# cliangyu/video-diffusion

Measured on AMD Instinct MI355X. Metric: denoise-steps/sec, higher is better.
Workload: dtype f32

## Files before the change

include/vd_amd.h:

```cpp
#ifndef VD_AMD_H
#define VD_AMD_H
#ifdef __cplusplus
extern "C" {
#endif

typedef struct vd_config {
    int image_size;
    int num_channels;
    int num_res_blocks;
    int num_heads;
    int T;
    int n_attention_ds;
    int attention_ds[8];
    int use_scale_shift_norm;
    int use_spatial_encoding;
    int use_frame_encoding;
    int enforce_position_invariance;
    int use_rpe_net;
    int allow_interactions_between_padding;
    float rp_alpha, rp_beta, rp_gamma;
    int time_embed_mult;
    int cond_emb_type;
    int learn_sigma;
} vd_config;
// ... 121 lines not shown
int vd_known_region(vd_engine* e);
int vd_known_merge(vd_engine* e, int B, int T, long long frame_pixels, float* sample, const float* known_src, const float* known_mask,
                   const float* latent_mask, const long long* t, const float* known_noise, unsigned long long seed,
                   unsigned long long offset, void* stream);
int vd_set_jump_rows(vd_engine* e, int num_timesteps, const float* sqrt_alpha, const float* sqrt_beta);
int vd_q_jump(vd_engine* e, int B, int T, long long frame_pixels, const float* x, const float* latent_mask, const long long* t,
              const float* noise, unsigned long long seed, unsigned long long offset, float* out, void* stream);
int vd_window_jump(vd_engine* e, int n, void* stream);

int vd_set_measurement(vd_engine* e, const float* y, int scale, int gray);
int vd_measurement(vd_engine* e, int* scale, int* gray);
int vd_measurement_project(vd_engine* e, int B, int T, int H, int W, float* x0_inout, const float* y, const float* latent_mask, int scale,
                           int gray, void* stream);

int vd_posterior_update(vd_engine* e, int mode, int B, long long per_sample, const float* x, const float* eps,
                        const long long* t, int clip_denoised, float eta, const float* noise,
                        unsigned long long seed, unsigned long long offset, float* sample, float* pred_xstart,
                        void* stream);

int vd_posterior_from_xstart(vd_engine* e, int mode, int B, long long per_sample, const float* x, const float* xstart_in,
                             const long long* t, int clip_denoised, float eta, const float* noise,
                             unsigned long long seed, unsigned long long offset, float* sample, float* pred_xstart,
                             float* mean, void* stream);

int vd_attn_blocks(vd_engine* e);
int vd_attn_block_info(vd_engine* e, int i, int* resolution, int* channels);
int vd_set_attn_capture(vd_engine* e, float* const* temporal, float* const* spatial, int n);

long long vd_bwd_weights_bytes(vd_engine* e);
int vd_set_bwd_weight_storage(vd_engine* e, void* buf, long long bytes, int on_host);
int vd_load_weight_bwd(vd_engine* e, const char* name, const float* host_data, long long numel);
int vd_guided_step(vd_engine* e, int B, int T, const float* x, const float* obs_mask, const float* latent_mask,
                   const float* kinda_marg_mask, const long long* frame_indices, const long long* t, int clip_denoised,
                   const float* x_t_minus_1, const float* noise, const float* noise2, float* mean, float* pred_xstart,
                   float* grad, float* sample, void* stream);

int vd_q_sample(vd_engine* e, int B, long long per_sample, const float* x_start, const long long* t,
                const float* noise, float* out, void* stream);

int vd_randn(float* out, long long n, unsigned long long seed, unsigned long long offset, void* stream);

int vd_profile_begin(void);
int vd_profile_end(double* out, int cap);
int vd_profile_classes(void);
const char* vd_profile_class_name(int i);

int vd_math_mode(void);
long long vd_split_image_u16(long long n_out, long long k_total);

int vd_op_conv(const float* src0, const float* src1, int C0, int Cin, int nfr, int Hs, int Ws, int ups, int stride,
               int pad, int ksz, const float* w_packed, const float* w_frag, const float* w_wino, const float* bias,
               const float* affA, const float* affB, int act, const float* res, const float* fbias, int fbias_ld,
               float* out, int Cout, void* stream);
int vd_conv_stats_split(int Hout);
int vd_conv_wino_block_couts(int nfr, int H, int Cin, int Cout);
int vd_op_conv_stats(const float* src0, int Cin, int nfr, int Hs, int Ws, int ups, const float* w_wino, const float* bias,
                     const float* res, const float* fbias, int fbias_ld, float* out, int Cout, double* gn_part,
                     void* stream);
int vd_op_gn_affine(const double* part0, int split0, int C0, const double* part1, int split1, int C, int nfr, int HW,
                    const float* gamma, const float* beta, const float* film, int film_ld, float* affA, float* affB,
                    void* stream);
int vd_pack_conv3_wino(const float* host_oihw, float* host_out, int O, int I);
int vd_pack_linear_frag(const float* host_w, float* host_out, int N, int K);
int vd_pack_linear_split(const float* host_w, unsigned short* host_out, int N, int K);
int vd_pack_conv3_split(const float* host_oihw, unsigned short* host_out, int O, int I);
int vd_op_conv_split(const float* src0, int Cin, int nfr, int Hs, int Ws, int stride, const void* w_split, const float* bias,
                     const float* res, float* out, int Cout, void* stream);
int vd_pack_conv3_wino_split(const float* host_oihw, unsigned short* host_out, int O, int I);
int vd_op_conv_wino_split(const float* src0, int Cin, int nfr, int Hs, int Ws, int ups, const void* w_split, const float* bias,
                          const float* res, const float* fbias, int fbias_ld, float* out, int Cout, double* gn_part,
                          void* stream);
int vd_op_conv_wino_act(const float* src0, const float* src1, int C0, int Cin, int nfr, int Hs, int Ws, const void* w_split, const float* bias,
                        const float* affA, const float* affB, const float* res, float* out, int Cout, double* gn_part, void* stream);
int vd_conv_wino_act_ok(int nfr, int H, int Cin, int Cout);
int vd_pack_conv3_wino_ups(const float* host_oihw, unsigned short* host_out, int O, int I);
int vd_conv_ups_stats_split(int Hs);
int vd_op_conv_wino_ups(const float* src0, int Cin, int nfr, int Hs, const void* w_ups, const float* bias, float* out, int Cout,
                        double* gn_part, void* stream);
int vd_op_linear_split(const float* a, int M, int K, const void* w_split, const float* bias, const float* res, int act,
                       float* out, int N, void* stream);
int vd_op_linear_split_stats(const float* a, int M, int K, const void* w_split, const float* bias, const float* res, int act,
                             float* out, int N, int HW, double* gn_part, void* stream);
int vd_linear_stats_split(int M, int N, int HW);
int vd_op_gn_fold(const float* src0, const float* src1, int C0, int C, int nfr, int HW, const float* gamma,
                  const float* beta, const float* film, int film_ld, float* affA, float* affB, void* stream);
int vd_op_affine_apply(const float* x, const float* affA, const float* affB, int nfr, int HW, int C, float* y,
                       void* stream);
int vd_op_affine_act(const float* src0, const float* src1, int C0, int C, const float* affA, const float* affB, int nfr,
                     int HW, int act, float* y, void* stream);
int vd_op_gn_temporal(const float* x, const float* gamma, const float* beta, int B, int T, int HW, int C, float* y,
                      void* stream);
int vd_op_attn_spatial(const float* qkv, int nfr, int L, int C, int heads, float* out, void* stream);
int vd_op_attn_temporal(const float* qkv, const float* Rk, const float* Rq, const float* Rv, const float* mask, int B,
                        int T, int HW, int C, int heads, int allow_pad, float* out, void* stream);
int vd_attn_temporal_variant(int T, int HW, int C, int heads, int rpe, char* name, int cap);
int vd_attn_spatial_variant(int L, int C, int heads, char* name, int cap);
int vd_op_out_conv(const float* x, const float* affA, const float* affB, const float* w_packed, const float* bias,
                   int nfr, int H, int W, int C, int Cout, float* out_nchw, void* stream);
int vd_op_gn_bwd(const float* x0, const float* x1, int C0, int C, const float* affA, const float* affB, const float* mr,
                 const float* dy, int act, int nfr, int HW, const float* extra, float* dx0, int acc0, float* dx1, int acc1,
                 void* stream);
int vd_op_gn_temporal_bwd(const float* x, const float* gamma, const float* dy, int B, int T, int HW, int C, int accumulate,
                          float* dx, void* stream);
int vd_op_attn_temporal_bwd(const float* qkv, const float* Rk, const float* Rq, const float* Rv, const float* mask, int B,
                            int T, int HW, int C, int heads, int allow_pad, const float* dout, float* dqkv, void* stream);
int vd_op_attn_spatial_bwd(const float* qkv, int nfr, int L, int C, int heads, const float* dout, float* dqkv, void* stream);
int vd_op_out_conv_bwd(const float* deps, const float* w, int nfr, int H, int W, int C, int Cout, float* da, void* stream);
int vd_op_stem_col2im(const float* dcols, const float* obs, const float* lat, const float* km, int nfr, int H, int W,
                      int cond_mode, float* dx, void* stream);
int vd_op_sinus_embed(const float* t, int n, int dim, const float* freqs, float* out, void* stream);
int vd_op_frame_t(const long long* frame_indices, int B, int T, int center, float* tv, void* stream);
int vd_op_rpe_hidden(const float* te, int te_ld, const float* wbase, const long long* tab, const long long* frame_indices, int B, int T,
                     int C, float* E, int nz, long long zs_e, void* stream);
int vd_op_rpe_table(const float* table, const long long* frame_indices, int B, int T, int C, float alpha, float beta, float gamma,
                    float* R, void* stream);
int vd_op_posenc_add(const float* x, const float* P, const float* femb, int nfr, int HW, int C, float* y, void* stream);
int vd_op_assemble(const float* x, const float* obs_src, const float* obs_mask, const float* latent_mask, const float* kinda_marg_mask,
                   const float* t_model, int obs_t_mode, int B, int T, int H, int W, int Kpad, int cond_mode, const int* frame_list,
                   int n_list, int scalars_only, float* x_cols, float* t_frames, float* amask, void* stream);
int vd_op_move_rows(int scatter, const float* src, const int* list, int n, long long row_floats, float* dst, void* stream);
int vd_op_scatter_stats(const double* src, int split, int C, const int* list, int n, double* dst, void* stream);

typedef struct vd_lpips vd_lpips;
int vd_lpips_create(vd_lpips** out);
void vd_lpips_destroy(vd_lpips* h);
int vd_lpips_load_weight(vd_lpips* h, const char* name, const float* host, long long bytes);
long long vd_lpips_dim(int H, int W);
int vd_lpips_embed(vd_lpips* h, int N, int H, int W, const float* frames, float* out, void* stream);
int vd_fps_select(int B, int n_cand, long long D, const float* embs, int n, const int* always_host, int n_always, float* work,
                  int* out, void* stream);

int vd_frame_metrics(int N, int C, int H, int W, const float* gt, const void* pred, int pred_is_u8, double ssim_data_range,
                     double* ssim_out, double* psnr_out, void* stream);
int vd_pair_sqdist(int N, long long D, const float* a, const float* b, double* out, void* stream);

int vd_hallway_counts(int N, int H, int W, int row0, int row1, const void* frames, int is_u8, int* counts, void* stream);
int vd_hallway_max_strip(void);
int vd_op_green_mask(long long n, const unsigned char* rgb, unsigned char* hsv, unsigned char* mask, void* stream);

typedef struct vd_i3d vd_i3d;
int vd_i3d_create(vd_i3d** out);
void vd_i3d_destroy(vd_i3d* h);
int vd_i3d_load_weight(vd_i3d* h, const char* name, const float* host, long long bytes);
int vd_i3d_max_frames(void);
int vd_i3d_embed(vd_i3d* h, int N, int T, int H, int W, const unsigned char* videos, float* out, void* stream);
int vd_op_conv3d_same(const float* x, const float* w, const float* bias, int T, int H, int W, int Cin, int Cout, int kt, int kh,
                      int kw, int st, int sh, int sw, int relu, float* out, long long out_stride, void* stream);
int vd_op_maxpool3d_same(const float* x, int T, int H, int W, int C, int kt, int kh, int kw, int st, int sh, int sw, float* out,
                         void* stream);
int vd_op_resize_bilinear_tf1(const unsigned char* frames, int T, int H, int W, float* out, void* stream);

#ifdef __cplusplus
}
#endif
#endif
```

video-diffusion_amd/_lib.py:

```python
import ctypes
import os
import subprocess

_HERE = os.path.dirname(os.path.abspath(__file__))
_CSRC = os.path.join(_HERE, "csrc")
SO_PATH = os.path.join(_HERE, "libvdamd.so")
SOURCES = ["igemm.hip", "conv_wino.hip", "conv_wino_r64.hip", "conv_wino_z128.hip", "gemm_frag.hip", "gemm_split.hip", "split_pack.hip", "norm.hip", "backward.hip", "attn_spatial.hip", "attn_temporal.hip", "attn_temporal_long.hip", "misc.hip", "guidance.hip", "known.hip", "measure.hip", "engine.hip", "lpips.hip", "metrics.hip", "i3d.hip", "conv_cl.hip", "hallway.hip"]
HEADER = os.path.join(os.path.dirname(_HERE), "include", "vd_amd.h")
HEADERS = [os.path.join(_CSRC, "vd_common.h"), os.path.join(_CSRC, "wino_common.h"), os.path.join(_CSRC, "igemm_tile.h"), HEADER]
SOURCE_FLAGS = {"conv_wino_z128.hip": ["-mllvm", "-pragma-unroll-threshold=1000000"]}


def _toolchain():
    hipcc = os.environ.get("HIPCC", "/opt/rocm/bin/hipcc")
    flags = ["--offload-arch=gfx950", "-O3", "-std=c++17", "-fPIC", "-Wno-unused-value"] + \
        os.environ.get("VD_HIPCC_FLAGS", "").split()
    return hipcc, flags


def _sha(*parts):
    import hashlib
    h = hashlib.sha1()
    for p in parts:
        h.update(p if isinstance(p, bytes) else str(p).encode())
# ... 114 lines not shown
    "vd_device_errors": (_I, [_P, ctypes.POINTER(_I)]),
    "vd_pos_channels": (_I, [_P]),
    "vd_pos_resolution": (_I, [_P]),
    "vd_set_freqs": (_I, [_P, _P, _I, _P, _I]),
    "vd_set_schedule": (_I, [_P, _I, _P, _P, _F]),
    "vd_workspace_bytes": (_I, [_P, _I, _I, ctypes.POINTER(_L)]),
    "vd_unet_forward": (_I, [_P, _I, _I, _P, _P, _P, _P, _P, _P, _P, _I, _P, _P]),
    "vd_p_sample": (_I, [_P, _I, _I, _P, _P, _P, _P, _P, _P, _P, _I, _I, _P, _U, _U, _P, _P, _P, _P]),
    "vd_ddim_sample": (_I, [_P, _I, _I, _P, _P, _P, _P, _P, _P, _P, _I, _I, _F, _P, _U, _U, _P, _P, _P, _P]),
    "vd_ddim_reverse_sample": (_I, [_P, _I, _I, _P, _P, _P, _P, _P, _P, _P, _I, _I, _P, _P, _P, _P]),
    "vd_ddim_reverse_from_xstart": (_I, [_P, _I, _L, _P, _P, _P, _I, _P, _P, _P]),
    "vd_set_multistep_weights": (_I, [_P, _I, _P]),
    "vd_dpmpp_2m_sample": (_I, [_P, _I, _I, _P, _P, _P, _P, _P, _P, _P, _P, _I, _I, _P, _P, _P, _P]),
    "vd_dpmpp_2m_from_xstart": (_I, [_P, _I, _L, _P, _P, _P, _P, _I, _P, _P, _P]),
    "vd_p_mean_variance": (_I, [_P, _I, _I, _P, _P, _P, _P, _P, _P, _P, _I, _I, _P, _P, _P, _P]),
    "vd_vb_terms": (_I, [_P, _I, _I, _P, _P, _P, _P, _P, _I, _P, _P, _P, _P, _P, _P]),
    "vd_prior_bpd": (_I, [_P, _I, _I, _P, _P, _P, _P]),
    "vd_score_windows": (_I, [_P, _I, _I, _P, _P, _P, _P, _P, _P, _I, _U, _P, _P, _I, _P, _P]),
    "vd_op_eps_mse": (_I, [_P, _I, _I, _P, _P, _P, _I, _P, _U, _P, _P, _P, _P]),
    "vd_window_generation": (_U, [_P]),
    "vd_set_window_prefix_cache": (_I, [_P, _I]),
    "vd_window_prefix_frames": (_I, [_P]),
    "vd_set_window_suffix_skip": (_I, [_P, _I]),
    "vd_window_suffix_frames": (_I, [_P]),
    "vd_set_cfg_scale": (_I, [_P, _F]),
    "vd_cfg_scale": (_F, [_P]),
    "vd_op_cfg_combine": (_I, [_P, _P, _F, _L, _P, _P]),
    "vd_set_guidance_rescale": (_I, [_P, _F]),
    "vd_guidance_rescale": (_F, [_P]),
    "vd_set_dynamic_threshold": (_I, [_P, _F]),
    "vd_dynamic_threshold": (_F, [_P]),
    "vd_op_cfg_rescale": (_I, [_P, _P, _F, _P, _I, _I, _L, _F, _P, _P, _P]),
    "vd_op_dynamic_threshold": (_I, [_P, _P, _I, _I, _L, _F, _P, _P, _P]),
    "vd_set_known_region": (_I, [_P, _P, _P, _P, _U, _U]),
    "vd_known_region": (_I, [_P]),
    "vd_known_merge": (_I, [_P, _I, _I, _L, _P, _P, _P, _P, _P, _P, _U, _U, _P]),
    "vd_set_jump_rows": (_I, [_P, _I, _P, _P]),
    "vd_q_jump": (_I, [_P, _I, _I, _L, _P, _P, _P, _P, _U, _U, _P, _P]),
    "vd_window_jump": (_I, [_P, _I, _P]),
    "vd_set_measurement": (_I, [_P, _P, _I, _I]),
    "vd_measurement": (_I, [_P, _P, _P]),
    "vd_measurement_project": (_I, [_P, _I, _I, _I, _I, _P, _P, _P, _I, _I, _P]),
    "vd_window_begin": (_I, [_P, _I, _I, _P, _P, _P, _P, _P, _P, _I, _I, _I, _F, _U, _U, _L, _P]),
    "vd_window_run": (_I, [_P, _I, _P]),
    "vd_window_graphs": (_I, [_P]),
    "vd_posterior_update": (_I, [_P, _I, _I, _L, _P, _P, _P, _I, _F, _P, _U, _U, _P, _P, _P]),
    "vd_posterior_from_xstart": (_I, [_P, _I, _I, _L, _P, _P, _P, _I, _F, _P, _U, _U, _P, _P, _P, _P]),
    "vd_attn_blocks": (_I, [_P]),
    "vd_attn_block_info": (_I, [_P, _I, ctypes.POINTER(_I), ctypes.POINTER(_I)]),
    "vd_set_attn_capture": (_I, [_P, _P, _P, _I]),
    "vd_bwd_weights_bytes": (_L, [_P]),
    "vd_set_bwd_weight_storage": (_I, [_P, _P, _L, _I]),
    "vd_load_weight_bwd": (_I, [_P, ctypes.c_char_p, _P, _L]),
    "vd_guided_step": (_I, [_P, _I, _I, _P, _P, _P, _P, _P, _P, _I, _P, _P, _P, _P, _P, _P, _P, _P]),
    "vd_q_sample": (_I, [_P, _I, _L, _P, _P, _P, _P, _P]),
    "vd_randn": (_I, [_P, _L, _U, _U, _P]),
    "vd_profile_begin": (_I, []),
    "vd_profile_end": (_I, [_P, _I]),
    "vd_profile_classes": (_I, []),
    "vd_profile_class_name": (ctypes.c_char_p, [_I]),
    "vd_op_conv": (_I, [_P, _P, _I, _I, _I, _I, _I, _I, _I, _I, _I, _P, _P, _P, _P, _P, _P, _I, _P, _P, _I, _P, _I, _P]),
    "vd_conv_stats_split": (_I, [_I]),
    "vd_conv_wino_block_couts": (_I, [_I, _I, _I, _I]),
    "vd_op_conv_stats": (_I, [_P, _I, _I, _I, _I, _I, _P, _P, _P, _P, _I, _P, _I, _P, _P]),
    "vd_op_gn_affine": (_I, [_P, _I, _I, _P, _I, _I, _I, _I, _P, _P, _P, _I, _P, _P, _P]),
    "vd_pack_conv3_wino": (_I, [_P, _P, _I, _I]),
    "vd_pack_linear_frag": (_I, [_P, _P, _I, _I]),
    "vd_pack_linear_split": (_I, [_P, _P, _I, _I]),
    "vd_pack_conv3_wino_split": (_I, [_P, _P, _I, _I]),
    "vd_set_model_mean_type": (_I, [_P, _I]),
    "vd_math_mode": (_I, []),
    "vd_split_image_u16": (_L, [_L, _L]),
    "vd_pack_conv3_wino_ups": (_I, [_P, _P, _I, _I]),
    "vd_conv_ups_stats_split": (_I, [_I]),
    "vd_op_conv_wino_ups": (_I, [_P, _I, _I, _I, _P, _P, _P, _I, _P, _P]),
    "vd_op_conv_wino_split": (_I, [_P, _I, _I, _I, _I, _I, _P, _P, _P, _P, _I, _P, _I, _P, _P]),
    "vd_op_conv_wino_act": (_I, [_P, _P, _I, _I, _I, _I, _I, _P, _P, _P, _P, _P, _P, _I, _P, _P]),
    "vd_conv_wino_act_ok": (_I, [_I, _I, _I, _I]),
    "vd_pack_conv3_split": (_I, [_P, _P, _I, _I]),
    "vd_op_conv_split": (_I, [_P, _I, _I, _I, _I, _I, _P, _P, _P, _P, _I, _P]),
    "vd_op_linear_split": (_I, [_P, _I, _I, _P, _P, _P, _I, _P, _I, _P]),
    "vd_op_linear_split_stats": (_I, [_P, _I, _I, _P, _P, _P, _I, _P, _I, _I, _P, _P]),
    "vd_linear_stats_split": (_I, [_I, _I, _I]),
    "vd_op_gn_fold": (_I, [_P, _P, _I, _I, _I, _I, _P, _P, _P, _I, _P, _P, _P]),
    "vd_op_affine_apply": (_I, [_P, _P, _P, _I, _I, _I, _P, _P]),
    "vd_op_affine_act": (_I, [_P, _P, _I, _I, _P, _P, _I, _I, _I, _P, _P]),
    "vd_op_gn_temporal": (_I, [_P, _P, _P, _I, _I, _I, _I, _P, _P]),
    "vd_op_attn_spatial": (_I, [_P, _I, _I, _I, _I, _P, _P]),
    "vd_op_attn_temporal": (_I, [_P, _P, _P, _P, _P, _I, _I, _I, _I, _I, _I, _P, _P]),
    "vd_attn_temporal_variant": (_I, [_I, _I, _I, _I, _I, ctypes.c_char_p, _I]),
    "vd_attn_spatial_variant": (_I, [_I, _I, _I, ctypes.c_char_p, _I]),
    "vd_op_out_conv": (_I, [_P, _P, _P, _P, _P, _I, _I, _I, _I, _I, _P, _P]),
    "vd_op_gn_bwd": (_I, [_P, _P, _I, _I, _P, _P, _P, _P, _I, _I, _I, _P, _P, _I, _P, _I, _P]),
    "vd_op_gn_temporal_bwd": (_I, [_P, _P, _P, _I, _I, _I, _I, _I, _P, _P]),
    "vd_op_attn_temporal_bwd": (_I, [_P, _P, _P, _P, _P, _I, _I, _I, _I, _I, _I, _P, _P, _P]),
    "vd_op_attn_spatial_bwd": (_I, [_P, _I, _I, _I, _I, _P, _P, _P]),
    "vd_op_out_conv_bwd": (_I, [_P, _P, _I, _I, _I, _I, _I, _P, _P]),
    "vd_op_stem_col2im": (_I, [_P, _P, _P, _P, _I, _I, _I, _I, _P, _P]),
    "vd_op_sinus_embed": (_I, [_P, _I, _I, _P, _P, _P]),
    "vd_op_frame_t": (_I, [_P, _I, _I, _I, _P, _P]),
    "vd_op_rpe_hidden": (_I, [_P, _I, _P, _P, _P, _I, _I, _I, _P, _I, _L, _P]),
    "vd_op_rpe_table": (_I, [_P, _P, _I, _I, _I, _F, _F, _F, _P, _P]),
    "vd_op_posenc_add": (_I, [_P, _P, _P, _I, _I, _I, _P, _P]),
    "vd_op_assemble": (_I, [_P, _P, _P, _P, _P, _P, _I, _I, _I, _I, _I, _I, _I, _P, _I, _I, _P, _P, _P, _P]),
    "vd_op_move_rows": (_I, [_I, _P, _P, _I, _L, _P, _P]),
    "vd_op_scatter_stats": (_I, [_P, _I, _I, _P, _I, _P, _P]),
    "vd_lpips_create": (_I, [ctypes.POINTER(_P)]),
    "vd_lpips_destroy": (None, [_P]),
    "vd_lpips_load_weight": (_I, [_P, ctypes.c_char_p, _P, _L]),
    "vd_lpips_dim": (_L, [_I, _I]),
    "vd_lpips_embed": (_I, [_P, _I, _I, _I, _P, _P, _P]),
    "vd_fps_select": (_I, [_I, _I, _L, _P, _I, _P, _I, _P, _P, _P]),
    "vd_frame_metrics": (_I, [_I, _I, _I, _I, _P, _P, _I, _D, _P, _P, _P]),
    "vd_pair_sqdist": (_I, [_I, _L, _P, _P, _P, _P]),
    "vd_i3d_create": (_I, [ctypes.POINTER(_P)]),
    "vd_i3d_destroy": (None, [_P]),
    "vd_i3d_load_weight": (_I, [_P, ctypes.c_char_p, _P, _L]),
    "vd_i3d_max_frames": (_I, []),
    "vd_i3d_embed": (_I, [_P, _I, _I, _I, _I, _P, _P, _P]),
    "vd_op_conv3d_same": (_I, [_P, _P, _P, _I, _I, _I, _I, _I, _I, _I, _I, _I, _I, _I, _I, _P, _L, _P]),
    "vd_op_maxpool3d_same": (_I, [_P, _I, _I, _I, _I, _I, _I, _I, _I, _I, _I, _P, _P]),
    "vd_op_resize_bilinear_tf1": (_I, [_P, _I, _I, _I, _P, _P]),
    "vd_hallway_counts": (_I, [_I, _I, _I, _I, _I, _P, _I, _P, _P]),
    "vd_hallway_max_strip": (_I, []),
    "vd_op_green_mask": (_I, [_L, _P, _P, _P, _P]),
}

_lib = None


def lib():
    global _lib
    if _lib is None:
        path = os.environ.get("VD_LIB")
        if not path:
            build()
            path = SO_PATH
        L = ctypes.CDLL(path)
        for name, (res, args) in SIGNATURES.items():
            fn = getattr(L, name)
            fn.restype = res
            fn.argtypes = args
        if not os.environ.get("VD_LIB") and L.vd_source_sha().decode() != source_sha():
            raise RuntimeError(f"libvdamd.so was built from other sources ({L.vd_source_sha().decode()}) than the ones beside it "
                               f"({source_sha()}): rebuild (video_diffusion_amd._lib.build(force=True))")
        _lib = L
    return _lib


class VdError(RuntimeError):
    pass


def check(rc):
    if rc != 0:
        msg = lib().vd_last_error().decode(errors="replace")
        raise VdError(f"libvdamd error {rc}: {msg}")


def ptr(t):
    if t is None:
        return None
    if hasattr(t, "data_ptr"):
        return ctypes.c_void_p(t.data_ptr())
    return ctypes.c_void_p(t.ctypes.data)

# ... 5 lines not shown
```

video-diffusion_amd/csrc/attn_temporal.hip:

```cpp
#include "vd_common.h"
#include <cstdlib>
#include <string>

namespace vd {

__device__ __forceinline__ float dot4(f32x4 a, f32x4 b) { return a.x * b.x + a.y * b.y + a.z * b.z + a.w * b.w; }

template <int PB, int TMAX, bool RPE>
__global__ __launch_bounds__(256) void attn_temporal_kernel(AttnTemporalArgs a) {
    extern __shared__ __attribute__((aligned(16))) float smem[];
    const int T = a.T, C = a.C, HW = a.HW, C3 = 3 * a.C;
    const int F = C / a.heads, F4 = F >> 2, FP = F + 4, TS = T + 1;
    float* qs = smem;
    float* ks = qs + PB * T * FP;
    float* sc = ks + PB * T * FP;
    const int b = blockIdx.z, h = blockIdx.y, p0 = blockIdx.x * PB;
    const int np = min(PB, HW - p0);
    const int tid = threadIdx.x;
    const float* qkv_b = a.qkv + (size_t)b * T * HW * C3 + h * F;

    for (int idx = tid; idx < PB * T * F4; idx += 256) {
        const int f4 = idx % F4, r = idx / F4;
        const int t = r % T, p = r / T;
        const float* src = qkv_b + ((size_t)t * HW + p0 + min(p, np - 1)) * C3 + f4 * 4;
        f32x4 q = *reinterpret_cast<const f32x4*>(src) * a.scale;
        f32x4 k = *reinterpret_cast<const f32x4*>(src + C);
        if (p >= np) { q = f32x4{0.f, 0.f, 0.f, 0.f}; k = q; }
        *reinterpret_cast<f32x4*>(qs + (p * T + t) * FP + f4 * 4) = q;
        *reinterpret_cast<f32x4*>(ks + (p * T + t) * FP + f4 * 4) = k;
    }
    __syncthreads();

    for (int pr = tid; pr < T * T; pr += 256) {
        const int t = pr / T, s = pr - t * T;
        float acc[PB];
#pragma unroll
        for (int p = 0; p < PB; ++p) acc[p] = 0.f;
        const float* rk = RPE ? a.Rk + (((size_t)b * T + t) * T + s) * C + h * F : nullptr;
        const float* rq = RPE ? a.Rq + (((size_t)b * T + s) * T + t) * C + h * F : nullptr;
        const float* qrow = qs + t * FP;
        const float* krow = ks + s * FP;
#pragma unroll 3
        for (int f0 = 0; f0 < F; f0 += 8) {
            f32x4 rk0, rk1, rq0, rq1;
            if constexpr (RPE) {
                rk0 = *reinterpret_cast<const f32x4*>(rk + f0); rk1 = *reinterpret_cast<const f32x4*>(rk + f0 + 4);
                rq0 = *reinterpret_cast<const f32x4*>(rq + f0) * a.scale; rq1 = *reinterpret_cast<const f32x4*>(rq + f0 + 4) * a.scale;
            }
#pragma unroll
            for (int p = 0; p < PB; ++p) {
                const f32x4 q0 = *reinterpret_cast<const f32x4*>(qrow + p * T * FP + f0);
                const f32x4 q1 = *reinterpret_cast<const f32x4*>(qrow + p * T * FP + f0 + 4);
                const f32x4 k0 = *reinterpret_cast<const f32x4*>(krow + p * T * FP + f0);
                const f32x4 k1 = *reinterpret_cast<const f32x4*>(krow + p * T * FP + f0 + 4);
                if constexpr (RPE)
                    acc[p] += dot4(q0, k0 + rk0) + dot4(q1, k1 + rk1) + dot4(k0, rq0) + dot4(k1, rq1);
                else
                    acc[p] += dot4(q0, k0) + dot4(q1, k1);
            }
        }
        bool masked = false;
        if (a.mask) {
            const float mt = a.mask[b * T + t], ms = a.mask[b * T + s];
            float allowed = mt * ms;
            if (a.allow_pad) allowed += (1.f - mt) * (1.f - ms);
            else if (t == s) allowed = 1.f;
            masked = allowed == 0.f;
        }
#pragma unroll
        for (int p = 0; p < PB; ++p) sc[(p * T + t) * TS + s] = masked ? -INFINITY : acc[p];
    }
    __syncthreads();

    for (int row = tid; row < np * T; row += 256) {
        float* r = sc + row * TS;
        float mx = -INFINITY;
        for (int s = 0; s < T; ++s) mx = fmaxf(mx, r[s]);
        float sum = 0.f;
        for (int s = 0; s < T; ++s) { const float e = __expf(r[s] - mx); r[s] = e; sum += e; }
        const float inv = 1.0f / sum;
        for (int s = 0; s < T; ++s) r[s] *= inv;
    }
    __syncthreads();

    for (int item = tid; item < T * F4; item += 256) {
        const int t = item / F4, f4 = item - t * F4;
        f32x4 rv[TMAX];
#pragma unroll
        for (int s = 0; s < TMAX; ++s) {
            rv[s] = f32x4{0.f, 0.f, 0.f, 0.f};
            if constexpr (RPE)
                rv[s] = *reinterpret_cast<const f32x4*>(a.Rv + (((size_t)b * T + t) * T + min(s, T - 1)) * C + h * F + f4 * 4);
        }
        for (int p = 0; p < np; ++p) {
            const float* ar = sc + (p * T + t) * TS;
            const float* vbase = qkv_b + 2 * C + (size_t)(p0 + p) * C3 + f4 * 4;
            f32x4 o = {0.f, 0.f, 0.f, 0.f};
#pragma unroll
            for (int s = 0; s < TMAX; ++s) {
                const f32x4 v = *reinterpret_cast<const f32x4*>(vbase + (size_t)min(s, T - 1) * HW * C3);
                const float w = s < T ? ar[min(s, T - 1)] : 0.f;
                o += (v + rv[s]) * w;
            }
            *reinterpret_cast<f32x4*>(a.out + (((size_t)b * T + t) * HW + p0 + p) * C + h * F + f4 * 4) = o;
        }
    }
}

#ifdef VD_ATT_TIMING
__device__ unsigned long long g_att_stamp[16];
#define ATT_STAMP(i)                                                                                   \
    do {                                                                                               \
        if (threadIdx.x == 0 && blockIdx.x == 3 && blockIdx.y == 1 && blockIdx.z == 2) {               \
            __builtin_amdgcn_sched_barrier(0);                                                         \
            g_att_stamp[i] = __builtin_amdgcn_s_memrealtime();                                         \
            __builtin_amdgcn_sched_barrier(0);                                                         \
        }                                                                                              \
    } while (0)
extern "C" int vd_debug_att_stamps(unsigned long long* host_out) {
    return (int)hipMemcpyFromSymbol(host_out, HIP_SYMBOL(g_att_stamp), sizeof(g_att_stamp));
}
#else
#define ATT_STAMP(i)
#endif

__device__ __forceinline__ f32x4 mfma4(float x, float y, f32x4 c) { return __builtin_amdgcn_mfma_f32_16x16x4f32(x, y, c, 0, 0, 0); }

__device__ __forceinline__ void rows_regs_transpose(float& x0, float& x1, float& x2, float& x3) {
    auto u = [](float f) { return __builtin_bit_cast(unsigned, f); };
    auto f = [](unsigned v) { return __builtin_bit_cast(float, v); };
    auto p01 = __builtin_amdgcn_permlane16_swap(u(x0), u(x1), false, false);
    auto p23 = __builtin_amdgcn_permlane16_swap(u(x2), u(x3), false, false);
    auto q02 = __builtin_amdgcn_permlane32_swap(p01[0], p23[0], false, false);
    auto q13 = __builtin_amdgcn_permlane32_swap(p01[1], p23[1], false, false);
    x0 = f(q02[0]); x2 = f(q02[1]); x1 = f(q13[0]); x3 = f(q13[1]);
}

template <int NT, int JM, bool RPE, bool EXACT>
__global__ __launch_bounds__(512, 2) void attn_temporal_mfma_kernel(AttnTemporalArgs a) {
    constexpr int TP = 16 * NT, RS = TP + 1, PS = TP * RS + (NT == 1 ? 1 : 17);
    extern __shared__ __attribute__((aligned(16))) float smem[];
    float* w = smem;
    const int T = EXACT ? 16 * NT : a.T, C = a.C, HW = a.HW, C3 = 3 * a.C;
    const int F = C / a.heads, NJ = EXACT ? JM : F >> 4;
    const int b = blockIdx.z, h = blockIdx.y, p0 = blockIdx.x * 16;
    const int tid = threadIdx.x, wv = tid >> 6, l = tid & 63, i16 = l & 15, g = l >> 4;
    const float* qb = a.qkv + ((size_t)b * T * HW + p0) * C3 + h * F;
    auto row = [&](int t, int px) { return qb + ((size_t)t * HW + px) * C3; };
    auto ld4 = [](const float* p) { return *reinterpret_cast<const f32x4*>(p); };
    const int tcl[2] = {min(i16, T - 1), min(16 + i16, T - 1)};
    const f32x4 zero4 = {0.f, 0.f, 0.f, 0.f};

    ATT_STAMP(0);
    constexpr int JG = NT == 1 ? 2 : 1, NG = JM / JG, NU = 2 * NT;
    constexpr bool AHEAD = NT == 1;
    struct Ops { f32x4 qa1[2][NT][JG], kb1[2][NT][JG], xa2[NU][JG], rb2[NU][NT][JG], xa3[NU][JG], rb3[NU][NT][JG]; };
    f32x4 acc1[2][NT][NT], acc2[NU][NT], acc3[NU][NT];
#pragma unroll
    for (int u = 0; u < 2; ++u)
#pragma unroll
        for (int m = 0; m < NT; ++m)
#pragma unroll
            for (int n = 0; n < NT; ++n) acc1[u][m][n] = zero4;
#pragma unroll
    for (int u = 0; u < NU; ++u)
#pragma unroll
        for (int n = 0; n < NT; ++n) { acc2[u][n] = zero4; acc3[u][n] = zero4; }
    const float* q1[2][NT];
#pragma unroll
    for (int u = 0; u < 2; ++u)
#pragma unroll
        for (int m = 0; m < NT; ++m) q1[u][m] = row(tcl[m], 2 * wv + u) + 4 * g;
    const float* rkq[NT];
#pragma unroll
    for (int n = 0; n < NT; ++n) rkq[n] = (size_t)b * T * T * C + (size_t)tcl[n] * C + h * F + 4 * g + (const float*)nullptr;
    auto request = [&](Ops& o, int grp, bool own, bool rel) {
#pragma unroll
        for (int jj = 0; jj < JG; ++jj) {
            const int j = grp * JG + jj;
            if (EXACT || j < NJ) {
                if (own) {
#pragma unroll
                    for (int u = 0; u < 2; ++u)
#pragma unroll
                        for (int m = 0; m < NT; ++m) { o.qa1[u][m][jj] = ld4(q1[u][m] + 16 * j); o.kb1[u][m][jj] = ld4(q1[u][m] + C + 16 * j); }
                }
                if constexpr (RPE) {
#pragma unroll
                    for (int u = 0; u < (rel ? NU : 0); ++u) {
                        const int t = wv + 8 * u;
                        if (EXACT || t < T) {
                            const float* xr = row(t, i16) + 4 * g + 16 * j;
                            o.xa2[u][jj] = ld4(xr);
                            o.xa3[u][jj] = ld4(xr + C);
#pragma unroll
                            for (int n = 0; n < NT; ++n) {
                                const size_t ro = (size_t)(rkq[n] - (const float*)nullptr) + (size_t)t * T * C + 16 * j;
                                o.rb2[u][n][jj] = ld4(a.Rk + ro);
                                o.rb3[u][n][jj] = ld4(a.Rq + ro);
                            }
                        }
                    }
                }
            }
        }
    };
    auto products = [&](const Ops& o, int grp, bool own, bool rel) {
#pragma unroll
        for (int jj = 0; jj < JG; ++jj) {
            if (EXACT || grp * JG + jj < NJ) {
#pragma unroll
                for (int e = 0; e < 4; ++e) {
#pragma unroll
                    for (int u = 0; u < (own ? 2 : 0); ++u)
#pragma unroll
                        for (int m = 0; m < NT; ++m)
#pragma unroll
                            for (int n = 0; n < NT; ++n) acc1[u][m][n] = mfma4(o.qa1[u][m][jj][e] * a.scale, o.kb1[u][n][jj][e], acc1[u][m][n]);
                    if constexpr (RPE) {
#pragma unroll
                        for (int u = 0; u < (rel ? NU : 0); ++u)
                            if (EXACT || wv + 8 * u < T) {
#pragma unroll
                                for (int n = 0; n < NT; ++n) {
                                    acc2[u][n] = mfma4(o.xa2[u][jj][e] * a.scale, o.rb2[u][n][jj][e], acc2[u][n]);
                                    acc3[u][n] = mfma4(o.xa3[u][jj][e], o.rb3[u][n][jj][e] * a.scale, acc3[u][n]);
                                }
                            }
                    }
                }
            }
        }
    };
    if constexpr (AHEAD) {
        Ops o[2];
        request(o[0], 0, true, true);
#pragma unroll
        for (int grp = 0; grp < NG; ++grp) {
            if (grp + 1 < NG) request(o[(grp + 1) & 1], grp + 1, true, true);
            __builtin_amdgcn_sched_barrier(0);
            products(o[grp & 1], grp, true, true);
            __builtin_amdgcn_sched_barrier(0);
        }
    } else {
#pragma unroll 1
        for (int grp = 0; grp < NG; ++grp) {
            Ops o;
            request(o, grp, true, false);
            products(o, grp, true, false);
            if constexpr (RPE) {
                request(o, grp, false, true);
                products(o, grp, false, true);
            }
        }
    }
    ATT_STAMP(1);
#pragma unroll
    for (int u = 0; u < 2; ++u)
#pragma unroll
        for (int m = 0; m < NT; ++m)
#pragma unroll
            for (int n = 0; n < NT; ++n)
#pragma unroll
                for (int r = 0; r < 4; ++r) w[(2 * wv + u) * PS + (16 * m + 4 * g + r) * RS + 16 * n + i16] = acc1[u][m][n][r];
    __syncthreads();
    if constexpr (RPE) {
#pragma unroll
        for (int u = 0; u < NU; ++u) {
            const int t = wv + 8 * u;
            if (t < T) {
#pragma unroll
                for (int n = 0; n < NT; ++n)
#pragma unroll
                    for (int r = 0; r < 4; ++r) w[(4 * g + r) * PS + t * RS + 16 * n + i16] += acc2[u][n][r];
            }
        }
        __syncthreads();
#pragma unroll
        for (int u = 0; u < NU; ++u) {
            const int sk = wv + 8 * u;
            if (sk < T) {
#pragma unroll
                for (int n = 0; n < NT; ++n)
#pragma unroll
                    for (int r = 0; r < 4; ++r) w[(4 * g + r) * PS + (16 * n + i16) * RS + sk] += acc3[u][n][r];
            }
        }
        __syncthreads();
    }

    ATT_STAMP(2);
    for (int rix = tid; rix < 16 * TP; rix += 512) {
        const int px = rix / TP, t = rix - px * TP;
        float* r = w + px * PS + t * RS;
        if (t >= T) {
            for (int s = 0; s < TP; ++s) r[s] = 0.f;
            continue;
        }
        float mx = -INFINITY;
        const float mt = a.mask ? a.mask[b * T + t] : 1.f;
        for (int s = 0; s < T; ++s) {
            float v = r[s];
            if (a.mask) {
                const float ms = a.mask[b * T + s];
                float allowed = mt * ms;
                if (a.allow_pad) allowed += (1.f - mt) * (1.f - ms);
                else if (t == s) allowed = 1.f;
                if (allowed == 0.f) v = -INFINITY;
            }
            r[s] = v;
            mx = fmaxf(mx, v);
        }
        float sum = 0.f;
        for (int s = 0; s < T; ++s) { const float e = __expf(r[s] - mx); r[s] = e; sum += e; }
        const float inv = 1.0f / sum;
        for (int s = 0; s < T; ++s) r[s] *= inv;
        for (int s = T; s < TP; ++s) r[s] = 0.f;
    }
    __syncthreads();

    ATT_STAMP(3);
    const int KS = (T + 3) >> 2;
    if (EXACT ? wv < JM : wv < NJ) {
        const int f0 = 16 * wv + i16;
        const float* vb = qb + 2 * C + f0;
        const float* rvb = RPE ? a.Rv + ((size_t)b * T) * T * C + h * F + f0 : nullptr;
#pragma unroll 1
        for (int m = 0; m < NT; ++m) {
            if (16 * m >= T) break;
            float rr[NT == 1 ? 4 : 1][16];
            f32x4 acc[16];
#pragma unroll
            for (int px = 0; px < 16; ++px) acc[px] = zero4;
#pragma unroll 1
            for (int kc = 0; kc < NT; ++kc) {
                if (16 * kc >= T) break;
                float vr[4][16];
#pragma unroll
                for (int k4 = 0; k4 < 4; ++k4)
                    if (EXACT || 4 * kc + k4 < KS) {
                        const float* vs = vb + (size_t)min(16 * kc + 4 * k4 + g, T - 1) * HW * C3;
#pragma unroll
                        for (int px = 0; px < 16; ++px) vr[k4][px] = vs[(size_t)px * C3];
                    }
                if constexpr (RPE && NT == 1) {
#pragma unroll
                    for (int k4 = 0; k4 < 4; ++k4)
                        if (EXACT || k4 < KS) {
                            const float* rv = rvb + (size_t)min(4 * k4 + g, T - 1) * C;
#pragma unroll
                            for (int tl = 0; tl < 16; ++tl) rr[k4][tl] = rv[(size_t)min(tl, T - 1) * T * C];
                        }
                }
                __builtin_amdgcn_sched_barrier(0);
#pragma unroll
                for (int k4 = 0; k4 < 4; ++k4)
                    if (EXACT || 4 * kc + k4 < KS) {
                        const float* ar = w + (16 * m + i16) * RS + 16 * kc + 4 * k4 + g;
#pragma unroll
                        for (int px = 0; px < 16; ++px) acc[px] = mfma4(ar[px * PS], vr[k4][px], acc[px]);
                    }
            }
            ATT_STAMP(4);
            f32x4 res[16];
#pragma unroll
            for (int bq = 0; bq < 4; ++bq)
#pragma unroll
                for (int d = 0; d < 4; ++d) {
                    float x0 = acc[bq][d], x1 = acc[4 + bq][d], x2 = acc[8 + bq][d], x3 = acc[12 + bq][d];
                    rows_regs_transpose(x0, x1, x2, x3);
                    res[d][bq] = x0; res[4 + d][bq] = x1; res[8 + d][bq] = x2; res[12 + d][bq] = x3;
                }
            if constexpr (RPE) {
                if constexpr (NT == 1) {
#pragma unroll
                    for (int k4 = 0; k4 < 4; ++k4)
                        if (EXACT || k4 < KS) {
                            const float* ar = w + i16 * PS + 4 * k4 + g;
#pragma unroll
                            for (int tl = 0; tl < 16; ++tl) res[tl] = mfma4(ar[tl * RS], rr[k4][tl], res[tl]);
                        }
                } else {
#pragma unroll 1
                    for (int kc = 0; kc < NT; ++kc) {
                        if (16 * kc >= T) break;
                        float r4[4][16];
#pragma unroll
                        for (int k4 = 0; k4 < 4; ++k4)
                            if (4 * kc + k4 < KS) {
                                const float* rv = rvb + (size_t)min(16 * kc + 4 * k4 + g, T - 1) * C;
#pragma unroll
                                for (int tl = 0; tl < 16; ++tl) r4[k4][tl] = rv[(size_t)min(16 * m + tl, T - 1) * T * C];
                            }
#pragma unroll
                        for (int k4 = 0; k4 < 4; ++k4)
                            if (4 * kc + k4 < KS) {
                                const float* ar = w + i16 * PS + (16 * m) * RS + 16 * kc + 4 * k4 + g;
#pragma unroll
                                for (int tl = 0; tl < 16; ++tl) res[tl] = mfma4(ar[tl * RS], r4[k4][tl], res[tl]);
                            }
                    }
                }
            }
            ATT_STAMP(5);
#pragma unroll
            for (int tl = 0; tl < 16; ++tl) {
                const int t = 16 * m + tl;
                if (t < T) {
                    float* o = a.out + (((size_t)b * T + t) * HW + p0 + 4 * g) * C + h * F + f0;
// ... 85 lines not shown
```

video-diffusion_amd/csrc/attn_temporal_long.hip:

```cpp
#include "vd_common.h"

namespace vd {

namespace {

__device__ __forceinline__ f32x4 mfma_l(float x, float y, f32x4 c) { return __builtin_amdgcn_mfma_f32_16x16x4f32(x, y, c, 0, 0, 0); }

__device__ __forceinline__ void rows_regs_transpose_l(float& x0, float& x1, float& x2, float& x3) {
    auto u = [](float f) { return __builtin_bit_cast(unsigned, f); };
    auto f = [](unsigned v) { return __builtin_bit_cast(float, v); };
    auto p01 = __builtin_amdgcn_permlane16_swap(u(x0), u(x1), false, false);
    auto p23 = __builtin_amdgcn_permlane16_swap(u(x2), u(x3), false, false);
    auto q02 = __builtin_amdgcn_permlane32_swap(p01[0], p23[0], false, false);
    auto q13 = __builtin_amdgcn_permlane32_swap(p01[1], p23[1], false, false);
    x0 = f(q02[0]); x2 = f(q02[1]); x1 = f(q13[0]); x3 = f(q13[1]);
}

__device__ __forceinline__ bool frame_pair_allowed(const AttnTemporalArgs& a, int b, int t, int s) {
    if (!a.mask) return true;
    const float mt = a.mask[b * a.T + t], ms = a.mask[b * a.T + s];
    float allowed = mt * ms;
    if (a.allow_pad) allowed += (1.f - mt) * (1.f - ms);
    else if (t == s) allowed = 1.f;
    return allowed != 0.f;
}

}

template <int NJ, bool RPE>
__global__ __launch_bounds__(512, 2) void attn_temporal_long_mfma_kernel(AttnTemporalArgs a) {
    constexpr int RS = 17, PS = 16 * RS;
    extern __shared__ __attribute__((aligned(16))) float smem[];
    float* pb = smem;
    float* al = pb + 16 * PS;
    float* s1 = al + 256;
    float* s2 = s1 + 16 * PS;
    float* s3 = s2 + 16 * PS;
    const int T = a.T, C = a.C, HW = a.HW, C3 = 3 * a.C, F = 16 * NJ;
    const int NQ = (T + 15) >> 4;
    const int b = blockIdx.z / NQ, t0 = 16 * (blockIdx.z - b * NQ), h = blockIdx.y, p0 = blockIdx.x * 16;
    const int tid = threadIdx.x, wv = tid >> 6, l = tid & 63, i16 = l & 15, g = l >> 4;
    const float* qb = a.qkv + ((size_t)b * T * HW + p0) * C3 + h * F;
    auto row = [&](int t, int px) { return qb + ((size_t)t * HW + px) * C3; };
    auto ld4 = [](const float* p) { return *reinterpret_cast<const f32x4*>(p); };
    const f32x4 zero4 = {0.f, 0.f, 0.f, 0.f};
    const size_t rbase = (size_t)b * T * T * C + h * F;
    const int tq = min(t0 + i16, T - 1);

    f32x4 acc[16];
#pragma unroll
    for (int i = 0; i < 16; ++i) acc[i] = zero4;
    float m_run = -INFINITY, l_run = 0.f;

    const int NK = (T + 15) >> 4;
#pragma unroll 1
    for (int kt = 0; kt < NK; ++kt) {
        const int s0 = 16 * kt;
        const int sk = min(s0 + i16, T - 1);
        f32x4 a1[2], a2[2], a3[2];
#pragma unroll
        for (int u = 0; u < 2; ++u) { a1[u] = zero4; a2[u] = zero4; a3[u] = zero4; }
        const int tf[2] = {min(t0 + wv, T - 1), min(t0 + wv + 8, T - 1)};
        const int sf[2] = {min(s0 + wv, T - 1), min(s0 + wv + 8, T - 1)};
#pragma unroll
        for (int j = 0; j < NJ; ++j) {
            const int fo = 16 * j + 4 * g;
            f32x4 qa[2], kb[2], x2[2], r2[2], x3[2], r3[2];
#pragma unroll
            for (int u = 0; u < 2; ++u) {
                qa[u] = ld4(row(tq, 2 * wv + u) + fo);
                kb[u] = ld4(row(sk, 2 * wv + u) + C + fo);
                if constexpr (RPE) {
                    x2[u] = ld4(row(tf[u], i16) + fo);
                    r2[u] = ld4(a.Rk + rbase + ((size_t)tf[u] * T + sk) * C + fo);
                    x3[u] = ld4(row(sf[u], i16) + C + fo);
                    r3[u] = ld4(a.Rq + rbase + ((size_t)sf[u] * T + tq) * C + fo);
                }
            }
#pragma unroll
            for (int e = 0; e < 4; ++e)
#pragma unroll
                for (int u = 0; u < 2; ++u) {
                    a1[u] = mfma_l(qa[u][e] * a.scale, kb[u][e], a1[u]);
                    if constexpr (RPE) {
                        a2[u] = mfma_l(x2[u][e] * a.scale, r2[u][e], a2[u]);
                        a3[u] = mfma_l(x3[u][e], r3[u][e] * a.scale, a3[u]);
                    }
                }
        }
#pragma unroll
        for (int u = 0; u < 2; ++u)
#pragma unroll
            for (int r = 0; r < 4; ++r) {
                s1[(2 * wv + u) * PS + (4 * g + r) * RS + i16] = a1[u][r];
                if constexpr (RPE) {
                    s2[(4 * g + r) * PS + (wv + 8 * u) * RS + i16] = a2[u][r];
                    s3[(4 * g + r) * PS + i16 * RS + wv + 8 * u] = a3[u][r];
                }
            }
        __syncthreads();

        if (tid < 256) {
            const int px = tid >> 4, tl = tid & 15, t = min(t0 + tl, T - 1);
            const int o = px * PS + tl * RS;
            float w[16];
            float mx = m_run;
#pragma unroll
            for (int s = 0; s < 16; ++s) {
                float v = s1[o + s];
                if constexpr (RPE) v = v + s2[o + s] + s3[o + s];
                if (s0 + s >= T || !frame_pair_allowed(a, b, t, s0 + s)) v = -INFINITY;
                w[s] = v;
                mx = fmaxf(mx, v);
            }
            const bool none = mx == -INFINITY;
            const float alpha = none ? 1.f : __expf(m_run - mx);
            float sum = 0.f;
#pragma unroll
            for (int s = 0; s < 16; ++s) {
                const float p = none ? 0.f : __expf(w[s] - mx);
                pb[o + s] = p;
                sum += p;
            }
            l_run = l_run * alpha + sum;
            m_run = mx;
            al[tid] = alpha;
        }
        __syncthreads();

        if (wv < NJ) {
            const int f0 = h * F + 16 * wv + i16;
#pragma unroll
            for (int tl = 0; tl < 16; ++tl)
#pragma unroll
                for (int r = 0; r < 4; ++r) acc[tl][r] *= al[(4 * g + r) * 16 + tl];
            if constexpr (RPE) {
                const float* rvb = a.Rv + (size_t)b * T * T * C + f0;
#pragma unroll 1
                for (int k4 = 0; k4 < 4; ++k4) {
                    const int s = min(s0 + 4 * k4 + g, T - 1);
                    float rr[16];
#pragma unroll
                    for (int tl = 0; tl < 16; ++tl) rr[tl] = rvb[((size_t)min(t0 + tl, T - 1) * T + s) * C];
#pragma unroll
                    for (int tl = 0; tl < 16; ++tl) acc[tl] = mfma_l(pb[i16 * PS + tl * RS + 4 * k4 + g], rr[tl], acc[tl]);
                }
            }
            f32x4 pv[16];
#pragma unroll
            for (int px = 0; px < 16; ++px) pv[px] = zero4;
            const float* vb = a.qkv + ((size_t)b * T * HW + p0) * C3 + 2 * C + f0;
#pragma unroll 1
            for (int k4 = 0; k4 < 4; ++k4) {
                const int s = min(s0 + 4 * k4 + g, T - 1);
                float vr[16];
#pragma unroll
                for (int px = 0; px < 16; ++px) vr[px] = vb[((size_t)s * HW + px) * C3];
#pragma unroll
                for (int px = 0; px < 16; ++px) pv[px] = mfma_l(pb[px * PS + i16 * RS + 4 * k4 + g], vr[px], pv[px]);
            }
#pragma unroll
            for (int bq = 0; bq < 4; ++bq)
#pragma unroll
                for (int d = 0; d < 4; ++d) {
                    float x0 = pv[bq][d], x1 = pv[4 + bq][d], x2 = pv[8 + bq][d], x3 = pv[12 + bq][d];
                    rows_regs_transpose_l(x0, x1, x2, x3);
                    acc[d][bq] += x0; acc[4 + d][bq] += x1; acc[8 + d][bq] += x2; acc[12 + d][bq] += x3;
                }
        }
    }
    __syncthreads();
    if (tid < 256) al[tid] = 1.0f / l_run;
    __syncthreads();

    if (wv < NJ) {
        const int f0 = h * F + 16 * wv + i16;
#pragma unroll
        for (int tl = 0; tl < 16; ++tl) {
            const int t = t0 + tl;
            if (t < T) {
                float* o = a.out + (((size_t)b * T + t) * HW + p0 + 4 * g) * C + f0;
#pragma unroll
                for (int r = 0; r < 4; ++r) o[(size_t)r * C] = acc[tl][r] * al[(4 * g + r) * 16 + tl];
            }
        }
    }
}

template <bool RPE>
__global__ __launch_bounds__(256) void attn_temporal_long_kernel(AttnTemporalArgs a) {
    extern __shared__ __attribute__((aligned(16))) float sc[];
    const int T = a.T, C = a.C, HW = a.HW, C3 = 3 * a.C, F = C / a.heads, F4 = F >> 2, TS = T + 1;
    const int NQ = (T + 15) >> 4;
    const int b = blockIdx.z / NQ, t0 = 16 * (blockIdx.z - b * NQ), h = blockIdx.y, p = blockIdx.x;
    const int nq = min(16, T - t0);
    const int tid = threadIdx.x;
    const float* qb = a.qkv + ((size_t)b * T * HW + p) * C3 + h * F;
    const size_t fr = (size_t)HW * C3;
    auto ld4 = [](const float* x) { return *reinterpret_cast<const f32x4*>(x); };

    for (int pr = tid; pr < nq * T; pr += 256) {
        const int tl = pr / T, s = pr - tl * T, t = t0 + tl;
        const float* q = qb + t * fr;
        const float* k = qb + s * fr + C;
        const float* rk = RPE ? a.Rk + (((size_t)b * T + t) * T + s) * C + h * F : nullptr;
        const float* rq = RPE ? a.Rq + (((size_t)b * T + s) * T + t) * C + h * F : nullptr;
        float acc = 0.f;
        for (int f = 0; f < F; f += 4) {
            const f32x4 qv = ld4(q + f) * a.scale, kv = ld4(k + f);
            if constexpr (RPE) {
                const f32x4 kr = kv + ld4(rk + f), rqv = ld4(rq + f) * a.scale;
                acc += qv.x * kr.x + qv.y * kr.y + qv.z * kr.z + qv.w * kr.w + kv.x * rqv.x + kv.y * rqv.y + kv.z * rqv.z + kv.w * rqv.w;
            } else {
                acc += qv.x * kv.x + qv.y * kv.y + qv.z * kv.z + qv.w * kv.w;
            }
        }
        sc[tl * TS + s] = frame_pair_allowed(a, b, t, s) ? acc : -INFINITY;
    }
    __syncthreads();
    if (tid < nq) {
        float* r = sc + tid * TS;
        float mx = -INFINITY;
        for (int s = 0; s < T; ++s) mx = fmaxf(mx, r[s]);
        float sum = 0.f;
        for (int s = 0; s < T; ++s) { const float e = mx == -INFINITY ? 0.f : __expf(r[s] - mx); r[s] = e; sum += e; }
        const float inv = 1.0f / sum;
        for (int s = 0; s < T; ++s) r[s] *= inv;
    }
    __syncthreads();
    for (int item = tid; item < nq * F4; item += 256) {
        const int tl = item / F4, f4 = item - tl * F4, t = t0 + tl;
        const float* ar = sc + tl * TS;
        const float* vb = qb + 2 * C + 4 * f4;
        const float* rv = RPE ? a.Rv + (((size_t)b * T + t) * T) * C + h * F + 4 * f4 : nullptr;
        f32x4 o = {0.f, 0.f, 0.f, 0.f};
        for (int s = 0; s < T; ++s) {
            f32x4 v = ld4(vb + s * fr);
            if constexpr (RPE) v += ld4(rv + (size_t)s * C);
            o += v * ar[s];
        }
        *reinterpret_cast<f32x4*>(a.out + (((size_t)b * T + t) * HW + p) * C + h * F + 4 * f4) = o;
    }
}

template <int NJ, bool RPE>
static int launch_long_mfma(const AttnTemporalArgs& a, hipStream_t s) {
    constexpr int PS = 16 * 17;
    constexpr size_t lds = ((size_t)(RPE ? 4 : 2) * 16 * PS + 256) * sizeof(float);
    if (lds > 48 * 1024) VD_RAISE_LDS((&attn_temporal_long_mfma_kernel<NJ, RPE>), lds);
    dim3 grid(a.HW / 16, a.heads, a.B * ((a.T + 15) / 16));
    hipLaunchKernelGGL((attn_temporal_long_mfma_kernel<NJ, RPE>), grid, dim3(512), lds, s, a);
    VD_HIP(hipGetLastError());
    return 0;
}

template <bool RPE>
static int launch_long_generic(const AttnTemporalArgs& a, hipStream_t s) {
    const size_t lds = (size_t)16 * (a.T + 1) * sizeof(float);
    dim3 grid(a.HW, a.heads, a.B * ((a.T + 15) / 16));
    hipLaunchKernelGGL((attn_temporal_long_kernel<RPE>), grid, dim3(256), lds, s, a);
    VD_HIP(hipGetLastError());
    return 0;
}

template <bool RPE>
static int launch_long_nj(const AttnTemporalArgs& a, int nj, hipStream_t s) {
    switch (nj) {
        case 1: return launch_long_mfma<1, RPE>(a, s);
        case 2: return launch_long_mfma<2, RPE>(a, s);
        case 3: return launch_long_mfma<3, RPE>(a, s);
        case 4: return launch_long_mfma<4, RPE>(a, s);
        case 5: return launch_long_mfma<5, RPE>(a, s);
        case 6: return launch_long_mfma<6, RPE>(a, s);
        case 7: return launch_long_mfma<7, RPE>(a, s);
        default: return launch_long_mfma<8, RPE>(a, s);
    }
}

int launch_attn_temporal_long(const AttnTemporalArgs& a, hipStream_t s) {
    const bool rpe = a.Rk != nullptr;
    const AttnTemporalVariant v = attn_temporal_variant(a.T, a.HW, a.C, a.heads, rpe);
    VD_REQUIRE(v.family == AttnTemporalVariant::kLongMfma || v.family == AttnTemporalVariant::kLongGeneric, "long temporal window: 33..128 frames");
    if (v.family == AttnTemporalVariant::kLongMfma) return rpe ? launch_long_nj<true>(a, v.p0, s) : launch_long_nj<false>(a, v.p0, s);
    return rpe ? launch_long_generic<true>(a, s) : launch_long_generic<false>(a, s);
}

}
```

video-diffusion_amd/csrc/backward.hip:

```cpp
#include <algorithm>
#include <cmath>

#include "vd_common.h"

namespace vd {

__device__ __forceinline__ float sigmoid_f(float v) { return __builtin_amdgcn_rcpf(1.0f + __expf(-v)); }
__device__ __forceinline__ float silu_grad_f(float y) { const float s = sigmoid_f(y); return s * (1.0f + y * (1.0f - s)); }

__global__ __launch_bounds__(256) void gn_bwd_partial_kernel(GnBwdArgs a, int split, int per) {
    const int n = blockIdx.y, sp = blockIdx.x;
    const int C = a.C, tpp = C >> 2, ppi = 256 / tpp, cg = C / 32;
    const int tid = threadIdx.x, pl = tid / tpp, q = tid - pl * tpp, c = q * 4;
    const int p_begin = sp * per, p_end = min(a.HW, p_begin + per);
    double t1[4] = {0, 0, 0, 0}, t2[4] = {0, 0, 0, 0};
    if (pl < ppi) {
        const float* src; int ld;
        if (c < a.C0) { src = a.x0 + (size_t)n * a.HW * a.C0 + c; ld = a.C0; } else { src = a.x1 + (size_t)n * a.HW * (C - a.C0) + (c - a.C0); ld = C - a.C0; }
        const f32x4 A = *reinterpret_cast<const f32x4*>(a.A + (size_t)n * C + c), B = *reinterpret_cast<const f32x4*>(a.B + (size_t)n * C + c);
        float mu[4];
#pragma unroll
        for (int e = 0; e < 4; ++e) mu[e] = a.mr[((size_t)n * 32 + (c + e) / cg) * 2];
        for (int p = p_begin + pl; p < p_end; p += ppi) {
            const f32x4 x = *reinterpret_cast<const f32x4*>(src + (size_t)p * ld);
// ... 514 lines not shown
        const float nz = tl != 0 ? 1.0f : 0.0f;
        const float smp = mean + nz * expf(0.5f * tb[TAB_LOGVAR * NT]) * a.noise[i];
        const float om = a.obs[(size_t)b * a.T + (i - (size_t)b * a.per) / perf];
        const float dmean = 2.0f * (smp - a.xtm1[i]) * om * om;
        const float pass = (!a.clip || (x0r >= -1.0f && x0r <= 1.0f)) ? 1.0f : 0.0f;
        const float dx0r = tb[TAB_COEF1 * NT] * dmean * pass;
        a.deps[i] = -tb[TAB_SQRT_RECIPM1 * NT] * dx0r;
        a.dxd[i] = tb[TAB_COEF2 * NT] * dmean + tb[TAB_SQRT_RECIP * NT] * dx0r;
        if (a.mean) a.mean[i] = mean;
        if (a.xstart) a.xstart[i] = x0;
    }
}
int launch_guided_grad(const GuidedArgs& a, hipStream_t s) {
    const size_t total = (size_t)a.B * a.per;
    hipLaunchKernelGGL(guided_grad_kernel, dim3((unsigned)std::min<size_t>((total + 255) / 256, 4096)), dim3(256), 0, s, a);
    VD_HIP(hipGetLastError());
    return 0;
}

__global__ __launch_bounds__(256) void grad_absmax_kernel(const float* __restrict__ g, size_t n, unsigned* __restrict__ mx) {
    float m = 0.f;
    for (size_t i = (size_t)blockIdx.x * 256 + threadIdx.x; i < n; i += (size_t)gridDim.x * 256) m = fmaxf(m, fabsf(g[i]));
    for (int o = 32; o > 0; o >>= 1) m = fmaxf(m, __shfl_xor(m, o));
    if ((threadIdx.x & 63) == 0) atomicMax(mx, __builtin_bit_cast(unsigned, m));
}
__global__ __launch_bounds__(256) void grad_scale_kernel(float* __restrict__ g, size_t n, float* __restrict__ gs) {
    const float m = __builtin_bit_cast(float, reinterpret_cast<const unsigned*>(gs)[2]);
    float s = 1.f;
    if (m > 0.f && m < 3.0e38f) {
        int ex;
        (void)frexpf(m, &ex);
        s = ldexpf(1.f, max(-100, min(100, 1 - ex)));
    }
    if (blockIdx.x == 0 && threadIdx.x == 0) { gs[0] = s; gs[1] = 1.f / s; }
    for (size_t i = (size_t)blockIdx.x * 256 + threadIdx.x; i < n; i += (size_t)gridDim.x * 256) g[i] *= s;
}
int launch_grad_rescale(float* deps, size_t n, float* gs, hipStream_t st) {
    VD_HIP(hipMemsetAsync(gs, 0, 4 * sizeof(float), st));
    const unsigned grid = (unsigned)std::min<size_t>((n + 255) / 256, 1024);
    hipLaunchKernelGGL(grad_absmax_kernel, dim3(grid), dim3(256), 0, st, deps, n, reinterpret_cast<unsigned*>(gs) + 2);
    hipLaunchKernelGGL(grad_scale_kernel, dim3(grid), dim3(256), 0, st, deps, n, gs);
    VD_HIP(hipGetLastError());
    return 0;
}

__global__ __launch_bounds__(256) void guided_final_kernel(GuidedArgs a, const float* __restrict__ dx_net, const float* __restrict__ noise2,
                                                           float* __restrict__ grad, float* __restrict__ mean_out, float* __restrict__ sample) {
    const float inv_s = a.gscale[1];
    const size_t total = (size_t)a.B * a.per;
    for (size_t i = (size_t)blockIdx.x * 256 + threadIdx.x; i < total; i += (size_t)gridDim.x * 256) {
        const int b = (int)(i / a.per);
        const long long tl = a.t[b];
        const int NT = a.num_timesteps;
        if (tl < 0 || tl >= NT) { if (mean_out) mean_out[i] = __builtin_nanf(""); if (sample) sample[i] = __builtin_nanf(""); continue; }
        const float* tb = a.tab + (int)tl;
        const float g = a.dxd[i] + dx_net[i] * inv_s;
        const float m = a.mean[i] - 10.0f * tb[TAB_ALPHA * NT] * g / 2.0f;
        if (grad) grad[i] = g;
        if (mean_out) mean_out[i] = m;
        if (sample) sample[i] = m + (tl != 0 ? 1.0f : 0.0f) * expf(0.5f * tb[TAB_LOGVAR * NT]) * noise2[i];
    }
}
int launch_guided_final(const GuidedArgs& a, const float* dx_net, const float* noise2, float* grad, float* mean_out, float* sample, hipStream_t s) {
    const size_t total = (size_t)a.B * a.per;
    hipLaunchKernelGGL(guided_final_kernel, dim3((unsigned)std::min<size_t>((total + 255) / 256, 4096)), dim3(256), 0, s, a, dx_net, noise2, grad, mean_out,
                       sample);
    VD_HIP(hipGetLastError());
    return 0;
}

}

namespace vd {

template <bool RPE>
__global__ __launch_bounds__(256) void attn_temporal_weights_kernel(AttnTemporalArgs a, float* __restrict__ out) {
    extern __shared__ __attribute__((aligned(16))) float smem[];
    const int T = a.T, C = a.C, HW = a.HW, C3 = 3 * C, F = C / a.heads, FP = F + 4, TS = T + 1;
    float* qs = smem;
    float* ks = qs + T * FP;
    float* P = ks + T * FP;
    float* M = P + T * TS;
    const int p = blockIdx.x, b = blockIdx.y, tid = threadIdx.x;
    const size_t tok0 = (size_t)b * T * HW + p;
    for (int i = tid; i < T * TS; i += 256) M[i] = 0.f;
    for (int h = 0; h < a.heads; ++h) {
        __syncthreads();
        for (int i = tid; i < T * F; i += 256) {
            const int t = i / F, f = i - t * F;
            const float* r = a.qkv + (tok0 + (size_t)t * HW) * C3 + h * F + f;
            qs[t * FP + f] = r[0] * a.scale; ks[t * FP + f] = r[C];
        }
        __syncthreads();
        for (int pr = tid; pr < T * T; pr += 256) {
            const int t = pr / T, s_ = pr - t * T;
            const float* rk = RPE ? a.Rk + (((size_t)b * T + t) * T + s_) * C + h * F : nullptr;
            const float* rq = RPE ? a.Rq + (((size_t)b * T + s_) * T + t) * C + h * F : nullptr;
            float w = 0.f;
            for (int f = 0; f < F; ++f) {
                const float k = ks[s_ * FP + f];
                w += qs[t * FP + f] * (k + (RPE ? rk[f] : 0.f)) + (RPE ? a.scale * k * rq[f] : 0.f);
            }
            bool masked = false;
            if (a.mask) {
                const float mt = a.mask[b * T + t], ms = a.mask[b * T + s_];
                float allowed = mt * ms;
                if (a.allow_pad) allowed += (1.f - mt) * (1.f - ms);
                else if (t == s_) allowed = 1.f;
                masked = allowed == 0.f;
            }
            P[t * TS + s_] = masked ? -INFINITY : w;
        }
        __syncthreads();
        if (tid < T) {
            float* r = P + tid * TS;
            float mx = -INFINITY;
            for (int s_ = 0; s_ < T; ++s_) mx = fmaxf(mx, r[s_]);
            float sum = 0.f;
            for (int s_ = 0; s_ < T; ++s_) { const float e = __expf(r[s_] - mx); r[s_] = e; sum += e; }
            const float inv = 1.0f / sum;
            for (int s_ = 0; s_ < T; ++s_) M[tid * TS + s_] += r[s_] * inv;
        }
    }
    __syncthreads();
    const float ih = 1.0f / (float)a.heads;
    for (int i = tid; i < T * T; i += 256) out[((size_t)b * HW + p) * T * T + i] = fabsf(M[(i / T) * TS + (i % T)] * ih);
}

template <bool RPE>
__global__ __launch_bounds__(256) void attn_temporal_weights_long_kernel(AttnTemporalArgs a, float* __restrict__ out) {
    constexpr int QC = 32;
    extern __shared__ __attribute__((aligned(16))) float smem[];
    const int T = a.T, C = a.C, HW = a.HW, C3 = 3 * C, F = C / a.heads, FP = F + 4, TS = T + 1;
    const int p = blockIdx.x, b = blockIdx.y, r0 = QC * blockIdx.z, nr = min(QC, T - r0), tid = threadIdx.x;
    float* qs = smem;
    float* ks = qs + QC * FP;
    float* P = ks + T * FP;
    float* M = P + QC * TS;
    const size_t tok0 = (size_t)b * T * HW + p;
    for (int i = tid; i < QC * TS; i += 256) M[i] = 0.f;
    for (int h = 0; h < a.heads; ++h) {
        __syncthreads();
        for (int i = tid; i < T * F; i += 256) {
            const int t = i / F, f = i - t * F;
            const float* r = a.qkv + (tok0 + (size_t)t * HW) * C3 + h * F + f;
            if (t >= r0 && t < r0 + nr) qs[(t - r0) * FP + f] = r[0] * a.scale;
            ks[t * FP + f] = r[C];
        }
        __syncthreads();
        for (int pr = tid; pr < nr * T; pr += 256) {
            const int tl = pr / T, s_ = pr - tl * T, t = r0 + tl;
            const float* rk = RPE ? a.Rk + (((size_t)b * T + t) * T + s_) * C + h * F : nullptr;
            const float* rq = RPE ? a.Rq + (((size_t)b * T + s_) * T + t) * C + h * F : nullptr;
            float w = 0.f;
            for (int f = 0; f < F; ++f) {
                const float k = ks[s_ * FP + f];
                w += qs[tl * FP + f] * (k + (RPE ? rk[f] : 0.f)) + (RPE ? a.scale * k * rq[f] : 0.f);
            }
            bool masked = false;
            if (a.mask) {
                const float mt = a.mask[b * T + t], ms = a.mask[b * T + s_];
                float allowed = mt * ms;
                if (a.allow_pad) allowed += (1.f - mt) * (1.f - ms);
                else if (t == s_) allowed = 1.f;
                masked = allowed == 0.f;
            }
            P[tl * TS + s_] = masked ? -INFINITY : w;
        }
        __syncthreads();
        if (tid < nr) {
            float* r = P + tid * TS;
            float mx = -INFINITY;
            for (int s_ = 0; s_ < T; ++s_) mx = fmaxf(mx, r[s_]);
            float sum = 0.f;
            for (int s_ = 0; s_ < T; ++s_) { const float e = __expf(r[s_] - mx); r[s_] = e; sum += e; }
            const float inv = 1.0f / sum;
            for (int s_ = 0; s_ < T; ++s_) M[tid * TS + s_] += r[s_] * inv;
        }
    }
    __syncthreads();
    const float ih = 1.0f / (float)a.heads;
    float* o = out + (((size_t)b * HW + p) * T + r0) * T;
    for (int i = tid; i < nr * T; i += 256) o[i] = fabsf(M[(i / T) * TS + (i % T)] * ih);
}

static int launch_attn_temporal_weights_long(const AttnTemporalArgs& a, float* out, hipStream_t s) {
    constexpr int QC = 32;
    const int F = a.C / a.heads;
    const size_t lds = ((size_t)(QC + a.T) * (F + 4) + (size_t)2 * QC * (a.T + 1)) * sizeof(float);
    VD_REQUIRE(lds <= 150 * 1024, "temporal attention weights: head dim too large");
    const dim3 grid(a.HW, a.B, (a.T + QC - 1) / QC);
    if (a.Rk) {
        VD_RAISE_LDS((&attn_temporal_weights_long_kernel<true>), lds);
        hipLaunchKernelGGL(attn_temporal_weights_long_kernel<true>, grid, dim3(256), lds, s, a, out);
    } else {
        VD_RAISE_LDS((&attn_temporal_weights_long_kernel<false>), lds);
        hipLaunchKernelGGL(attn_temporal_weights_long_kernel<false>, grid, dim3(256), lds, s, a, out);
    }
    VD_HIP(hipGetLastError());
    return 0;
}

int launch_attn_temporal_weights(const AttnTemporalArgs& a, float* out, hipStream_t s) {
    VD_REQUIRE(a.T >= 1 && a.T <= kMaxWindowFrames && a.C % a.heads == 0, "temporal attention weights: shape");
    if (a.T > 32) return launch_attn_temporal_weights_long(a, out, s);
    const int F = a.C / a.heads;
    const size_t lds = ((size_t)2 * a.T * (F + 4) + (size_t)2 * a.T * (a.T + 1)) * sizeof(float);
    VD_REQUIRE(lds <= 150 * 1024, "temporal attention weights: head dim too large");
    const dim3 grid(a.HW, a.B);
    if (a.Rk) {
        VD_RAISE_LDS((&attn_temporal_weights_kernel<true>), lds);
        hipLaunchKernelGGL(attn_temporal_weights_kernel<true>, grid, dim3(256), lds, s, a, out);
    } else {
        VD_RAISE_LDS((&attn_temporal_weights_kernel<false>), lds);
        hipLaunchKernelGGL(attn_temporal_weights_kernel<false>, grid, dim3(256), lds, s, a, out);
    }
    VD_HIP(hipGetLastError());
    return 0;
}

__global__ __launch_bounds__(256) void attn_spatial_weights_kernel(AttnSpatialArgs a, float* __restrict__ out) {
    extern __shared__ __attribute__((aligned(16))) float smem[];
    const int L = a.L, C = a.C, C3 = 3 * C, F = C / a.heads, FP = F + 4, LS = L + 1;
    float* qs = smem;
    float* S = qs + SQT * FP;
    float* M = S + SQT * LS;
    const int n = blockIdx.y, t0 = blockIdx.x * SQT, tid = threadIdx.x;
    const size_t tok0 = (size_t)n * L;
    for (int i = tid; i < SQT * LS; i += 256) M[i] = 0.f;
    for (int h = 0; h < a.heads; ++h) {
        __syncthreads();
        for (int i = tid; i < SQT * F; i += 256) {
            const int t = i / F, f = i - t * F, tt = min(t0 + t, L - 1);
            qs[t * FP + f] = a.qkv[(tok0 + tt) * C3 + h * F + f] * a.scale;
        }
        __syncthreads();
// ... 50 lines not shown
```

video-diffusion_amd/csrc/engine.hip:

```cpp
#include <cmath>
#include <cstring>
#include <unordered_map>
#include <vector>

#include "../../include/vd_amd.h"
#include "vd_common.h"

namespace vd {

thread_local std::string g_last_error;
void set_error(const std::string& msg) { g_last_error = msg; }

int launch_frame_t(const int64_t* fidx, int B, int T, int center, float* tv, hipStream_t s);

enum ParamKind { PK_RAW = 0, PK_CONV3, PK_STEM, PK_POSENC, PK_OUTCONV, PK_LINF, PK_CONV3W, PK_CONV3S,
                 PK_CONV3WU };

struct Param {
    std::string name;
    int nd = 0;
    long long shape[4] = {1, 1, 1, 1};
    size_t numel = 0;
    size_t packed = 0;
    size_t off = 0;
    int kind = PK_RAW;
    bool loaded = false;
    int frag_rows = 0, frag_row0 = 0;
    int kind_bwd = -1;
    size_t off_bwd = 0, packed_bwd = 0;
};

struct ResP {
    int cin, cout;
    int gn1w, gn1b, c1w, c1b, embw, embb, gn2w, gn2b, c2w, c2b, skw = -1, skb = -1;
    int film_off = 0;
};
struct RpeP { int dw = -1, db = -1, tw = -1, tb = -1, ow = -1, ob = -1, table = -1; int te_off = 0; };
struct AttP { int normw, normb, qkvw, qkvb, projw, projb; };
struct AttnP { int C; AttP sp, tp; RpeP rq, rk, rv; };
struct ConvP { int w, b, c; };
struct Layer { int type; int idx; };
struct Tens { float* p; int C, H; double* part = nullptr; int split = 0; };

struct TapeRes { int idx; Tens x0, x1; bool has_x1; int N; float *A1, *B1, *mr1, *h, *A2, *B2, *mr2, *o; };
struct TapeAttn { int idx; Tens x; int B, T; float *xn, *qkv, *Rk, *Rq, *Rv, *o, *xt, *A, *Bf, *mr, *xn2, *qkv2, *o2, *xs; const float* amask; };
struct TapeConv { int type, idx; Tens in, out; };
struct TapePos { Tens in, out; };
struct TapeOp { int kind, i; };
struct Tape {
    std::vector<TapeOp> ops;
    std::vector<TapeRes> res; std::vector<TapeAttn> attn; std::vector<TapeConv> conv; std::vector<TapePos> pos;
    Tens head; float *headA = nullptr, *headB = nullptr, *head_mr = nullptr;
    void clear() { ops.clear(); res.clear(); attn.clear(); conv.clear(); pos.clear(); }
};

static const int CH_MULT_256[] = {1, 1, 2, 2, 4, 4};
static const int CH_MULT_128[] = {1, 1, 2, 3, 4};
static const int CH_MULT_64[] = {1, 2, 3, 4};
static const int CH_MULT_32[] = {1, 2, 2, 2};
static bool split_math() { return math_mode() != MATH_FP32; }

constexpr int STEM_KPAD = 64;

struct Arena {
    char* base = nullptr;
    size_t cap = 0, used = 0, peak = 0;
    bool dry = false, overflow = false;
    template <class Tp> Tp* get(size_t n) {
        size_t bytes = (n * sizeof(Tp) + 255) & ~(size_t)255;
        if (!dry && cap && used + bytes > cap) {
            overflow = true;
            return reinterpret_cast<Tp*>(base);
        }
        char* p = (dry ? reinterpret_cast<char*>(0x1000) : base) + used;
        used += bytes;
        peak = std::max(peak, used);
        return reinterpret_cast<Tp*>(p);
    }
    size_t mark() const { return used; }
    void release(size_t m) { used = m; }
};

enum ProfClass { PC_IGEMM_128x128 = 0, PC_IGEMM_128x64, PC_IGEMM_64x128, PC_IGEMM_64x64, PC_GN_STATS, PC_GN_TEMPORAL,
                 PC_ATTN_SPATIAL, PC_ATTN_TEMPORAL, PC_OUT_CONV, PC_ELEMENTWISE, PC_POSTERIOR,
                 PC_CONV_128x128, PC_CONV_128x64, PC_CONV_64x128, PC_CONV_64x64, PC_CONV_WINO, PC_CONV_WINO_R64, PC_IGEMM_128x192,
                 PC_CONV_WINO_R64_UPS, PC_CONV_WINO_Z128, PC_COUNT };
static const char* kProfNames[PC_COUNT][2] = {
    {"gemm_split_kernel<128,128>", "gemm_frag_kernel<128,128>"}, {"gemm_split_kernel<128,64>", "gemm_frag_kernel<128,64>"},
    {"gemm_split_kernel<64,128>", "gemm_frag_kernel<64,128>"}, {"gemm_split_kernel<64,64>", "gemm_frag_kernel<64,64>"},
    {"gn_stats_partial", "gn_stats_partial"}, {"gn_temporal_kernel", "gn_temporal_kernel"},
    {"attn_spatial_kernel", "attn_spatial_kernel"}, {"attn_temporal_kernel", "attn_temporal_kernel"},
    {"out_conv_kernel", "out_conv_kernel"}, {"affine_act_kernel", "affine_act_kernel"}, {"posterior_kernel", "posterior_kernel"},
    {"igemm_kernel<128,128> 3x3", "igemm_kernel<128,128> 3x3"}, {"igemm_kernel<128,64> 3x3", "igemm_kernel<128,64> 3x3"},
    {"igemm_kernel<64,128> 3x3", "igemm_kernel<64,128> 3x3"}, {"igemm_kernel<64,64> 3x3", "igemm_kernel<64,64> 3x3"},
    {"conv3x3_wino_kernel", "conv3x3_wino_kernel"}, {"conv3x3_wino_r64_kernel", "conv3x3_wino_r64_kernel"},
    {"gemm_split_kernel<128,192>", "gemm_split_kernel<128,192>"},
    {"conv3x3_wino_r64_ups_kernel", "conv3x3_wino_r64_ups_kernel"}, {"conv3x3_wino_z128_kernel", "conv3x3_wino_z128_kernel"}};
struct ProfRec { int cls; double flops, bytes; hipEvent_t a, b; char tag[56]; };
struct Profiler {
    bool on = false;
    std::vector<ProfRec> recs;
};
static Profiler g_prof;
static const char* prof_name(int i) {
    if (i < 0 || i >= PC_COUNT) return "";
    return kProfNames[i][!split_math()];
}

struct ProfScope {
    hipStream_t st; bool live;
    ProfScope(int cls, double flops, double bytes, hipStream_t s, const char* tag = "") : st(s), live(g_prof.on) {
        if (!live) return;
        ProfRec r{cls, flops, bytes, nullptr, nullptr, {0}};
        snprintf(r.tag, sizeof(r.tag), "%s", tag);
        (void)hipEventCreate(&r.a); (void)hipEventCreate(&r.b);
        (void)hipEventRecord(r.a, st);
        g_prof.recs.push_back(r);
    }
    ~ProfScope() { if (live) (void)hipEventRecord(g_prof.recs.back().b, st); }
};
struct ProfPause {
    bool was = g_prof.on;
    ProfPause() { g_prof.on = false; }
    ~ProfPause() { g_prof.on = was; }
};

static bool act_conv_will_dispatch(const IgemmArgs& g) {
    return g.affA && igemm_kernel(igemm_first_launch(g)) == IK_Z128;
}

static int igemm_p(const IgemmArgs& g, hipStream_t st, int cin_alg = 0) {
    const double taps = (double)g.ksz * g.ksz, cin = cin_alg ? cin_alg : g.Cin;
    const double in_pix = (double)g.nfr * g.Hs * g.Ws;
    const double nz = g.zcount > 1 ? g.zcount : 1;
    const double bytes = nz * 4.0 * (in_pix * cin + (double)g.M * g.Cout * (g.res ? 2 : 1) + taps * cin * g.Cout + (g.side ? in_pix * cin : 0.0));
    const IgemmArgs one = igemm_first_launch(g);
    const IgemmKernel k = igemm_kernel(one);
    const bool wino = k == IK_R64_UPS || k == IK_Z128 || k == IK_R64 || k == IK_WINO;
    const int tile = igemm_tile_class(igemm_sel_M(one), g.Cout);
    int cls;
    switch (k) {
        case IK_R64_UPS: cls = PC_CONV_WINO_R64_UPS; break;
        case IK_Z128: cls = PC_CONV_WINO_Z128; break;
        case IK_R64: cls = PC_CONV_WINO_R64; break;
        case IK_WINO: cls = PC_CONV_WINO; break;
        case IK_SPLIT: cls = gemm_split_tile_class(igemm_sel_M(one), g.Cout) == 4 ? (int)PC_IGEMM_128x192 : tile; break;
        default: cls = tile + (g.ksz == 3 ? (int)PC_CONV_128x128 : 0);
    }
    char tag[56];
    snprintf(tag, sizeof(tag), "M=%d N=%d K=%d k%d s%d%s%s%s", g.M, g.Cout, g.Cin, g.ksz, g.stride, g.ups ? " ups" : "",
             g.affA ? " pro" : (g.act ? " act" : ""), g.res ? " res" : "");
    VD_REQUIRE(g.stats == nullptr || wino || (k == IK_SPLIT && g.stats_hw > 0),
               "GroupNorm partial sums requested from a kernel that has no such epilogue");
    ProfScope ps(cls, nz * 2.0 * g.M * g.Cout * cin * taps, bytes, st, tag);
    return launch_igemm(g, st);
}

static int affine_act(const float* src0, const float* src1, int C0, int C, const float* A, const float* B, int N, int HW,
                      float* y, hipStream_t st) {
    ProfScope ps(PC_ELEMENTWISE, 0.0, 8.0 * N * HW * C, st);
    return launch_affine_act(src0, src1, C0, C, A, B, N, HW, 1, y, st);
}

struct FwdIn {
    int B, T;
    const float *x, *obs_src, *obs, *lat, *km, *t_model;
    const int64_t* fidx;
    int obs_mode;
    float* eps;
};

struct PrefixStore { std::vector<float*> tens; std::vector<double*> parts; std::vector<size_t> floats; };
struct PrefixPlan {
    int n = 0;
    const int* list = nullptr;
    bool build_only = false;
    PrefixStore* store = nullptr;
};

struct SuffixPlan { int n = 0; const int* list = nullptr; };

static inline int out_t_cols(int Cout) { return (9 * Cout + 31) / 32 * 32; }

static thread_local int g_sel_nfr = 0;

}

using namespace vd;

struct vd_engine {
    vd_config cfg;
    int E = 0;
    std::vector<Param> params;
    std::unordered_map<std::string, int> pidx;
    std::vector<ResP> res;
    std::vector<AttnP> attn;
    std::vector<ConvP> convs;
    std::vector<std::vector<Layer>> input_blocks, output_blocks;
    std::vector<Layer> middle;
    int n_before_attn = 0, pos_res = 0, pos_ch = 0, final_ch = 0;
    int suf_blk = -2, suf_layer = -1;
    int p_posenc = -1, p_te0w, p_te0b, p_te2w, p_te2b, p_outgw, p_outgb, p_outw, p_outb;
    size_t film_w_off = 0, film_b_off = 0, te_w_off = 0, te_b_off = 0;
    int film_total = 0, te_total = 0;
    size_t packed_total = 0;
    float* wbuf = nullptr;
    bool wbuf_on_host = false;
    int put(void* dst, const void* src, size_t bytes) {
        if (wbuf_on_host) { std::memcpy(dst, src, bytes); return 0; }
        VD_HIP(hipMemcpy(dst, src, bytes, hipMemcpyHostToDevice));
        return 0;
    }
    struct RpeGroup { int C; std::vector<int> blocks; long long* d_hid = nullptr; long long* d_out = nullptr; };
    std::vector<RpeGroup> rpe_groups;
    std::vector<float*> rpe_R;
    int rpe_all(const float* te, const int64_t* fidx, int B, int T, hipStream_t st, Arena& ar);
    int rpe_tables();
    void rpe_group_blocks();
    float* d_freq_time = nullptr; int n_freq_time = 0;
    float* d_freq_frame = nullptr; int n_freq_frame = 0;
    float* d_tab = nullptr; int num_timesteps = 0;
    float* d_tmap = nullptr; float rescale = 1.f;
    float* d_w2m = nullptr;
    float* d_jump = nullptr;
    char* ws = nullptr; size_t ws_cap = 0;
    bool ws_suf = false;
    int ws_B = 0, ws_T = 0; size_t ws_tail = 0;
    std::unordered_map<long long, size_t> ws_peaks;
    static size_t tm_bytes(int B) { return ((size_t)B * sizeof(float) + 255) & ~(size_t)255; }
    size_t out_floats(int B, int T) const { return (size_t)B * T * (cfg.learn_sigma ? 6 : 3) * cfg.image_size * cfg.image_size; }
    size_t guid_off(int B, int T) const { return (tm_bytes(B) + 2 * out_floats(B, T) * sizeof(float) + 255) & ~(size_t)255; }
    size_t step_tail_bytes(int B, int T) const { return guid_off(B, T) + guidance_scratch_bytes(B); }
    float* step_tm() const { return reinterpret_cast<float*>(ws + ws_tail); }
    float* step_eps(int B) const { return reinterpret_cast<float*>(ws + ws_tail + tm_bytes(B)); }
    float* step_eps_u(int B, int T) const { return step_eps(B) + out_floats(B, T); }
    void* step_guid(int B, int T) const { return ws + ws_tail + guid_off(B, T); }
    Arena step_arena() const { Arena a; a.base = ws; a.cap = ws_tail; return a; }
    float* wbuf_bwd = nullptr; bool wbuf_bwd_on_host = false; size_t packed_bwd_total = 0;
    Tape* tape = nullptr;
    std::vector<float*> attn_cap_t, attn_cap_s;
    int attn_seq = 0;
    float cfg_w = 1.f;
    float* d_cfg_zero = nullptr; size_t cfg_zero_cap = 0;
    float guid_phi = 0.f, dyn_p = 0.f;
    const float *known_src = nullptr, *known_mask = nullptr, *known_noise = nullptr;
    unsigned long long known_seed = 0, known_offset = 0;
    const float* meas_y = nullptr;
    int meas_scale = 1, meas_gray = 0;
    int mean_type = 0;
    int* d_err = nullptr;
    int device = -1;
    double* d_part = nullptr; size_t part_cap = 0;
    float* d_score_xt = nullptr; size_t score_xt_cap = 0;
    int* d_score_list = nullptr; size_t score_list_cap = 0;
    std::vector<float> score_mask_h; std::vector<int> score_list_h;
    struct WinKey {
        int B, T, obs_mode, sampler, clip, flags; float eta;
        float cfg_w;
        float guid_phi, dyn_p;
        float* x; const float *obs_src, *obs, *lat, *km; const long long* fidx;
        const float *known_src, *known_mask;
        const float* meas_y; int meas_scale, meas_gray;
        bool operator==(const WinKey& o) const { return std::memcmp(this, &o, sizeof(WinKey)) == 0; }
    };
    struct WinGraph {
        WinKey key; hipGraph_t graph = nullptr; hipGraphExec_t exec = nullptr;
        std::vector<unsigned char> inv; int n_inv = 0, n_suf = 0;
        int* d_lists = nullptr;
        PrefixStore* store = nullptr;
        void release() {
            if (exec) (void)hipGraphExecDestroy(exec);
            if (graph) (void)hipGraphDestroy(graph);
            if (d_lists) (void)hipFree(d_lists);
            if (store) { for (float* p : store->tens) if (p) (void)hipFree(p); for (double* p : store->parts) if (p) (void)hipFree(p); delete store; }
            exec = nullptr; graph = nullptr; d_lists = nullptr; store = nullptr;
        }
    };
    bool prefix_cache_on = false;
    bool suffix_skip_on = false;
    std::vector<WinGraph> win_graphs;
    int win_cur = -1;
    bool win_lost = false;
    unsigned long long win_gen = 0;
    long long win_left = 0;
    long long* d_win_t = nullptr; size_t win_t_cap = 0;
    float* d_win_xtm1 = nullptr; size_t win_xtm1_cap = 0;
    unsigned long long* d_win_rng = nullptr;
    float* d_win_hist = nullptr; size_t win_hist_cap = 0;

    ~vd_engine() {
        if (d_freq_time) (void)hipFree(d_freq_time);
        if (d_freq_frame) (void)hipFree(d_freq_frame);
        for (auto& g : rpe_groups) { if (g.d_hid) (void)hipFree(g.d_hid); if (g.d_out) (void)hipFree(g.d_out); }
        if (d_tab) (void)hipFree(d_tab);
        if (d_tmap) (void)hipFree(d_tmap);
        if (ws) (void)hipFree(ws);
        if (d_err) (void)hipFree(d_err);
        if (d_part) (void)hipFree(d_part);
        if (d_score_xt) (void)hipFree(d_score_xt);
// ... 445 lines not shown
            g.out = h; g.ldo = r.cout; g.Cout = r.cout; g.stats = ht.part; g.stats_split = ht.split;
            g.ksplit_ws = ksw; g.ksplit_ws_floats = ksf;
            if (!cfg.use_scale_shift_norm) { g.fbias = film; g.fbias_ld = film_total; }
            VD_REQUIRE(!za1 || act_conv_will_dispatch(g), "res_block: in_layers conv was planned on conv_wino_z128's activating form (no activation image "
                                                          "written) but the call as built is not one it takes");
            if ((rc = igemm_p(g, st))) return rc;
        }
        ar.release(mk);
    }
    if ((!fold || za2 || ar.dry) && (rc = gn_fold(ht, nullptr, N, r.gn2w, r.gn2b, cfg.use_scale_shift_norm ? film : nullptr, film_total, st, ar, &A2, &B2, &mr2)))
        return rc;
    const float* skip = x0.p;
    if (fuse_skip) skip = sk_early;
    else if (r.skw >= 0) {
        float* sk = ar.get<float>((size_t)N * HW * r.cout);
        if (!ar.dry) {
            IgemmArgs g = conv_args(x0, x1, N, 1, 1, 0);
            set_w(g, r.skw); g.bias = W(r.skb); g.out = sk; g.ldo = r.cout; g.Cout = r.cout;
            if ((rc = igemm_p(g, st))) return rc;
        }
        skip = sk;
    } else {
        VD_REQUIRE(x1 == nullptr, "identity skip over a concatenated input");
    }
    float* o = ar.get<float>((size_t)N * HW * r.cout);
    {
        const size_t mk = ar.mark();
        float* a2 = ar.get<float>((size_t)N * HW * r.cout);
        const size_t ksf = ksplit_scratch(ar, N, H, r.cout, r.cout);
        float* ksw = ksf ? ar.get<float>(ksf) : nullptr;
        if (fold && !za2 && (rc = gn_act(ht, nullptr, N, r.gn2w, r.gn2b, cfg.use_scale_shift_norm ? film : nullptr, film_total, 1, a2, st, ar))) return rc;
        if (!ar.dry) {
            if (!fold && !za2 && (rc = affine_act(h, nullptr, r.cout, r.cout, A2, B2, N, HW, a2, st))) return rc;
            Tens at{a2, r.cout, H};
            IgemmArgs g = conv_args(za2 ? ht : at, nullptr, N, 3, 1, 0);
            if (za2) { g.affA = A2; g.affB = B2; g.act = 1; }
            set_w(g, r.c2w); g.bias = W(r.c2b);
            g.res = skip; g.res_ld = r.cout; g.out = o; g.ldo = r.cout; g.Cout = r.cout;
            g.stats = ot.part; g.stats_split = ot.split;
            g.ksplit_ws = ksw; g.ksplit_ws_floats = ksf;
            VD_REQUIRE(!za2 || act_conv_will_dispatch(g), "res_block: out_layers conv was planned on conv_wino_z128's activating form (no activation image "
                                                          "written) but the call as built is not one it takes");
            if ((rc = igemm_p(g, st))) return rc;
        }
        ar.release(mk);
    }
    ot.p = o;
    *out = ot;
    if (tape) {
        tape->ops.push_back(TapeOp{1, (int)tape->res.size()});
        tape->res.push_back(TapeRes{(int)(&r - res.data()), x0, x1 ? *x1 : Tens{}, x1 != nullptr, N, A1, B1, mr1, h, A2, B2, mr2, o});
    }
    return 0;
}

int vd_engine::attn_block(const AttnP& a, Tens x, int B, int T, const int64_t* fidx,
                          const float* amask, hipStream_t st, Arena& ar, Tens* out) {
    const int C = a.C, H = x.H, HW = H * H, N = B * T;
    const size_t tok = (size_t)N * HW;
    const float scale = 1.0f / sqrtf((float)(C / cfg.num_heads));
    int rc;
    float* xn = ar.get<float>(tok * C);
    float* qkv = ar.get<float>(tok * 3 * C);
    const RpeP* rp[3] = {&a.rq, &a.rk, &a.rv};
    const size_t rrows = (size_t)B * T * T;
    const int blk = (int)(&a - attn.data());
    VD_REQUIRE(!cfg.use_rpe_net || !rpe_R.empty(), "attn_block: rpe_all has not run");
    float* Rall = cfg.use_rpe_net ? rpe_R[3 * blk] : ar.get<float>(3 * rrows * C);
    float* R[3] = {Rall + rrows * C, Rall, Rall + 2 * rrows * C};
    float* o = ar.get<float>(tok * C);
    float* xt = ar.get<float>(tok * C);
    Tens xt_t{xt, C, H};
    gemm_stats_table(ar, (int)tok, C, C, &xt_t);
    if (!ar.dry) {
        { ProfScope ps(PC_GN_TEMPORAL, 0.0, 8.0 * tok * C, st);
          rc = launch_gn_temporal(x.p, W(a.tp.normw), W(a.tp.normb), B, T, HW, C, xn, st); }
        if (rc) return rc;
        if ((rc = linear(xn, (int)tok, C, 3 * C, W(a.tp.qkvw), W(a.tp.qkvb), 0, nullptr, qkv, st))) return rc;
        if (!cfg.use_rpe_net)
            for (int i = 0; i < 3; ++i)
                if ((rc = launch_rpe_table(W(rp[i]->table), fidx, B, T, C, cfg.rp_alpha, cfg.rp_beta, cfg.rp_gamma,
                                           Rall + i * rrows * C, st))) return rc;
        AttnTemporalArgs ta{qkv, R[0], R[1], R[2], amask, o, B, T, HW, C, cfg.num_heads,
                            cfg.allow_interactions_between_padding, scale};
        { const double Fd = C / cfg.num_heads;
          ProfScope ps(PC_ATTN_TEMPORAL, 10.0 * B * HW * cfg.num_heads * T * T * Fd, 16.0 * tok * C + 12.0 * rrows * C, st);
          rc = launch_attn_temporal(ta, st); }
        if (rc) return rc;
        if (!attn_cap_t.empty() && attn_seq < (int)attn_cap_t.size() && attn_cap_t[attn_seq] &&
            (rc = launch_attn_temporal_weights(ta, attn_cap_t[attn_seq], st))) return rc;
        if ((rc = linear(o, (int)tok, C, C, W(a.tp.projw), W(a.tp.projb), 0, xn, xt, st, &xt_t))) return rc;
    }
    float *A = nullptr, *Bf = nullptr, *mrs = nullptr;
    const bool fold = !tape;
    if (!fold && (rc = gn_fold(xt_t, nullptr, N, a.sp.normw, a.sp.normb, nullptr, 0, st, ar, &A, &Bf, &mrs))) return rc;
    float* xn2 = ar.get<float>(tok * C);
    float* qkv2 = ar.get<float>(tok * 3 * C);
    float* o2 = ar.get<float>(tok * C);
    float* xs = ar.get<float>(tok * C);
    Tens xs_t{xs, C, H};
    gemm_stats_table(ar, (int)tok, C, C, &xs_t);
    if (fold && (rc = gn_act(xt_t, nullptr, N, a.sp.normw, a.sp.normb, nullptr, 0, 0, xn2, st, ar))) return rc;
    if (!ar.dry) {
        if (!fold) { ProfScope ps(PC_ELEMENTWISE, 0.0, 8.0 * tok * C, st); rc = launch_affine_apply(xt, A, Bf, N, HW, C, xn2, st); }
        if (rc) return rc;
        if ((rc = linear(xn2, (int)tok, C, 3 * C, W(a.sp.qkvw), W(a.sp.qkvb), 0, nullptr, qkv2, st))) return rc;
        AttnSpatialArgs sa{qkv2, o2, N, HW, C, cfg.num_heads, scale};
        { ProfScope ps(PC_ATTN_SPATIAL, 4.0 * N * (double)HW * HW * C, 16.0 * tok * C, st); rc = launch_attn_spatial(sa, st); }
        if (rc) return rc;
        if (!attn_cap_s.empty() && attn_seq < (int)attn_cap_s.size() && attn_cap_s[attn_seq] &&
            (rc = launch_attn_spatial_weights(sa, attn_cap_s[attn_seq], st))) return rc;
        if ((rc = linear(o2, (int)tok, C, C, W(a.sp.projw), W(a.sp.projb), 0, xn2, xs, st, &xs_t))) return rc;
    }
    *out = xs_t;
    if (!ar.dry) ++attn_seq;
    if (tape) {
        tape->ops.push_back(TapeOp{2, (int)tape->attn.size()});
        tape->attn.push_back(TapeAttn{(int)(&a - attn.data()), x, B, T, xn, qkv, R[0], R[1], R[2], o, xt, A, Bf, mrs, xn2, qkv2, o2, xs, amask});
    }
    return 0;
}

void vd_engine::rpe_group_blocks() {
    if (!rpe_groups.empty()) return;
    for (size_t b = 0; b < attn.size(); ++b) {
        size_t gi = 0;
        while (gi < rpe_groups.size() && rpe_groups[gi].C != attn[b].C) ++gi;
        if (gi == rpe_groups.size()) rpe_groups.push_back(RpeGroup{attn[b].C, {}});
        rpe_groups[gi].blocks.push_back((int)b);
    }
}

int vd_engine::rpe_tables() {
    if (!cfg.use_rpe_net || attn.empty() || !te_total) return 0;
    rpe_group_blocks();
    for (auto& g : rpe_groups) {
        if (g.d_hid) continue;
        const int nn = 3 * (int)g.blocks.size();
        std::vector<long long> th(3 * nn), to(2 * nn);
        for (size_t i = 0; i < g.blocks.size(); ++i) {
            const AttnP& a = attn[g.blocks[i]];
            const RpeP* rp[3] = {&a.rq, &a.rk, &a.rv};
            for (int k = 0; k < 3; ++k) {
                const int z = 3 * (int)i + k;
                th[3 * z] = rp[k]->te_off; th[3 * z + 1] = (long long)params[rp[k]->dw].off; th[3 * z + 2] = (long long)params[rp[k]->db].off;
                to[2 * z] = (long long)params[rp[k]->ow].off; to[2 * z + 1] = (long long)params[rp[k]->ob].off;
            }
        }
        VD_HIP(hipMalloc(reinterpret_cast<void**>(&g.d_hid), th.size() * sizeof(long long)));
        VD_HIP(hipMalloc(reinterpret_cast<void**>(&g.d_out), to.size() * sizeof(long long)));
        VD_HIP(hipMemcpy(g.d_hid, th.data(), th.size() * sizeof(long long), hipMemcpyHostToDevice));
        VD_HIP(hipMemcpy(g.d_out, to.data(), to.size() * sizeof(long long), hipMemcpyHostToDevice));
    }
    return 0;
}

int vd_engine::rpe_all(const float* te, const int64_t* fidx, int B, int T, hipStream_t st, Arena& ar) {
    rpe_R.clear();
    if (!cfg.use_rpe_net || attn.empty() || !te_total) return 0;
    rpe_group_blocks();
    const size_t rrows = (size_t)B * T * T;
    rpe_R.assign(3 * attn.size(), nullptr);
    int rc = 0;
    for (auto& g : rpe_groups) {
        const int nn = 3 * (int)g.blocks.size(), C = g.C;
        float* Rg = ar.get<float>((size_t)nn * rrows * C);
        for (size_t i = 0; i < g.blocks.size(); ++i)
            for (int k = 0; k < 3; ++k) rpe_R[3 * g.blocks[i] + k] = Rg + (3 * i + k) * rrows * C;
        const size_t mk = ar.mark();
        float* Eh = ar.get<float>((size_t)nn * rrows * C);
        ar.release(mk);
        if (ar.dry) continue;
        VD_REQUIRE(g.d_hid && g.d_out, "rpe_all: offset tables missing (ensure_ws builds them)");
        if ((rc = launch_rpe_hidden_tab(te, te_total, wbuf, g.d_hid, fidx, B, T, C, Eh, nn, rrows * C, st))) return rc;
        IgemmArgs q = linear_args((int)rrows, C, C);
        q.src0 = Eh; q.out = Rg;
        q.wfrag = wbuf + params[attn[g.blocks[0]].rq.ow].off; q.bias = wbuf + params[attn[g.blocks[0]].rq.ob].off;
        q.zcount = nn; q.zs_a = q.zs_out = (int)(rrows * C); q.ztab = g.d_out; q.zbase = wbuf;
        if ((rc = igemm_p(q, st))) return rc;
    }
    return 0;
}

int vd_engine::forward(const FwdIn& in, hipStream_t st, Arena& ar, const PrefixPlan* pp, const SuffixPlan* sp) {
    const int B = in.B, T = in.T, N = B * T, S = cfg.image_size, mc = cfg.num_channels;
    int rc;
    VD_REQUIRE(!pp || (!tape && !ar.dry && pp->store && n_before_attn > 0), "prefix plan: executor steps only");
    VD_REQUIRE(!sp || (!tape && sp->n > 0 && sp->n <= N && (ar.dry || sp->list)), "suffix plan: executor steps only, at least one frame");
    struct SelGuard { ~SelGuard() { g_sel_nfr = 0; } } sel_guard;
    const int Npre = pp ? pp->n : N;
    float* x8 = ar.get<float>((size_t)Npre * S * S * STEM_KPAD);
    float* tfr = ar.get<float>(N);
    float* amask = ar.get<float>(N);
    float* tsin = ar.get<float>((size_t)N * mc);
    float* e1 = ar.get<float>((size_t)N * E);
    float* emb = ar.get<float>((size_t)N * E);
    float* film = ar.get<float>((size_t)N * film_total);
    float* te = te_total ? ar.get<float>((size_t)N * te_total) : nullptr;
    float* ftv = cfg.use_frame_encoding ? ar.get<float>(N) : nullptr;
    float* femb = cfg.use_frame_encoding ? ar.get<float>((size_t)N * pos_ch) : nullptr;
    if (!ar.dry) {
        VD_REQUIRE(d_freq_time && n_freq_time == mc / 2, "vd_set_freqs not called (time frequencies)");
        AssembleArgs aa{in.x, in.obs_src, in.obs, in.lat, in.km, in.t_model, in.obs_mode, B, T, S, S, STEM_KPAD, cfg.cond_emb_type, x8, tfr, amask};
        if (pp) {
            AssembleArgs sc = aa; sc.scalars_only = 1;
            if ((rc = launch_assemble(sc, st))) return rc;
            aa.frame_list = pp->list; aa.n_list = pp->n;
        }
        if ((rc = launch_assemble(aa, st))) return rc;
        if ((rc = launch_sinus_embed(tfr, N, mc, d_freq_time, tsin, st))) return rc;
        if ((rc = linear(tsin, N, mc, E, W(p_te0w), W(p_te0b), 0, nullptr, e1, st))) return rc;
        if ((rc = linear(e1, N, E, E, W(p_te2w), W(p_te2b), 1, nullptr, emb, st))) return rc;
        if ((rc = linear(emb, N, E, film_total, wbuf + film_w_off, wbuf + film_b_off, 1, nullptr, film, st))) return rc;
        if (te_total && (rc = linear(emb, N, E, te_total, wbuf + te_w_off, wbuf + te_b_off, 0, nullptr, te, st))) return rc;
        if (cfg.use_frame_encoding) {
            VD_REQUIRE(d_freq_frame && n_freq_frame == pos_ch / 2, "vd_set_freqs not called (frame frequencies)");
            if ((rc = launch_frame_t(in.fidx, B, T, cfg.enforce_position_invariance, ftv, st))) return rc;
            if ((rc = launch_sinus_embed(ftv, N, pos_ch, d_freq_frame, femb, st))) return rc;
        }
    }
    rpe_R.clear();
    if (!(pp && pp->build_only) && (rc = rpe_all(te, in.fidx, B, T, st, ar))) return rc;
    attn_seq = 0;
    std::vector<Tens> hs;
    Tens h{x8, STEM_KPAD, S};
    int Nrun = Npre;
    const float* film_full = film;
    if (pp || ar.dry) {
        float* fc = ar.get<float>((size_t)std::max(pp ? Npre : N, 1) * film_total);
        if (pp) {
            if ((rc = launch_gather_rows(film_full, pp->list, Npre, film_total, fc, st))) return rc;
            film = fc;
        }
    }
    auto run = [&](const std::vector<Layer>& blk, Tens in0, const Tens* in1, Tens* outp, size_t l0 = 0, size_t l1 = ~(size_t)0) -> int {
        const int N = Nrun;
        Tens cur = in0;
        const Tens* second = in1;
        for (size_t li = l0; li < std::min(l1, blk.size()); ++li) {
            const Layer& L = blk[li];
            Tens nxt{};
            if (L.type == 1) {
                if ((rc = res_block(res[L.idx], cur, second, N, film, st, ar, &nxt))) return rc;
            } else if (L.type == 2) {
                if ((rc = attn_block(attn[L.idx], cur, B, T, in.fidx, amask, st, ar, &nxt))) return rc;
            } else if (L.type == 0) {
                const ConvP& c = convs[L.idx];
                float* o = ar.get<float>((size_t)N * S * S * c.c);
                nxt = Tens{o, c.c, S};
                gemm_stats_table(ar, N * S * S, STEM_KPAD, c.c, &nxt);
                if (!ar.dry && (rc = linear(cur.p, N * S * S, STEM_KPAD, c.c, W(c.w), W(c.b), 0, nullptr, o, st, &nxt))) return rc;
                if (tape) { tape->ops.push_back(TapeOp{0, (int)tape->conv.size()}); tape->conv.push_back(TapeConv{0, L.idx, cur, nxt}); }
            } else {
                const ConvP& c = convs[L.idx];
                const int stride = L.type == 3 ? 2 : 1, ups = L.type == 4 ? 1 : 0;
                IgemmArgs g = conv_args(cur, nullptr, N, 3, stride, ups);
                float* o = ar.get<float>((size_t)g.M * c.c);
                nxt = Tens{o, c.c, g.Ho};
                const bool phase = params[c.w].kind == PK_CONV3WU;
                if (params[c.w].kind == PK_CONV3W) nxt.part = stats_table(ar, N, g.Ho, c.c, &nxt.split);
                else if (phase) { nxt.split = conv_wino_ups_stats_split(cur.H); nxt.part = ar.get<double>((size_t)N * nxt.split * c.c * 2); }
                else if (stride == 2) conv_split_stats_table(ar, g, c.c, &nxt);
                const size_t mk = ar.mark();
                const size_t ksf = stride == 1 && !phase ? ksplit_scratch(ar, N, g.Ho, cur.C, c.c) : 0;
                float* ksw = ksf ? ar.get<float>(ksf) : nullptr;
                ar.release(mk);
                if (!ar.dry) {
                    g.ksplit_ws = ksw; g.ksplit_ws_floats = ksf;
                    set_w(g, c.w); g.bias = W(c.b); g.out = o; g.ldo = c.c; g.Cout = c.c;
                    g.stats = nxt.part; g.stats_split = nxt.split;
                    if (nxt.part && params[c.w].kind != PK_CONV3W && !phase) g.stats_hw = g.Ho * g.Wo;
                    if ((rc = igemm_p(g, st))) return rc;
                }
                if (tape) { tape->ops.push_back(TapeOp{0, (int)tape->conv.size()}); tape->conv.push_back(TapeConv{L.type, L.idx, cur, nxt}); }
            }
            cur = nxt;
            second = nullptr;
            VD_REQUIRE(!ar.overflow, "workspace overflow: the forward asked for more than the dry run measured (this step's output is invalid)");
        }
        *outp = cur;
        return 0;
    };
    for (size_t i = 0; i < input_blocks.size(); ++i) {
        if (pp && (int)i < n_before_attn) {
            Tens hc{};
            if (Npre > 0 && (rc = run(input_blocks[i], h, nullptr, &hc))) return rc;
            PrefixStore& ps = *pp->store;
            if (ps.tens.size() <= i) { ps.tens.resize(i + 1, nullptr); ps.parts.resize(i + 1, nullptr); ps.floats.resize(i + 1, 0); }
            if (Npre == 0) { VD_REQUIRE(ps.tens[i], "prefix cache: no tensor to reuse"); }
            else {
                const size_t per = (size_t)hc.H * hc.H * hc.C;
                if (!ps.tens[i]) {
                    VD_REQUIRE(pp->build_only, "prefix cache: the window's first pass allocates");
                    VD_HIP(hipMalloc(reinterpret_cast<void**>(&ps.tens[i]), (size_t)N * per * sizeof(float)));
                    ps.floats[i] = per | ((size_t)hc.C << 40) | ((size_t)hc.H << 52);
                    if (hc.part) VD_HIP(hipMalloc(reinterpret_cast<void**>(&ps.parts[i]), (size_t)N * hc.C * 2 * sizeof(double)));
                }
                VD_REQUIRE((ps.parts[i] != nullptr) == (hc.part != nullptr), "prefix cache: statistics table");
                if ((rc = launch_scatter_rows(hc.p, pp->list, Npre, per, ps.tens[i], st))) return rc;
                if (hc.part && (rc = launch_scatter_stats(hc.part, hc.split, hc.C, pp->list, Npre, ps.parts[i], st))) return rc;
            }
            const int Cc = (int)((ps.floats[i] >> 40) & 0xfff), Hc = (int)(ps.floats[i] >> 52);
            Tens full{ps.tens[i], Cc, Hc, ps.parts[i], ps.parts[i] ? 1 : 0};
            if ((int)i + 1 == n_before_attn) {
                if (pp->build_only) return 0;
// ... 962 lines not shown
    if (sampler_has_history(k.sampler)) {
        r.hist = r.xstart = e->d_win_hist;
        r.hist_on = e->d_win_rng + 2;
    }
    if (pre_on) r.pp = &plan;
    if (suf_on) r.sp = &splan;
    r.cfg_w = k.cfg_w; r.guid_phi = k.guid_phi; r.dyn_p = k.dyn_p;
    r.known_src = k.known_src; r.known_mask = k.known_mask;
    r.meas_y = k.meas_y; r.meas_scale = k.meas_scale; r.meas_gray = k.meas_gray;
    if (!rc) rc = step_launches(e, r, st);
    if (!rc) {
        hipLaunchKernelGGL(win_advance_kernel, dim3((B + 63) / 64), dim3(64), 0, st, e->d_win_t, e->d_win_rng, B,
                           sampler_walks_up(k.sampler) ? 1LL : -1LL, sampler_draws_noise(k.sampler) || k.known_src ? (unsigned long long)B * per : 0ULL);
        if (hipGetLastError() != hipSuccess) { set_error("win_advance_kernel launch"); rc = -2; }
    }
    const hipError_t ce = hipStreamEndCapture(st, &wg.graph);
    if (rc) return rc;
    if (ce != hipSuccess) { set_error(std::string("hipStreamEndCapture: ") + hipGetErrorString(ce)); return -2; }
    hipGraphExec_t exec = nullptr;
    if (hipGraphInstantiate(&exec, wg.graph, nullptr, nullptr, 0) != hipSuccess) { set_error("hipGraphInstantiate"); return -2; }
    wg.exec = exec;
    if (wg.store) {
        int cnt = 0, oldest = -1;
        for (size_t i = 0; i < e->win_graphs.size(); ++i) if (e->win_graphs[i].store) { ++cnt; if (oldest < 0) oldest = (int)i; }
        if (cnt >= 4) {
            (void)hipDeviceSynchronize();
            e->win_graphs[oldest].release();
            e->win_graphs.erase(e->win_graphs.begin() + oldest);
        }
    }
    e->win_graphs.push_back(wg);
    owner.g = nullptr;
    e->win_cur = (int)e->win_graphs.size() - 1;
    return 0;
}

int vd_window_begin(vd_engine* e, int B, int T, float* x, const float* obs_src, const float* obs, const float* lat,
                    const float* km, const long long* fidx, int obs_mode, int sampler, int clip, float eta,
                    unsigned long long seed, unsigned long long offset, long long t_start, void* stream) {
    int rc = check_sampler(e, B, T, obs_mode, 3, "observed_frames must be x_0 / x_t / x_t_minus_1 (2: re-noised per step, 3: the caller's tensor as it is)");
    if (rc) return rc;
    VD_REQUIRE(x && obs_src && obs && lat && km && fidx, "null tensor");
    VD_REQUIRE(sampler_valid(sampler), "sampler: 0 p_sample, 1 ddim_sample, 2 ddim_reverse_sample, 3 dpmpp_2m_sample");
    VD_REQUIRE(sampler_draws_noise(sampler) || obs_mode != 2, "sampler " + std::to_string(sampler) + " (" + sampler_name(sampler) + ") draws no noise: observed_frames = 2 "
               "re-noises the observed frames to t - 1 inside the graph and is not served; hand x_t_minus_1 as it is (observed_frames = 3)");
    VD_REQUIRE(!sampler_has_history(sampler) || e->d_w2m, "sampler 3 (dpmpp_2m_sample): no multistep weight row for the bound schedule (vd_set_multistep_weights, after vd_set_schedule)");
    VD_REQUIRE(t_start >= 0 && t_start < e->num_timesteps, "t_start outside the schedule");
    if ((rc = refuse_cut_step(e->cfg_w, e->dyn_p != 0.f && clip, e->prefix_cache_on, e->suffix_skip_on))) return rc;
    if (e->known_src) {
        VD_REQUIRE(!sampler_walks_up(sampler), "sampler 2 (ddim_reverse_sample) together with a known region (vd_set_known_region) is not served: the merge noises to t - 1");
        VD_REQUIRE(!e->known_noise, "a window draws the known region's noise from its own Philox stream: known_noise must be NULL (vd_set_known_region)");
        VD_REQUIRE(!e->prefix_cache_on, "a known region (vd_set_known_region) together with the window prefix cache (vd_set_window_prefix_cache) is not served");
        VD_REQUIRE(!e->suffix_skip_on, "a known region (vd_set_known_region) together with the window suffix skip (vd_set_window_suffix_skip) is not served");
    }
    if (e->meas_y) {
        if ((rc = refuse_with_measurement(e, sampler))) return rc;
        VD_REQUIRE(!e->prefix_cache_on, "a measurement (vd_set_measurement) together with the window prefix cache (vd_set_window_prefix_cache) is not served");
        VD_REQUIRE(!e->suffix_skip_on, "a measurement (vd_set_measurement) together with the window suffix skip (vd_set_window_suffix_skip) is not served");
    }
    hipStream_t st = static_cast<hipStream_t>(stream);
    VD_REQUIRE(st != nullptr, "the window executor captures a hipGraph: it needs a non-default stream");
    if ((rc = step_workspace(e, B, T, st))) return rc;
    if ((rc = window_buffers(e, B, obs_mode, sampler, (size_t)T * 3 * e->cfg.image_size * e->cfg.image_size))) return rc;
    hipLaunchKernelGGL(win_set_kernel, dim3((B + 63) / 64), dim3(64), 0, st, e->d_win_t, e->d_win_rng, B, t_start, seed, offset);
    VD_HIP(hipGetLastError());
    vd_engine::WinKey key;
    std::memset(&key, 0, sizeof(key));
    key.B = B; key.T = T; key.obs_mode = obs_mode; key.sampler = sampler; key.clip = clip; key.eta = eta; key.cfg_w = e->cfg_w;
    key.guid_phi = e->guid_phi; key.dyn_p = e->dyn_p;
    key.x = x; key.obs_src = obs_src; key.obs = obs; key.lat = lat; key.km = km; key.fidx = fidx;
    key.known_src = e->known_src; key.known_mask = e->known_mask;
    if (e->meas_y) { key.meas_y = e->meas_y; key.meas_scale = e->meas_scale; key.meas_gray = e->meas_gray; }
    e->win_cur = -1;
    e->win_lost = false;
    ++e->win_gen;
    e->win_left = sampler_walks_up(sampler) ? e->num_timesteps - t_start : t_start + 1;
    const int N = B * T;
    const bool use_pre = e->prefix_cache_on && obs_mode == 0 && e->cfg.cond_emb_type == 0 && e->n_before_attn > 0;
    const bool want_suf = e->suffix_skip_on && obs_mode != 1 && e->cfg.cond_emb_type == 0 && e->suf_blk >= -1 && !e->attn.empty();
    std::vector<unsigned char> inv;
    int n_inv = 0;
    if ((use_pre || want_suf) && (rc = invariant_frames(obs, lat, N, st, &inv, &n_inv))) return rc;
    const bool pre_on = use_pre && n_inv > 0, suf_on = want_suf && n_inv > 0 && n_inv < N;
    key.flags = (pre_on ? 1 : 0) | (suf_on ? 2 : 0);
    const int hit = find_window_graph(e, key, inv);
    if (hit >= 0) {
        e->win_cur = hit;
        return pre_on ? prefix_build_pass(e, key, e->win_graphs[hit], st) : 0;
    }
    const float* net_obs_src = obs_mode == 2 ? e->d_win_xtm1 : obs_src;
    const int net_mode = obs_mode == 3 ? 2 : obs_mode;
    if ((rc = warmup_forward(e, key, net_obs_src, net_mode, st))) return rc;
    return capture_window(e, key, inv, n_inv, net_obs_src, net_mode, st);
}

int vd_set_window_prefix_cache(vd_engine* e, int on) {
    VD_REQUIRE(e, "null engine");
    e->prefix_cache_on = on != 0;
    return 0;
}

int vd_set_cfg_scale(vd_engine* e, float w) {
    VD_REQUIRE(e, "null engine");
    VD_REQUIRE(w == w && std::fabs(w) <= 3.4028234e38f, "cfg_scale must be finite");
    e->cfg_w = w;
    return 0;
}

float vd_cfg_scale(vd_engine* e) { return e ? e->cfg_w : 1.f; }

int vd_op_cfg_combine(const float* out_c, const float* out_u, float w, long long n, float* out, void* stream) {
    return launch_cfg_combine(out_c, out_u, w, n, out, static_cast<hipStream_t>(stream));
}

int vd_set_guidance_rescale(vd_engine* e, float phi) {
    VD_REQUIRE(e, "null engine");
    VD_REQUIRE(phi >= 0.f && phi <= 1.f, "guidance_rescale must lie in [0, 1]");
    e->guid_phi = phi;
    return 0;
}

float vd_guidance_rescale(vd_engine* e) { return e ? e->guid_phi : 0.f; }

int vd_set_dynamic_threshold(vd_engine* e, float p) {
    VD_REQUIRE(e, "null engine");
    VD_REQUIRE(p >= 0.f && p <= 1.f, "dynamic_threshold must lie in (0, 1], or be 0 (off)");
    e->dyn_p = p;
    return 0;
}

float vd_dynamic_threshold(vd_engine* e) { return e ? e->dyn_p : 0.f; }

int vd_op_cfg_rescale(const float* out_c, const float* out_u, float w, const float* lat, int B, int T, long long frame_elems, float phi,
                      float* out, float* factor_out, void* stream) {
    VD_REQUIRE(B > 0 && frame_elems > 0, "vd_op_cfg_rescale: shape");
    OpScratch ws(stream);
    char* buf = nullptr;
    int rc = ws.get(&buf, guidance_scratch_bytes(B));
    return rc ? rc : launch_cfg_rescale(out_c, out_u, w, lat, B, T, (long)frame_elems, phi, out, factor_out, buf, ws.st);
}

int vd_op_dynamic_threshold(const float* x0, const float* lat, int B, int T, long long frame_elems, float p, float* out, float* s_out,
                            void* stream) {
    VD_REQUIRE(B > 0 && frame_elems > 0, "vd_op_dynamic_threshold: shape");
    OpScratch ws(stream);
    char* buf = nullptr;
    int rc = ws.get(&buf, guidance_scratch_bytes(B));
    if (rc) return rc;
    DynThreshArgs da{x0, nullptr, nullptr, nullptr, 0, lat, B, T, (long)frame_elems, p, out, s_out, nullptr, buf};
    return launch_dynamic_threshold(da, ws.st);
}

int vd_window_prefix_frames(vd_engine* e) {
    VD_REQUIRE(e, "null engine");
    return e->win_cur >= 0 && e->win_graphs[e->win_cur].store ? e->win_graphs[e->win_cur].n_inv : 0;
}

int vd_set_window_suffix_skip(vd_engine* e, int on) {
    VD_REQUIRE(e, "null engine");
    e->suffix_skip_on = on != 0;
    return 0;
}

int vd_window_suffix_frames(vd_engine* e) {
    VD_REQUIRE(e, "null engine");
    return e->win_cur >= 0 ? e->win_graphs[e->win_cur].n_suf : 0;
}
// ... 318 lines not shown

int vd_op_conv_wino_split(const float* src0, int Cin, int nfr, int Hs, int Ws, int ups, const void* w_split, const float* bias,
                          const float* res, const float* fbias, int fbias_ld, float* out, int Cout, double* gn_part,
                          void* stream) {
    IgemmArgs g = conv_args(src0, nullptr, Cin, Cin, nfr, Hs, Ws, ups, 1, 1, 3);
    g.wwino = static_cast<const float*>(w_split); g.wsplit = 2; g.bias = bias; g.res = res; g.res_ld = Cout;
    g.fbias = fbias; g.fbias_ld = fbias_ld; g.out = out; g.ldo = Cout; g.Cout = Cout;
    g.stats = gn_part; g.stats_split = conv_wino_stats_split(g.Ho);
    VD_REQUIRE(conv_wino_r64_supported(g), "vd_op_conv_wino_split: shape not covered by conv_wino_r64.hip");
    return launch_igemm(g, static_cast<hipStream_t>(stream));
}

int vd_op_conv_wino_act(const float* src0, const float* src1, int C0, int Cin, int nfr, int Hs, int Ws, const void* w_split, const float* bias,
                        const float* affA, const float* affB, const float* res, float* out, int Cout, double* gn_part, void* stream) {
    VD_REQUIRE(src0 && (src1 ? C0 > 0 && C0 < Cin : C0 == Cin), "vd_op_conv_wino_act: one source of Cin channels, or two of C0 and Cin - C0");
    IgemmArgs g = conv_args(src0, src1, C0, Cin, nfr, Hs, Ws, 0, 1, 1, 3);
    g.wwino = static_cast<const float*>(w_split); g.wsplit = 2; g.bias = bias; g.res = res; g.res_ld = Cout;
    g.affA = affA; g.affB = affB; g.act = 1;
    g.out = out; g.ldo = Cout; g.Cout = Cout;
    g.stats = gn_part; g.stats_split = conv_wino_stats_split(g.Ho);
    VD_REQUIRE(conv_wino_z128_act_supported(g), "vd_op_conv_wino_act: shape not covered by conv_wino_z128.hip's activating form (vd_conv_wino_act_ok)");
    return launch_igemm(g, static_cast<hipStream_t>(stream));
}

int vd_conv_wino_act_ok(int nfr, int H, int Cin, int Cout) { return f16_math() && conv_wino_z128_act_shape(nfr, H, Cin, Cout) ? 1 : 0; }

int vd_pack_conv3_wino_ups(const float* host_oihw, unsigned short* host_out, int O, int I) {
    VD_REQUIRE(host_oihw && host_out && O % 64 == 0 && I % 32 == 0, "vd_pack_conv3_wino_ups: O multiple of 64, I of 32");
    pack_conv3_wino_ups(host_oihw, host_out, O, I);
    return 0;
}

int vd_conv_ups_stats_split(int Hs) { return conv_wino_ups_stats_split(Hs); }

int vd_op_conv_wino_ups(const float* src0, int Cin, int nfr, int Hs, const void* w_ups, const float* bias, float* out, int Cout,
                        double* gn_part, void* stream) {
    IgemmArgs g = conv_args(src0, nullptr, Cin, Cin, nfr, Hs, Hs, 1, 1, 1, 3);
    g.ups_phase = 1;
    g.wwino = static_cast<const float*>(w_ups); g.wsplit = 2; g.bias = bias; g.out = out; g.ldo = Cout; g.Cout = Cout;
    g.stats = gn_part; g.stats_split = conv_wino_ups_stats_split(Hs);
    VD_REQUIRE(conv_wino_r64_supported(g), "vd_op_conv_wino_ups: shape not covered (square power-of-two source map >= 8, Cout % 64, Cin % 32)");
    return launch_igemm(g, static_cast<hipStream_t>(stream));
}

int vd_pack_conv3_split(const float* host_oihw, unsigned short* host_out, int O, int I) {
    VD_REQUIRE(host_oihw && host_out && O % 32 == 0 && I % 32 == 0, "vd_pack_conv3_split: O, I multiples of 32");
    pack_conv3_split(host_oihw, host_out, O, I);
    return 0;
}

int vd_op_conv_split(const float* src0, int Cin, int nfr, int Hs, int Ws, int stride, const void* w_split, const float* bias,
                     const float* res, float* out, int Cout, void* stream) {
    IgemmArgs g = conv_args(src0, nullptr, Cin, Cin, nfr, Hs, Ws, 0, stride, 1, 3);
    g.wfrag = static_cast<const float*>(w_split); g.wsplit = 1; g.bias = bias; g.res = res; g.res_ld = Cout;
    g.out = out; g.ldo = Cout; g.Cout = Cout;
    VD_REQUIRE(conv_split_supported(g), "vd_op_conv_split: shape not covered by the kernel");
    return launch_igemm(g, static_cast<hipStream_t>(stream));
}

int vd_pack_linear_split(const float* host_w, unsigned short* host_out, int N, int K) {
    VD_REQUIRE(host_w && host_out && N % 32 == 0 && K % 32 == 0, "vd_pack_linear_split: N, K multiples of 32");
    pack_linear_split(host_w, host_out, N, K, N, 0);
    return 0;
}

int vd_op_linear_split(const float* a, int M, int K, const void* w_split, const float* bias, const float* res, int act,
                       float* out, int N, void* stream) {
    IgemmArgs g = linear_args(M, K, N);
    g.src0 = a; g.wfrag = static_cast<const float*>(w_split); g.wsplit = 1; g.bias = bias; g.act = act; g.res = res; g.out = out;
    return launch_igemm(g, static_cast<hipStream_t>(stream));
}

int vd_op_linear_split_stats(const float* a, int M, int K, const void* w_split, const float* bias, const float* res, int act,
                             float* out, int N, int HW, double* gn_part, void* stream) {
    IgemmArgs g = linear_args(M, K, N);
    g.src0 = a; g.wfrag = static_cast<const float*>(w_split); g.wsplit = 1; g.bias = bias; g.act = act; g.res = res; g.out = out;
    VD_REQUIRE(gn_part && HW > 0 && gemm_split_supported(g), "vd_op_linear_split_stats: shape not covered by gemm_split.hip");
    g.stats = gn_part; g.stats_hw = HW; g.stats_split = HW / gemm_split_stats_rows(M, N);
    return launch_igemm(g, static_cast<hipStream_t>(stream));
}

int vd_linear_stats_split(int M, int N, int HW) { return HW / gemm_split_stats_rows(M, N); }

int vd_pack_conv3_wino(const float* host_oihw, float* host_out, int O, int I) {
    VD_REQUIRE(host_oihw && host_out && O % 64 == 0 && I % 16 == 0, "O multiple of 64, I multiple of 16");
    pack_conv3_wino(host_oihw, host_out, O, I);
    return 0;
}

int vd_pack_linear_frag(const float* host_w, float* host_out, int N, int K) {
    VD_REQUIRE(host_w && host_out && N % 32 == 0 && K % 32 == 0, "N and K multiples of 32");
    pack_linear_frag(host_w, host_out, N, K, N, 0);
    return 0;
}

int vd_profile_begin(void) {
    for (auto& r : g_prof.recs) { (void)hipEventDestroy(r.a); (void)hipEventDestroy(r.b); }
    g_prof.recs.clear();
    g_prof.on = true;
    return 0;
}

int vd_profile_end(double* out, int cap) {
    g_prof.on = false;
    VD_REQUIRE(out && cap >= 4 * PC_COUNT, "output needs 4*vd_profile_classes() doubles");
    for (int i = 0; i < 4 * PC_COUNT; ++i) out[i] = 0.0;
    for (auto& r : g_prof.recs) {
        VD_HIP(hipEventSynchronize(r.b));
        float ms = 0.f;
        VD_HIP(hipEventElapsedTime(&ms, r.a, r.b));
        out[r.cls * 4 + 0] += 1.0; out[r.cls * 4 + 1] += ms; out[r.cls * 4 + 2] += r.flops; out[r.cls * 4 + 3] += r.bytes;
        if (getenv("VD_PROF_DUMP"))
            fprintf(stderr, "[vd_prof] %-28s %-40s %8.1f us %7.1f TFLOP/s\n", prof_name(r.cls), r.tag, ms * 1e3,
                    ms > 0 ? r.flops / ms / 1e9 : 0.0);
        (void)hipEventDestroy(r.a); (void)hipEventDestroy(r.b);
    }
    g_prof.recs.clear();
    return 0;
}

int vd_profile_classes(void) { return PC_COUNT; }
const char* vd_profile_class_name(int i) { return prof_name(i); }

int vd_op_conv(const float* src0, const float* src1, int C0, int Cin, int nfr, int Hs, int Ws, int ups, int stride,
               int pad, int ksz, const float* w, const float* w_frag, const float* w_wino, const float* bias, const float* affA,
               const float* affB, int act,
               const float* res, const float* fbias, int fbias_ld, float* out, int Cout, void* stream) {
    IgemmArgs g = conv_args(src0, src1, C0, Cin, nfr, Hs, Ws, ups, stride, pad, ksz);
    g.w = w; g.wfrag = w_frag; g.wwino = w_wino; g.bias = bias; g.affA = affA; g.affB = affB; g.act = act; g.res = res; g.res_ld = Cout;
    g.fbias = fbias; g.fbias_ld = fbias_ld; g.out = out; g.ldo = Cout; g.Cout = Cout;
    return launch_igemm(g, static_cast<hipStream_t>(stream));
}

int vd_conv_stats_split(int Hout) { return conv_wino_stats_split(Hout); }
int vd_conv_wino_block_couts(int nfr, int H, int Cin, int Cout) { return conv_wino_z128_shape(nfr, H, Cin, Cout) ? 128 : 64; }

int vd_op_conv_stats(const float* src0, int Cin, int nfr, int Hs, int Ws, int ups, const float* w_wino, const float* bias,
                     const float* res, const float* fbias, int fbias_ld, float* out, int Cout, double* gn_part,
                     void* stream) {
    IgemmArgs g = conv_args(src0, nullptr, Cin, Cin, nfr, Hs, Ws, ups, 1, 1, 3);
    g.wwino = w_wino; g.bias = bias; g.res = res; g.res_ld = Cout; g.fbias = fbias; g.fbias_ld = fbias_ld;
    g.out = out; g.ldo = Cout; g.Cout = Cout;
    g.stats = gn_part; g.stats_split = conv_wino_stats_split(g.Ho);
    VD_REQUIRE(conv_wino_supported(g), "vd_op_conv_stats: shape not covered by the Winograd kernel");
    return launch_igemm(g, static_cast<hipStream_t>(stream));
}

int vd_op_gn_affine(const double* part0, int split0, int C0, const double* part1, int split1, int C, int nfr, int HW,
                    const float* gamma, const float* beta, const float* film, int film_ld, float* affA, float* affB,
                    void* stream) {
    return launch_gn_affine(part0, split0, C0, part1, split1, (double)HW * (C / 32), gamma, beta, film, film_ld, nfr, C, affA,
                            affB, static_cast<hipStream_t>(stream));
}

int vd_op_gn_fold(const float* src0, const float* src1, int C0, int C, int nfr, int HW, const float* gamma,
                  const float* beta, const float* film, int film_ld, float* affA, float* affB, void* stream) {
    OpScratch ws(stream);
    const int split = gn_stats_split(nfr, HW, C);
    double* part;
    int rc = ws.get(&part, (size_t)nfr * split * C * 2);
    if (!rc) rc = launch_gn_stats(src0, src1, C0, C, nfr, HW, part, split, ws.st);
    if (!rc) rc = launch_gn_affine(part, split, C, nullptr, 0, (double)HW * (C / 32), gamma, beta, film, film_ld, nfr, C, affA, affB, ws.st);
    return rc;
}

int vd_op_affine_act(const float* src0, const float* src1, int C0, int C, const float* affA, const float* affB, int nfr,
// ... 145 lines not shown
```

video-diffusion_amd/csrc/gemm_frag.hip:

```cpp
#include "vd_common.h"

namespace vd {

constexpr int GLD = 36;

#ifdef VD_GEMM_TIMING
__device__ unsigned long long g_gemm_stamp[6];
#define GEMM_STAMP(i) do { if (threadIdx.x == 0 && blockIdx.x == gridDim.x / 2 && blockIdx.y == 0) {                  \
        g_gemm_stamp[i] = __builtin_readcyclecounter();                                                             \
        if (i == 0) g_gemm_stamp[4] = __builtin_amdgcn_s_memrealtime();                                             \
        if (i == 3) g_gemm_stamp[5] = __builtin_amdgcn_s_memrealtime(); } } while (0)
extern "C" int vd_debug_gemm_stamps(unsigned long long* host_out) {
    return (int)hipMemcpyFromSymbol(host_out, HIP_SYMBOL(g_gemm_stamp), sizeof(g_gemm_stamp));
}
#else
#define GEMM_STAMP(i)
#endif

template <int BM, int BN, bool ACT>
__global__ __launch_bounds__(256, 3) void gemm_frag_kernel(IgemmArgs a) {
    constexpr int MI = BM / 64, NI = BN / 64, AR = BM / 32;
    extern __shared__ __attribute__((aligned(16))) float smem[];
    const int tid = threadIdx.x, lane = tid & 63, wave = __builtin_amdgcn_readfirstlane(tid >> 6);
    const int wm = wave >> 1, wn = wave & 1;
    const int lr = lane & 31, lh = lane >> 5;
    const int m0 = blockIdx.x * BM, n0 = blockIdx.y * BN;
    const int lrow = tid >> 3, lq = tid & 7;
    const int nchunk = a.Cin >> 5, ncoblk = a.Cout >> 5;
    const int C1 = a.Cin - a.C0;
    GEMM_STAMP(0);
    if (a.zcount > 1) {
        const int z = blockIdx.z;
        a.src0 += (size_t)z * a.zs_a; a.out += (size_t)z * a.zs_out;
        a.wfrag = a.zbase + a.ztab[2 * z];
        a.bias = a.zbase + a.ztab[2 * z + 1];
    }

    const auto asrc0 = __builtin_amdgcn_make_buffer_rsrc(const_cast<float*>(a.src0), 0, a.M * a.C0 * 4, 0x00020000);
    const auto asrc1 = __builtin_amdgcn_make_buffer_rsrc(const_cast<float*>(a.src1 ? a.src1 : a.src0), 0,
                                                         a.src1 ? a.M * C1 * 4 : 0, 0x00020000);
    unsigned ao0[AR], ao1[AR];
#pragma unroll
    for (int j = 0; j < AR; ++j) {
        const unsigned row = (unsigned)min(m0 + lrow + 32 * j, a.M - 1);
        ao0[j] = row * (unsigned)(a.C0 * 4) + lq * 16u;
        ao1[j] = row * (unsigned)(C1 * 4) + lq * 16u;
    }
    const auto bsrc = __builtin_amdgcn_make_buffer_rsrc(const_cast<float*>(a.wfrag), 0, a.Cin * a.Cout * 4, 0x00020000);
    unsigned bo[NI];
#pragma unroll
    for (int j = 0; j < NI; ++j) bo[j] = (unsigned)min((int)blockIdx.y * (BN / 32) + wn * NI + j, ncoblk - 1) * 4096u + lane * 16u;

    f32x4 ra[AR], bfr[4][NI], afr[2][MI];
    auto a_prefetch = [&](int chunk) {
        const int c = chunk * 32;
        if (c < a.C0) {
#pragma unroll
            for (int j = 0; j < AR; ++j)
                ra[j] = __builtin_bit_cast(f32x4, __builtin_amdgcn_raw_buffer_load_b128(asrc0, ao0[j], c * 4, 0));
        } else {
#pragma unroll
            for (int j = 0; j < AR; ++j)
                ra[j] = __builtin_bit_cast(f32x4, __builtin_amdgcn_raw_buffer_load_b128(asrc1, ao1[j], (c - a.C0) * 4, 0));
        }
    };
    auto a_store = [&](float* Ad) {
#pragma unroll
        for (int j = 0; j < AR; ++j) {
            f32x4 v = ra[j];
            if constexpr (ACT) { v.x = silu_f(v.x); v.y = silu_f(v.y); v.z = silu_f(v.z); v.w = silu_f(v.w); }
            *reinterpret_cast<f32x4*>(Ad + (lrow + 32 * j) * GLD + lq * 4) = v;
        }
    };
    auto b_load = [&](int slot, int chunk, int kg) {
        const int so = chunk * ncoblk * 4096 + kg * 1024;
#pragma unroll
        for (int j = 0; j < NI; ++j) bfr[slot][j] = __builtin_bit_cast(f32x4, __builtin_amdgcn_raw_buffer_load_b128(bsrc, bo[j], so, 0));
    };

    const auto osrc = __builtin_amdgcn_make_buffer_rsrc(a.out, 0, a.M * a.ldo * 4, 0x00020000);
    const auto rsrc = __builtin_amdgcn_make_buffer_rsrc(const_cast<float*>(a.res ? a.res : a.out), 0,
                                                        a.res ? a.M * a.ldo * 4 : 0, 0x00020000);
    unsigned vb[MI][NI];
    float bv[NI];
#pragma unroll
    for (int j = 0; j < NI; ++j) {
        const int co = n0 + wn * (BN / 2) + j * 32 + lr;
        bv[j] = a.bias && co < a.Cout ? a.bias[co] : 0.f;
#pragma unroll
        for (int i = 0; i < MI; ++i)
            vb[i][j] = co < a.Cout ? (unsigned)((m0 + wm * (BM / 2) + i * 32 + 4 * lh) * a.ldo + co) * 4u : 0x80000000u;
    }
    f32x16 acc[MI][NI];
#pragma unroll
    for (int i = 0; i < MI; ++i)
#pragma unroll
        for (int j = 0; j < NI; ++j)
#pragma unroll
            for (int r = 0; r < 16; ++r) {
                const int srow = ((r & 3) + 8 * (r >> 2)) * a.ldo * 4;
                acc[i][j][r] = bv[j] + __builtin_bit_cast(float, __builtin_amdgcn_raw_buffer_load_b32(rsrc, vb[i][j] + srow, 0, 0));
            }

    a_prefetch(0);
    b_load(0, 0, 0);
    b_load(1, 0, 1);
    a_store(smem);
    __syncthreads();

    const int aoff = (wm * (BM / 2) + lr) * GLD + lh * 4;
    GEMM_STAMP(1);
    for (int chunk = 0; chunk < nchunk; ++chunk) {
        const int nxt = min(chunk + 1, nchunk - 1);
        const float* Acur = smem + (chunk & 1) * BM * GLD + aoff;
        float* Anext = smem + ((chunk + 1) & 1) * BM * GLD;
        a_prefetch(nxt);
#pragma unroll
        for (int i = 0; i < MI; ++i) afr[0][i] = *reinterpret_cast<const f32x4*>(Acur + i * 32 * GLD);
#pragma unroll
        for (int kg = 0; kg < 4; ++kg) {
            if (kg + 2 < 4) b_load(kg + 2, chunk, kg + 2);
            else b_load(kg - 2, nxt, kg - 2);
            if (kg + 1 < 4) {
#pragma unroll
                for (int i = 0; i < MI; ++i)
                    afr[(kg + 1) & 1][i] = *reinterpret_cast<const f32x4*>(Acur + i * 32 * GLD + (kg + 1) * 8);
            }
            __builtin_amdgcn_sched_barrier(0);
#pragma unroll
            for (int e = 0; e < 4; ++e)
#pragma unroll
                for (int i = 0; i < MI; ++i)
#pragma unroll
                    for (int j = 0; j < NI; ++j)
// ... 72 lines not shown
```

video-diffusion_amd/csrc/gemm_split.hip:

```cpp
#include <cstring>
#include <vector>

#include "vd_common.h"

namespace vd {

typedef __bf16 bf16x4 __attribute__((ext_vector_type(4)));
typedef __bf16 bf16x8 __attribute__((ext_vector_type(8)));
typedef unsigned u32x4 __attribute__((ext_vector_type(4)));
typedef unsigned u32x2 __attribute__((ext_vector_type(2)));

template <bool F16>
__device__ __forceinline__ f32x16 mfma_piece(u32x4 a, u32x4 b, f32x16 c) {
    if constexpr (F16) return __builtin_amdgcn_mfma_f32_32x32x16_f16(__builtin_bit_cast(f16x8, a), __builtin_bit_cast(f16x8, b), c, 0, 0, 0);
    else return __builtin_amdgcn_mfma_f32_32x32x16_bf16(__builtin_bit_cast(bf16x8, a), __builtin_bit_cast(bf16x8, b), c, 0, 0, 0);
}

#ifndef VD_GS_SKIP
#define VD_GS_SKIP 0
#endif
#ifdef VD_GS_TIMING
__device__ unsigned long long g_gs_stamp[8];
#define GS_STAMP(i) do { if (threadIdx.x == 0 && blockIdx.x == gridDim.x / 2 && blockIdx.y == 0) {                        \
        __builtin_amdgcn_sched_barrier(0); g_gs_stamp[i] = __builtin_amdgcn_s_memrealtime(); __builtin_amdgcn_sched_barrier(0); } } while (0)
extern "C" int vd_debug_gs_stamps(unsigned long long* host_out) { return (int)hipMemcpyFromSymbol(host_out, HIP_SYMBOL(g_gs_stamp), sizeof(g_gs_stamp)); }
#else
#define GS_STAMP(i)
#endif
constexpr int SROW = 80;

template <bool F16>
__device__ __forceinline__ void split3(f32x4 v, u32x2& p1, u32x2& p2, u32x2& p3) {
    if constexpr (F16) {
        p1.x = f16_pack(v.x, v.y); p1.y = f16_pack(v.z, v.w);
        p2.x = f16_pack_scaled(f16_rem_lo(p1.x, v.x), f16_rem_hi(p1.x, v.y));
        p2.y = f16_pack_scaled(f16_rem_lo(p1.y, v.z), f16_rem_hi(p1.y, v.w));
        p3 = p2;
    } else {
        const bf16x4 q1 = __builtin_convertvector(v, bf16x4);
        f32x4 r = v - __builtin_convertvector(q1, f32x4);
        const bf16x4 q2 = __builtin_convertvector(r, bf16x4);
        r = r - __builtin_convertvector(q2, f32x4);
        const bf16x4 q3 = __builtin_convertvector(r, bf16x4);
        p1 = __builtin_bit_cast(u32x2, q1); p2 = __builtin_bit_cast(u32x2, q2); p3 = __builtin_bit_cast(u32x2, q3);
    }
}

template <int BM, int BN, bool ACT, bool CONV, bool F16 = true, bool SIDE = false>
__global__ __launch_bounds__(256, 2) void gemm_split_kernel(IgemmArgs a) {
    constexpr int MI = BM / 64, NI = BN / 64, AR = BM / 32;
    constexpr bool B2R = F16;
    constexpr int RING = NI >= 3 ? 2 : (BM == 64 && BN == 64) ? 6 : 3;
    constexpr int BP = B2R ? 2 : 3;
    constexpr int PF = BM == 64 ? 3 : 1;
    constexpr int NPL = F16 ? 2 : 3;
    constexpr int PLANE = BM * SROW, ABUF = NPL * PLANE;
    extern __shared__ __attribute__((aligned(16))) char smem_c[];
    const int tid = threadIdx.x, lane = tid & 63, wave = __builtin_amdgcn_readfirstlane(tid >> 6);
    GS_STAMP(0);
    const int wm = wave >> 1, wn = wave & 1;
    const int lr = lane & 31, lh = lane >> 5;
    int bxi = blockIdx.x, byi = blockIdx.y;
    if (gridDim.y > 1 && (gridDim.x & 7) == 0 && gridDim.x >= 128) {
        const unsigned lin = blockIdx.x + gridDim.x * blockIdx.y, xcd = lin & 7, loc = lin >> 3;
        byi = loc % gridDim.y;
        bxi = (loc / gridDim.y) * 8 + xcd;
    }
    const int m0 = bxi * BM, n0 = byi * BN;
    const int lgrp = tid >> 3, lrow = ((lgrp >> 1) & 3) + 8 * (lgrp >> 3) + 4 * (lgrp & 1), lq = tid & 7;
    const int cpt = a.Cin >> 5;
    const int nchunk = CONV ? 9 * cpt : cpt, ncoblk = a.Cout >> 5;
    const int C1 = a.Cin - a.C0;
    if (a.zcount > 1) {
        const int z = blockIdx.z;
        a.src0 += (size_t)z * a.zs_a; a.out += (size_t)z * a.zs_out;
        a.wfrag = a.zbase + a.ztab[2 * z];
        a.bias = a.zbase + a.ztab[2 * z + 1];
    }

    const auto asrc0 = __builtin_amdgcn_make_buffer_rsrc(const_cast<float*>(a.src0), 0,
                                                         (CONV ? a.nfr * a.Hs * a.Ws : a.M) * a.C0 * 4, 0x00020000);
    const auto asrc1 = __builtin_amdgcn_make_buffer_rsrc(const_cast<float*>(a.src1 ? a.src1 : a.src0), 0,
                                                         a.src1 ? a.M * C1 * 4 : 0, 0x00020000);
    unsigned ao0[AR], ao1[AR];
    int iy0[AR], ix0[AR];
#pragma unroll
    for (int j = 0; j < AR; ++j) {
        const unsigned row = (unsigned)min(m0 + lrow + 32 * j, a.M - 1);
        if constexpr (CONV) {
            const unsigned ox = row % (unsigned)a.Wo, t = row / (unsigned)a.Wo;
            const unsigned oy = t % (unsigned)a.Ho, n = t / (unsigned)a.Ho;
            iy0[j] = (int)oy * a.stride - 1;
            ix0[j] = (int)ox * a.stride - 1;
            ao0[j] = (unsigned)(((int)n * a.Hs + iy0[j]) * a.Ws + ix0[j]) * (unsigned)(a.Cin * 4) + lq * 16u;
            ao1[j] = 0;
        } else {
            ao0[j] = row * (unsigned)(a.C0 * 4) + lq * 16u;
            ao1[j] = row * (unsigned)(C1 * 4) + lq * 16u;
        }
    }
    const auto bsrc = __builtin_amdgcn_make_buffer_rsrc(const_cast<float*>(a.wfrag), 0, (CONV ? 9 : 1) * a.Cin * a.Cout * 6, 0x00020000);
    unsigned bo[NI];
#pragma unroll
    for (int j = 0; j < NI; ++j) bo[j] = (unsigned)min(byi * (BN / 32) + wn * NI + j, ncoblk - 1) * 3072u + lane * 16u;

    f32x4 ra[PF][AR];
    u32x4 bfr[RING][NI][BP], b2[NI], afr[2][MI][NPL];
    static_assert(!SIDE || (BM == 128 && !CONV && !ACT), "side output: 128-row tiles of a plain 1x1");
    const bool side_on = SIDE && byi == 0;
    const float* sAp = SIDE ? a.sideA + (size_t)(m0 / (SIDE ? a.side_hw : 1)) * a.Cin + lq * 4 : nullptr;
    const float* sBp = SIDE ? a.sideB + (size_t)(m0 / (SIDE ? a.side_hw : 1)) * a.Cin + lq * 4 : nullptr;
    f32x4 sA = {0.f, 0.f, 0.f, 0.f}, sB = sA;
    auto side_affine = [&](int chunk) {
        if constexpr (SIDE) {
            if (side_on) { sA = *reinterpret_cast<const f32x4*>(sAp + chunk * 32); sB = *reinterpret_cast<const f32x4*>(sBp + chunk * 32); }
        }
    };
    auto side_store = [&](f32x4 v, int chunk, int j) {
        if constexpr (SIDE) {
            const int row = m0 + lrow + 32 * j;
            if (side_on && row < a.M) {
                f32x4 r = v * sA + sB;
                r.x = silu_f(r.x); r.y = silu_f(r.y); r.z = silu_f(r.z); r.w = silu_f(r.w);
                *reinterpret_cast<f32x4*>(a.side + (size_t)row * a.Cin + chunk * 32 + lq * 4) = r;
            }
        }
    };
    auto a_prefetch = [&](int chunk, int rs) {
        if constexpr (CONV) {
            const int tap = chunk / cpt, c = (chunk - tap * cpt) * 32;
            const int kh = tap / 3, kw = tap - 3 * kh;
            const unsigned shift = (unsigned)((kh * a.Ws + kw) * a.Cin * 4);
#pragma unroll
            for (int j = 0; j < AR; ++j) {
                const bool ok = (unsigned)(iy0[j] + kh) < (unsigned)a.Hs && (unsigned)(ix0[j] + kw) < (unsigned)a.Ws;
                ra[rs][j] = __builtin_bit_cast(f32x4, __builtin_amdgcn_raw_buffer_load_b128(asrc0, ok ? ao0[j] + shift : 0x80000000u, c * 4, 0));
            }
            return;
        }
        const int c = chunk * 32;
        if (c < a.C0) {
#pragma unroll
            for (int j = 0; j < AR; ++j)
                ra[rs][j] = __builtin_bit_cast(f32x4, __builtin_amdgcn_raw_buffer_load_b128(asrc0, ao0[j], c * 4, 0));
        } else {
#pragma unroll
            for (int j = 0; j < AR; ++j)
                ra[rs][j] = __builtin_bit_cast(f32x4, __builtin_amdgcn_raw_buffer_load_b128(asrc1, ao1[j], (c - a.C0) * 4, 0));
        }
    };
    auto a_store = [&](char* Ad, int rs) {
#pragma unroll
        for (int j = 0; j < AR; ++j) {
            f32x4 v = ra[rs][j];
            side_store(v, 0, j);
            if constexpr (ACT) { v.x = silu_f(v.x); v.y = silu_f(v.y); v.z = silu_f(v.z); v.w = silu_f(v.w); }
            u32x2 p1, p2, p3;
// ... 303 lines not shown
```

video-diffusion_amd/csrc/misc.hip:

```cpp
#include <algorithm>

#include "vd_common.h"

namespace vd {

__global__ __launch_bounds__(256) void assemble_kernel(AssembleArgs a) {
    const int n = a.frame_list ? a.frame_list[blockIdx.y] : blockIdx.y;
    const int HW = a.H * a.W;
    const float om = a.obs_mask[n], lm = a.lat_mask[n], km = a.km_mask[n];
    const float any = fminf(om + lm + km, 1.0f);
    const int Cs = a.cond_mode == 0 ? 5 : (a.cond_mode == 1 ? 6 : 3);
    if (blockIdx.x == 0 && threadIdx.x == 0 && !a.frame_list) {
        const float t = a.t_model[n / a.T];
        const float tobs = a.obs_t_mode == 0 ? 0.f : (a.obs_t_mode == 1 ? t : t - 1.f);
        float tf = t;
        if (a.cond_mode == 0) tf = tobs * om + t * (1.f - om);
        else if (a.cond_mode == 2) {
            bool any_obs = false;
            for (int k = 0; k < a.T; ++k) any_obs |= a.obs_mask[(n / a.T) * a.T + k] == 1.f;
            if (any_obs) tf = -1.f;
        }
        a.t_frames[n] = tf;
        a.amask[n] = any;
    }
// ... 50 lines not shown
    VD_HIP(hipGetLastError());
    return 0;
}

template <bool SCATTER>
__global__ __launch_bounds__(256) void move_rows_kernel(const float* __restrict__ src, const int* __restrict__ list, size_t row4,
                                                        float* __restrict__ dst) {
    const int i = blockIdx.y, f = list[i];
    const f32x4* s4 = reinterpret_cast<const f32x4*>(src) + (size_t)(SCATTER ? i : f) * row4;
    f32x4* d4 = reinterpret_cast<f32x4*>(dst) + (size_t)(SCATTER ? f : i) * row4;
    for (size_t k = (size_t)blockIdx.x * 256 + threadIdx.x; k < row4; k += (size_t)gridDim.x * 256) d4[k] = s4[k];
}

static int move_rows(bool scatter, const float* src, const int* list, int n, size_t row_floats, float* dst, hipStream_t s) {
    VD_REQUIRE(row_floats % 4 == 0, "frame rows in 16-byte units");
    if (n == 0) return 0;
    const size_t row4 = row_floats / 4;
    const int bx = (int)std::min<size_t>((row4 + 1023) / 1024, 64);
    if (scatter) hipLaunchKernelGGL(move_rows_kernel<true>, dim3(bx, n), dim3(256), 0, s, src, list, row4, dst);
    else hipLaunchKernelGGL(move_rows_kernel<false>, dim3(bx, n), dim3(256), 0, s, src, list, row4, dst);
    VD_HIP(hipGetLastError());
    return 0;
}
int launch_gather_rows(const float* src, const int* list, int n, size_t row_floats, float* dst, hipStream_t s) {
    return move_rows(false, src, list, n, row_floats, dst, s);
}
int launch_scatter_rows(const float* src, const int* list, int n, size_t row_floats, float* dst, hipStream_t s) {
    return move_rows(true, src, list, n, row_floats, dst, s);
}

__global__ void scatter_stats_kernel(const double* __restrict__ src, int split, int C, const int* __restrict__ list,
                                     double* __restrict__ dst) {
    const int i = blockIdx.x, f = list[i];
    for (int k = threadIdx.x; k < 2 * C; k += blockDim.x) {
        double v = 0;
        for (int sp = 0; sp < split; ++sp) v += src[((size_t)i * split + sp) * 2 * C + k];
        dst[(size_t)f * 2 * C + k] = v;
    }
}
int launch_scatter_stats(const double* src, int split, int C, const int* list, int n, double* dst, hipStream_t s) {
    if (n == 0) return 0;
    hipLaunchKernelGGL(scatter_stats_kernel, dim3(n), dim3(256), 0, s, src, split, C, list, dst);
    VD_HIP(hipGetLastError());
    return 0;
}

__global__ void sinus_kernel(const float* __restrict__ t, const float* __restrict__ freqs, int half, int dim,
                             float* __restrict__ out) {
    const int n = blockIdx.x;
    const float tv = t[n];
    for (int i = threadIdx.x; i < half; i += blockDim.x) {
        const float arg = tv * freqs[i];
        out[(size_t)n * dim + i] = cosf(arg);
        out[(size_t)n * dim + half + i] = sinf(arg);
    }
    if ((dim & 1) && threadIdx.x == 0) out[(size_t)n * dim + dim - 1] = 0.f;
}

int launch_sinus_embed(const float* t, int n, int dim, const float* freqs, float* out, hipStream_t s) {
    hipLaunchKernelGGL(sinus_kernel, dim3(n), dim3(64), 0, s, t, freqs, dim / 2, dim, out);
    VD_HIP(hipGetLastError());
    return 0;
}

__global__ void frame_t_kernel(const int64_t* __restrict__ fidx, int T, int center, float* __restrict__ tv) {
    const int b = blockIdx.x;
    float mean = 0.f;
    if (center) {
        float s = 0.f;
        for (int t = 0; t < T; ++t) s += (float)fidx[b * T + t];
        mean = s / (float)T;
    }
    for (int t = threadIdx.x; t < T; t += blockDim.x) tv[b * T + t] = (float)fidx[b * T + t] - mean;
}

int launch_frame_t(const int64_t* fidx, int B, int T, int center, float* tv, hipStream_t s) {
    hipLaunchKernelGGL(frame_t_kernel, dim3(B), dim3(64), 0, s, fidx, T, center, tv);
    VD_HIP(hipGetLastError());
    return 0;
}

__global__ __launch_bounds__(256) void rpe_hidden_tab_kernel(const float* __restrict__ te, int te_ld, const float* __restrict__ wbase,
                                                             const long long* __restrict__ tab, const int64_t* __restrict__ fidx, int T, int C,
                                                             float* __restrict__ E, size_t zs_e) {
    __shared__ float feat[64][3];
    const long long* tz = tab + 3 * blockIdx.y;
    te += tz[0];
    const float* Wd = wbase + tz[1];
    const float* bd = wbase + tz[2];
    E += blockIdx.y * zs_e;
    const int bt = blockIdx.x, b = bt / T;
    for (int s0 = 0; s0 < T; s0 += 64) {
        const int ns = min(64, T - s0);
        __syncthreads();
        if ((int)threadIdx.x < ns) {
            const float d = (float)(fidx[bt] - fidx[b * T + s0 + threadIdx.x]);
            feat[threadIdx.x][0] = logf(1.0f + fmaxf(d, 0.f));
            feat[threadIdx.x][1] = logf(1.0f + fmaxf(-d, 0.f));
            feat[threadIdx.x][2] = d == 0.f ? 1.f : 0.f;
        }
        __syncthreads();
        for (int c = threadIdx.x; c < C; c += 256) {
            const float bc = bd[c], w0 = Wd[c * 3], w1 = Wd[c * 3 + 1], w2 = Wd[c * 3 + 2], tv = te[(size_t)bt * te_ld + c];
            for (int k = 0; k < ns; ++k) {
                const float lin = bc + feat[k][0] * w0 + feat[k][1] * w1 + feat[k][2] * w2;
                E[((size_t)bt * T + s0 + k) * C + c] = silu_f(tv + lin);
            }
        }
    }
}

int launch_rpe_hidden_tab(const float* te, int te_ld, const float* wbase, const long long* tab, const int64_t* fidx, int B, int T, int C,
                          float* E, int nz, size_t zs_e, hipStream_t s) {
    hipLaunchKernelGGL(rpe_hidden_tab_kernel, dim3(B * T, nz), dim3(256), 0, s, te, te_ld, wbase, tab, fidx, T, C, E, zs_e);
    VD_HIP(hipGetLastError());
    return 0;
}

__global__ __launch_bounds__(256) void rpe_table_kernel(const float* __restrict__ table, const int64_t* __restrict__ fidx,
                                                        int T, int C, float alpha, float beta, float gamma, double lg,
                                                        float* __restrict__ R) {
    const int row = blockIdx.x;
    const int s_ = row % T, bt = row / T, b = bt / T;
    const long long d = fidx[bt] - fidx[b * T + s_];
    long long id = d;
    const float ad = fabsf((float)d);
    if (ad > alpha) {
        double v = (double)alpha + log((double)ad / (double)alpha) / lg * ((double)beta - (double)alpha);
        const double r = rint(v);
        if (fabs(v - r) < 1e-6) v = r;
        v = fmin((double)beta, v);
        id = (long long)(int)v * (d > 0 ? 1 : -1);
    }
    const int nb = 2 * (int)beta + 1;
    if (id < 0) id += nb;
    for (int c = threadIdx.x; c < C; c += 256) R[(size_t)row * C + c] = table[(size_t)id * C + c];
}

int launch_rpe_table(const float* table, const int64_t* fidx, int B, int T, int C, float alpha, float beta,
                     float gamma, float* R, hipStream_t s) {
    const double lg = log((double)gamma / (double)alpha);
    hipLaunchKernelGGL(rpe_table_kernel, dim3(B * T * T), dim3(256), 0, s, table, fidx, T, C, alpha, beta, gamma, lg, R);
    VD_HIP(hipGetLastError());
    return 0;
}

__global__ __launch_bounds__(256) void posenc_kernel(const float* __restrict__ x, const float* __restrict__ P,
                                                     const float* __restrict__ femb, size_t per_frame4, int C4,
                                                     size_t total4, float* __restrict__ y) {
    for (size_t i = (size_t)blockIdx.x * 256 + threadIdx.x; i < total4; i += (size_t)gridDim.x * 256) {
        f32x4 v = reinterpret_cast<const f32x4*>(x)[i];
        if (P) v += reinterpret_cast<const f32x4*>(P)[i % per_frame4];
        if (femb) v += reinterpret_cast<const f32x4*>(femb)[(i / per_frame4) * C4 + (i % C4)];
        reinterpret_cast<f32x4*>(y)[i] = v;
    }
}

int launch_posenc_add(const float* x, const float* P, const float* femb, int nfr, int HW, int C, float* y,
                      hipStream_t s) {
    const size_t total4 = (size_t)nfr * HW * C / 4;
    const int grid = (int)std::min<size_t>((total4 + 255) / 256, 4096);
    hipLaunchKernelGGL(posenc_kernel, dim3(grid), dim3(256), 0, s, x, P, femb, (size_t)HW * C / 4, C / 4, total4, y);
    VD_HIP(hipGetLastError());
    return 0;
}

constexpr int OT = 16;
template <int NCO>
__global__ __launch_bounds__(256) void out_conv_kernel(const float* __restrict__ x, const float* __restrict__ affA,
                                                       const float* __restrict__ affB, const float* __restrict__ w,
                                                       const float* __restrict__ bias, int H, int W, int C, int Cout,
                                                       float* __restrict__ out) {
    __shared__ __attribute__((aligned(16))) float tile[(OT + 2) * (OT + 2) * 36];
    __shared__ __attribute__((aligned(16))) float ws[9 * NCO * 32];
    const int n = blockIdx.z, y0 = blockIdx.y * OT, x0 = blockIdx.x * OT;
    const int tid = threadIdx.x, ty = tid / OT, tx = tid % OT;
    float acc[NCO];
#pragma unroll
    for (int co = 0; co < NCO; ++co) acc[co] = 0.f;
    for (int c0 = 0; c0 < C; c0 += 32) {
        __syncthreads();
        for (int i = tid; i < (OT + 2) * (OT + 2) * 8; i += 256) {
            const int pix = i >> 3, q = i & 7;
            const int iy = y0 + pix / (OT + 2) - 1, ix = x0 + pix % (OT + 2) - 1;
            f32x4 v = {0.f, 0.f, 0.f, 0.f};
            if (iy >= 0 && iy < H && ix >= 0 && ix < W) {
                v = *reinterpret_cast<const f32x4*>(x + (((size_t)n * H + iy) * W + ix) * C + c0 + q * 4);
                const f32x4 A = *reinterpret_cast<const f32x4*>(affA + (size_t)n * C + c0 + q * 4);
                const f32x4 B = *reinterpret_cast<const f32x4*>(affB + (size_t)n * C + c0 + q * 4);
                v = v * A + B;
                v.x = silu_f(v.x); v.y = silu_f(v.y); v.z = silu_f(v.z); v.w = silu_f(v.w);
            }
            *reinterpret_cast<f32x4*>(tile + pix * 36 + q * 4) = v;
        }
        for (int i = tid; i < 9 * NCO * 32; i += 256) {
            const int tap = i / (NCO * 32), co = (i / 32) % NCO, c = i % 32;
            ws[i] = co < Cout ? w[((size_t)tap * Cout + co) * C + c0 + c] : 0.f;
// ... 546 lines not shown
```

video-diffusion_amd/csrc/vd_common.h:

```cpp
#pragma once
#include <hip/hip_runtime.h>
#include <cstdint>
#include <cstdio>
#include <string>

typedef float f32x4 __attribute__((ext_vector_type(4)));
typedef float f32x16 __attribute__((ext_vector_type(16)));

namespace vd {

constexpr int kMaxWindowFrames = 128;
constexpr int kMaxGuidedWindowFrames = 32;

void set_error(const std::string& msg);
extern thread_local std::string g_last_error;

#define VD_HIP(call)                                                                   \
    do {                                                                               \
        hipError_t e_ = (call);                                                        \
        if (e_ != hipSuccess) {                                                        \
            vd::set_error(std::string(#call) + ": " + hipGetErrorString(e_));          \
            return -2;                                                                 \
        }                                                                              \
    } while (0)

#define VD_REQUIRE(cond, msg)                                                          \
    do {                                                                               \
        if (!(cond)) {                                                                 \
            vd::set_error(std::string("requirement failed: ") + #cond + " -- " + msg); \
            return -1;                                                                 \
        }                                                                              \
    } while (0)

struct LdsAttr { size_t have[64] = {}; };
inline int raise_dynamic_lds(LdsAttr& st, const void* fn, size_t bytes) {
    int dev = 0;
    VD_HIP(hipGetDevice(&dev));
    VD_REQUIRE(dev >= 0 && dev < 64, "device ordinal beyond the per-device attribute table");
    if (bytes > st.have[dev]) {
        VD_HIP(hipFuncSetAttribute(fn, hipFuncAttributeMaxDynamicSharedMemorySize, (int)bytes));
        st.have[dev] = bytes;
    }
    return 0;
}
#define VD_RAISE_LDS(fn, bytes)                                                                        \
    do {                                                                                               \
        static vd::LdsAttr lds_attr_;                                                                  \
        if (int rc_ = vd::raise_dynamic_lds(lds_attr_, reinterpret_cast<const void*>(fn), (bytes))) return rc_; \
    } while (0)

inline int upload_f32(float** dst, const float* host, size_t n) {
    if (!*dst) VD_HIP(hipMalloc(reinterpret_cast<void**>(dst), n * sizeof(float)));
    VD_HIP(hipMemcpy(*dst, host, n * sizeof(float), hipMemcpyHostToDevice));
    return 0;
}
template <class T>
inline int grow_ws(T** ws, size_t* have, size_t need) {
    if (*have >= need) return 0;
    VD_HIP(hipFree(*ws));
    *ws = nullptr; *have = 0;
    VD_HIP(hipMalloc(reinterpret_cast<void**>(ws), need * sizeof(T)));
    *have = need;
    return 0;
}
inline int require_device(int dev, const char* what) {
    int cur = -1;
    VD_HIP(hipGetDevice(&cur));
    VD_REQUIRE(cur == dev, std::string("the ") + what + " handle belongs to another device");
    return 0;
}

struct IgemmArgs {
    const float* src0;
    const float* src1;
    int C0, Cin;
    int nfr, Hs, Ws;
    int ups;
    int nfr_sel = 0;
    int ups_phase = 0;
    float* side = nullptr; const float* sideA = nullptr; const float* sideB = nullptr; int side_hw = 0;
    int stride, pad, ksz;
    int Ho, Wo;
    const float* w;
    const float* wfrag;
    const float* wwino;
    const float* bias;
    const float* affA;
    const float* affB;
    int act;
    const float* res;
    int res_ld;
    const float* fbias;
    int fbias_ld;
    float* out;
    int ldo;
    int Cout, M;
    double* stats;
    int stats_split;
    int stats_hw;
    int zcount, zs_a, zs_out;
    const long long* ztab = nullptr; const float* zbase = nullptr;
    int wsplit;
    float* ksplit_ws;
    size_t ksplit_ws_floats;
};

struct AttnSpatialArgs {
    const float* qkv;
    float* out;
    int nfr, L, C, heads;
    float scale;
};

struct AttnTemporalArgs {
    const float* qkv;
    const float* Rk;
    const float* Rq;
    const float* Rv;
    const float* mask;
    float* out;
    int B, T, HW, C, heads;
    int allow_pad;
    float scale;
};

enum ConvClGather {
    CG_QUAD,
    CG_ELEM,
    CG_NCHW_SCALED
};
struct ConvClArgs {
    const float* src;
    const float* w;
    const float* bias;
    float* out;
    long long out_stride;
    int T, H, W, Cin, Cout, kt, kh, kw, st, sh, sw, pt, ph, pw, To, Ho, Wo, relu;
    float shift[3], scale[3];
    int M, K, Kreal;
};
inline int conv_cl_kpad(int kreal) { return (kreal + 31) / 32 * 32; }
int launch_conv_cl(ConvClArgs a, ConvClGather g, hipStream_t s);
int launch_conv_cl_pack(const float* w, float* packed, int Cout, int Cin, int taps, hipStream_t s);
int conv_cl_load_weight(float** packed, const float* host, int Cout, int Cin, int taps);
struct PoolClArgs {
    const float* src;
    float* dst;
    int T, H, W, C, kt, kh, kw, st, sh, sw, pt, ph, pw, To, Ho, Wo;
};
int launch_maxpool_cl(const PoolClArgs& a, hipStream_t s);

int launch_igemm(const IgemmArgs& a, hipStream_t s);
int igemm_frames_per_launch(const IgemmArgs& a);
IgemmArgs igemm_first_launch(const IgemmArgs& a);
enum IgemmKernel { IK_R64_UPS, IK_SPLIT, IK_Z128, IK_R64, IK_FRAG, IK_WINO, IK_GENERIC };
IgemmKernel igemm_kernel(const IgemmArgs& a);
int igemm_tile_class(int M, int Cout);
bool gemm_frag_supported(const IgemmArgs& a);
int launch_gemm_frag(const IgemmArgs& a, int tile_class, hipStream_t s);
void pack_linear_frag(const float* w, float* out_base, int rows, int K, int n_total, int row0);
bool conv_wino_supported(const IgemmArgs& a);
inline int igemm_sel_M(const IgemmArgs& a) { return a.nfr_sel > a.nfr ? a.nfr_sel * a.Ho * a.Wo : a.M; }
int conv_wino_stats_split(int Hout);
__device__ __forceinline__ void split_a(float x0, float x1, unsigned& p1, float& r0, float& r1, unsigned) {
    float h0, h1;
    asm("v_cvt_pk_bf16_f32 %0, %5, %6\n\t"
        "v_lshlrev_b32 %3, 16, %0\n\t"
        "v_and_b32 %4, 0xffff0000, %0\n\t"
        "v_sub_f32 %1, %5, %3\n\t"
        "v_sub_f32 %2, %6, %4"
        : "=&v"(p1), "=&v"(r0), "=&v"(r1), "=&v"(h0), "=&v"(h1)
        : "v"(x0), "v"(x1));
}
__device__ __forceinline__ void split_b(float r0, float r1, unsigned& p2, unsigned& p3, unsigned) {
    float h0, h1;
    asm("v_cvt_pk_bf16_f32 %0, %4, %5\n\t"
        "v_lshlrev_b32 %2, 16, %0\n\t"
        "v_and_b32 %3, 0xffff0000, %0\n\t"
        "v_sub_f32 %2, %4, %2\n\t"
        "v_sub_f32 %3, %5, %3\n\t"
        "v_cvt_pk_bf16_f32 %1, %2, %3"
        : "=&v"(p2), "=&v"(p3), "=&v"(h0), "=&v"(h1)
        : "v"(r0), "v"(r1));
}

enum { MATH_F16X3 = 0, MATH_BF16X6 = 1, MATH_FP32 = 2 };
int math_mode();
inline bool f16_math() { return math_mode() == MATH_F16X3; }
typedef _Float16 f16x8 __attribute__((ext_vector_type(8)));
typedef _Float16 f16x4 __attribute__((ext_vector_type(4)));
__device__ __forceinline__ unsigned f16_pack(float x0, float x1) {
    unsigned p;
    asm("v_cvt_pk_f16_f32 %0, %1, %2" : "=v"(p) : "v"(x0), "v"(x1));
    return p;
}
__device__ __forceinline__ float f16_rem_lo(unsigned p0, float x0) {
    float r;
    asm("v_fma_mix_f32 %0, %1, -1.0, %2 op_sel_hi:[1,0,0]" : "=v"(r) : "v"(p0), "v"(x0));
    return r;
}
__device__ __forceinline__ float f16_rem_hi(unsigned p0, float x1) {
    float r;
    asm("v_fma_mix_f32 %0, %1, -1.0, %2 op_sel:[1,0,0] op_sel_hi:[1,0,0]" : "=v"(r) : "v"(p0), "v"(x1));
    return r;
}
__device__ __forceinline__ unsigned f16_pack_scaled(float r0, float r1) {
    float s0, s1;
// ... 6 lines not shown
size_t split_image_u16(size_t n_out, size_t k_total);
void pack_conv3_wino_split(const float* oihw, unsigned short* out, int O, int I);
bool conv_wino_r64_supported(const IgemmArgs& a);
int launch_conv_wino_r64(const IgemmArgs& a, hipStream_t s);
bool conv_wino_z128_supported(const IgemmArgs& a);
bool conv_wino_z128_shape(int nfr, int H, int Cin, int Cout);
int launch_conv_wino_z128(const IgemmArgs& a, hipStream_t s);
bool conv_wino_z128_act_shape(int nfr, int H, int Cin, int Cout);
bool conv_wino_z128_act_supported(const IgemmArgs& a);
void pack_conv3_wino_ups(const float* oihw, unsigned short* out, int O, int I);
int conv_wino_ups_stats_split(int Hs);
int conv_wino_r64_ksplit(int nfr, int Hl, int Cin, int Cout);
size_t conv_wino_r64_ksplit_floats(int nfr, int Hl, int Cin, int Cout, int nfr_sel = 0);
bool gemm_split_supported(const IgemmArgs& a);
bool gemm_split_side_supported(const IgemmArgs& a);
bool conv_split_supported(const IgemmArgs& a);
void pack_conv3_split(const float* w_oihw, unsigned short* out, int Cout, int Cin);
int launch_gemm_split(const IgemmArgs& a, int tile_class, hipStream_t s);
int gemm_split_tile_class(int M, int Cout);
int gemm_split_stats_rows(int M, int Cout);
void pack_linear_split(const float* w, unsigned short* out_base, int rows, int K, int n_total, int row0);
int launch_conv_wino(const IgemmArgs& a, hipStream_t s);
void pack_conv3_wino(const float* oihw, float* out, int O, int I);
int launch_attn_spatial(const AttnSpatialArgs& a, hipStream_t s);
struct AttnSpatialVariant {
    int row;
    int F, NW;
    bool f16;
    const char* why;
};
AttnSpatialVariant attn_spatial_variant(int L, int C, int heads);
std::string attn_spatial_variant_name(const AttnSpatialVariant& v);
int launch_attn_temporal(const AttnTemporalArgs& a, hipStream_t s);
struct AttnTemporalVariant {
    enum Family { kRefused = 0, kMfma, kValu, kLongMfma, kLongGeneric };
    Family family;
    int p0, p1;
    bool exact, rpe;
    size_t lds;
    const char* why;
};
AttnTemporalVariant attn_temporal_variant(int T, int HW, int C, int heads, bool rpe);
std::string attn_temporal_variant_name(const AttnTemporalVariant& v);
int launch_attn_temporal_long(const AttnTemporalArgs& a, hipStream_t s);

int launch_gn_stats(const float* src0, const float* src1, int C0, int C, int nfr, int HW, double* part, int split,
                    hipStream_t s);
int gn_stats_split(int nfr, int HW, int C);
int launch_gn_affine(const double* part0, int split0, int C0, const double* part1, int split1, double count,
                     const float* gamma, const float* beta, const float* film, int film_ld, int nfr, int C, float* affA,
                     float* affB, hipStream_t s, float* mr_out = nullptr);
struct GnFold { const double* part0; int split0; const double* part1; int split1; double count; const float* gamma; const float* beta;
                const float* film; int film_ld; };
int launch_affine_act_fold(const float* src0, const float* src1, int C0, int C, const GnFold& f, int nfr, int HW, int act, float* y,
                           hipStream_t s);
int launch_affine_act(const float* src0, const float* src1, int C0, int C, const float* affA, const float* affB, int nfr,
                      int HW, int act, float* y, hipStream_t s);
int launch_affine_apply(const float* x, const float* affA, const float* affB, int nfr, int HW, int C, float* y,
                        hipStream_t s);
int launch_gn_temporal(const float* x, const float* gamma, const float* beta, int B, int T, int HW, int C, float* y,
                       hipStream_t s);

struct AssembleArgs {
    const float* x;
    const float* obs_src;
    const float* obs_mask, *lat_mask, *km_mask;
    const float* t_model;
    int obs_t_mode;
    int B, T, H, W, Kpad;
    int cond_mode;
    float* x_cols;
    float* t_frames;
    float* amask;
    const int* frame_list = nullptr;
    int n_list = 0;
    int scalars_only = 0;
};
int launch_assemble(const AssembleArgs& a, hipStream_t s);
int launch_gather_rows(const float* src, const int* list, int n, size_t row_floats, float* dst, hipStream_t s);
int launch_scatter_rows(const float* src, const int* list, int n, size_t row_floats, float* dst, hipStream_t s);
int launch_scatter_stats(const double* src, int split, int C, const int* list, int n, double* dst, hipStream_t s);
int launch_sinus_embed(const float* t, int n, int dim, const float* freqs, float* out, hipStream_t s);
int launch_rpe_hidden_tab(const float* te, int te_ld, const float* wbase, const long long* tab, const int64_t* fidx, int B, int T, int C,
                          float* E, int nz, size_t zs_e, hipStream_t s);
int launch_rpe_table(const float* table, const int64_t* fidx, int B, int T, int C, float alpha, float beta,
                     float gamma, float* R, hipStream_t s);
int launch_posenc_add(const float* x, const float* P, const float* femb, int nfr, int HW, int C, float* y,
                      hipStream_t s);
int launch_frame_t(const int64_t* fidx, int B, int T, int center, float* tv, hipStream_t s);
int launch_out_conv(const float* x, const float* affA, const float* affB, const float* w, const float* bias, int nfr,
                    int H, int W, int C, int Cout, float* out_nchw, hipStream_t s);

bool head_gemm_supported(int HW, int C, int ldt);
int launch_head_gemm(const float* h, const float* affA, const float* affB, const float* Wt, int nfr, int HW, int C, int ldt, float* T, hipStream_t s);
int launch_out_gather(const float* T, const float* bias, int nfr, int H, int W, int ldt, int Cout, float* out_nchw, hipStream_t s);

enum Sampler { SAMPLER_P = 0, SAMPLER_DDIM = 1, SAMPLER_DDIM_REVERSE = 2, SAMPLER_DPMPP_2M = 3 };
inline bool sampler_valid(int s) { return s >= SAMPLER_P && s <= SAMPLER_DPMPP_2M; }
inline bool sampler_walks_up(int s) { return s == SAMPLER_DDIM_REVERSE; }
inline bool sampler_draws_noise(int s) { return s == SAMPLER_P || s == SAMPLER_DDIM; }
inline bool sampler_has_history(int s) { return s == SAMPLER_DPMPP_2M; }
inline const char* sampler_name(int s) {
    return s == SAMPLER_P ? "p_sample" : s == SAMPLER_DDIM ? "ddim_sample" : s == SAMPLER_DDIM_REVERSE ? "ddim_reverse_sample" : "dpmpp_2m_sample";
}
struct SamplerPassArgs {
    int sampler;
    const float* x;
    const float* eps;
    const float* x0_given;
    const int64_t* t;
    const float* tab;
    int num_timesteps;
    int B; long per;
    int clip;
    float* sample;
    float* xstart;
    int* err;
    float* mean = nullptr;
    float eta = 0.f;
    const float* noise = nullptr;
    unsigned long long seed = 0, offset = 0;
    const unsigned long long* dstate = nullptr;
    const float* hist = nullptr;
    const unsigned long long* hist_on = nullptr;
    const float* w = nullptr;
};
enum { VD_ERR_TIMESTEP = 1, VD_ERR_NONFINITE = 2 };
int launch_sampler_pass(const SamplerPassArgs& a, hipStream_t s);
int launch_cfg_combine(const float* out_c, const float* out_u, float w, long long n, float* out, hipStream_t s);
__device__ __forceinline__ float cfg_combine_one(float c, float u, float w) {
    const float d = c - u;
    if (!(fabsf(d) <= 3.4028234e38f)) return __builtin_nanf("");
    return w == 0.0f ? u : fmaf(w, d, u);
}
__device__ __forceinline__ float xstart_from_eps(float sr, float x, float srm1, float eps) {
#pragma clang fp contract(off)
    const float a = sr * x, b = srm1 * eps;
    return a - b;
}
__device__ __forceinline__ float pass_x0(float x, float src, bool given, float sr, float srm1, int clip, bool& nonfinite) {
    float x0 = given ? src : xstart_from_eps(sr, x, srm1, src);
    const bool bad = !(fabsf(x0) <= 3.4028234e38f);
    nonfinite |= bad;
    if (clip && !bad) x0 = fminf(fmaxf(x0, -1.0f), 1.0f);
    return x0;
}
size_t guidance_scratch_bytes(int B);
int launch_cfg_rescale(const float* out_c, const float* out_u, float w, const float* lat, int B, int T, long frame_elems, float phi,
                       float* out, float* factor_out, void* scratch, hipStream_t s);
struct DynThreshArgs {
    const float* src;
    const float* x;
    const int64_t* t;
    const float* tab;
    int num_timesteps;
    const float* lat;
    int B, T; long frame_elems;
    float p;
    float* out;
    float* s_out;
    int* err;
    void* scratch;
};
int launch_dynamic_threshold(const DynThreshArgs& a, hipStream_t s);
int launch_q_sample(const float* x0, const float* noise, const int64_t* t, const float* tab, int num_timesteps, int B,
                    long per, float* out, hipStream_t s);
int launch_randn(float* out, long n, unsigned long long seed, unsigned long long offset, hipStream_t s);
// ... 170 lines not shown
```

Baseline: 51.09.

## Deduplicate RPE table computation across batch items with identical timesteps and frames

A small device kernel compares each batch item's timestep bits and frame indices with earlier items and records a representative item for each. The RPE hidden-feature kernel and the batched RPE GEMMs exit early for row blocks that belong only to duplicate items, and their blocks are reordered so the redundant ones cluster together. The temporal attention forward and backward kernels then read the Rk/Rq/Rv tables of the representative item. This removes repeated RPE work when a batch contains identical conditioning, such as guidance pairs. The cost is an extra tiny launch and per-block checks over the item map, and the window-graph cache key now includes the dedup flag.

```diff
diff --git a/include/vd_amd.h b/include/vd_amd.h
--- a/include/vd_amd.h
+++ b/include/vd_amd.h
@@ -227,6 +227,10 @@
 int vd_op_linear_split_stats(const float* a, int M, int K, const void* w_split, const float* bias, const float* res, int act,
                              float* out, int N, int HW, double* gn_part, void* stream);
 int vd_linear_stats_split(int M, int N, int HW);
+int vd_set_rpe_dedup(vd_engine* e, int on);
+int vd_rpe_dedup(vd_engine* e);
+int vd_rpe_item_rep_host(const float* t_frames, const long long* frame_indices, int B, int T, int* rep);
+int vd_rpe_rows_redundant_host(const int* rep, int rows_per_item, int m0, int m1);
 int vd_op_gn_fold(const float* src0, const float* src1, int C0, int C, int nfr, int HW, const float* gamma,
                   const float* beta, const float* film, int film_ld, float* affA, float* affB, void* stream);
 int vd_op_affine_apply(const float* x, const float* affA, const float* affB, int nfr, int HW, int C, float* y,
diff --git a/video-diffusion_amd/_lib.py b/video-diffusion_amd/_lib.py
--- a/video-diffusion_amd/_lib.py
+++ b/video-diffusion_amd/_lib.py
@@ -220,6 +220,10 @@
     "vd_op_linear_split": (_I, [_P, _I, _I, _P, _P, _P, _I, _P, _I, _P]),
     "vd_op_linear_split_stats": (_I, [_P, _I, _I, _P, _P, _P, _I, _P, _I, _I, _P, _P]),
     "vd_linear_stats_split": (_I, [_I, _I, _I]),
+    "vd_set_rpe_dedup": (_I, [_P, _I]),
+    "vd_rpe_dedup": (_I, [_P]),
+    "vd_rpe_item_rep_host": (_I, [_P, _P, _I, _I, _P]),
+    "vd_rpe_rows_redundant_host": (_I, [_P, _I, _I, _I]),
     "vd_op_gn_fold": (_I, [_P, _P, _I, _I, _I, _I, _P, _P, _P, _I, _P, _P, _P]),
     "vd_op_affine_apply": (_I, [_P, _P, _P, _I, _I, _I, _P, _P]),
     "vd_op_affine_act": (_I, [_P, _P, _I, _I, _P, _P, _I, _I, _I, _P, _P]),
diff --git a/video-diffusion_amd/csrc/attn_temporal.hip b/video-diffusion_amd/csrc/attn_temporal.hip
--- a/video-diffusion_amd/csrc/attn_temporal.hip
+++ b/video-diffusion_amd/csrc/attn_temporal.hip
@@ -15,6 +15,7 @@
     float* ks = qs + PB * T * FP;
     float* sc = ks + PB * T * FP;
     const int b = blockIdx.z, h = blockIdx.y, p0 = blockIdx.x * PB;
+    const int rb = RPE && a.item_rep ? a.item_rep[b] : b;
     const int np = min(PB, HW - p0);
     const int tid = threadIdx.x;
     const float* qkv_b = a.qkv + (size_t)b * T * HW * C3 + h * F;
@@ -36,8 +37,8 @@
         float acc[PB];
 #pragma unroll
         for (int p = 0; p < PB; ++p) acc[p] = 0.f;
-        const float* rk = RPE ? a.Rk + (((size_t)b * T + t) * T + s) * C + h * F : nullptr;
-        const float* rq = RPE ? a.Rq + (((size_t)b * T + s) * T + t) * C + h * F : nullptr;
+        const float* rk = RPE ? a.Rk + (((size_t)rb * T + t) * T + s) * C + h * F : nullptr;
+        const float* rq = RPE ? a.Rq + (((size_t)rb * T + s) * T + t) * C + h * F : nullptr;
         const float* qrow = qs + t * FP;
         const float* krow = ks + s * FP;
 #pragma unroll 3
@@ -90,7 +91,7 @@
         for (int s = 0; s < TMAX; ++s) {
             rv[s] = f32x4{0.f, 0.f, 0.f, 0.f};
             if constexpr (RPE)
-                rv[s] = *reinterpret_cast<const f32x4*>(a.Rv + (((size_t)b * T + t) * T + min(s, T - 1)) * C + h * F + f4 * 4);
+                rv[s] = *reinterpret_cast<const f32x4*>(a.Rv + (((size_t)rb * T + t) * T + min(s, T - 1)) * C + h * F + f4 * 4);
         }
         for (int p = 0; p < np; ++p) {
             const float* ar = sc + (p * T + t) * TS;
@@ -144,6 +145,7 @@
     const int T = EXACT ? 16 * NT : a.T, C = a.C, HW = a.HW, C3 = 3 * a.C;
     const int F = C / a.heads, NJ = EXACT ? JM : F >> 4;
     const int b = blockIdx.z, h = blockIdx.y, p0 = blockIdx.x * 16;
+    const int rb = RPE && a.item_rep ? a.item_rep[b] : b;
     const int tid = threadIdx.x, wv = tid >> 6, l = tid & 63, i16 = l & 15, g = l >> 4;
     const float* qb = a.qkv + ((size_t)b * T * HW + p0) * C3 + h * F;
     auto row = [&](int t, int px) { return qb + ((size_t)t * HW + px) * C3; };
@@ -173,7 +175,7 @@
         for (int m = 0; m < NT; ++m) q1[u][m] = row(tcl[m], 2 * wv + u) + 4 * g;
     const float* rkq[NT];
 #pragma unroll
-    for (int n = 0; n < NT; ++n) rkq[n] = (size_t)b * T * T * C + (size_t)tcl[n] * C + h * F + 4 * g + (const float*)nullptr;
+    for (int n = 0; n < NT; ++n) rkq[n] = (size_t)rb * T * T * C + (size_t)tcl[n] * C + h * F + 4 * g + (const float*)nullptr;
     auto request = [&](Ops& o, int grp, bool own, bool rel) {
 #pragma unroll
         for (int jj = 0; jj < JG; ++jj) {
@@ -324,7 +326,7 @@
     if (EXACT ? wv < JM : wv < NJ) {
         const int f0 = 16 * wv + i16;
         const float* vb = qb + 2 * C + f0;
-        const float* rvb = RPE ? a.Rv + ((size_t)b * T) * T * C + h * F + f0 : nullptr;
+        const float* rvb = RPE ? a.Rv + ((size_t)rb * T) * T * C + h * F + f0 : nullptr;
 #pragma unroll 1
         for (int m = 0; m < NT; ++m) {
             if (16 * m >= T) break;
diff --git a/video-diffusion_amd/csrc/attn_temporal_long.hip b/video-diffusion_amd/csrc/attn_temporal_long.hip
--- a/video-diffusion_amd/csrc/attn_temporal_long.hip
+++ b/video-diffusion_amd/csrc/attn_temporal_long.hip
@@ -44,7 +44,8 @@
     auto row = [&](int t, int px) { return qb + ((size_t)t * HW + px) * C3; };
     auto ld4 = [](const float* p) { return *reinterpret_cast<const f32x4*>(p); };
     const f32x4 zero4 = {0.f, 0.f, 0.f, 0.f};
-    const size_t rbase = (size_t)b * T * T * C + h * F;
+    const int rb = RPE && a.item_rep ? a.item_rep[b] : b;
+    const size_t rbase = (size_t)rb * T * T * C + h * F;
     const int tq = min(t0 + i16, T - 1);
 
     f32x4 acc[16];
@@ -135,7 +136,7 @@
 #pragma unroll
                 for (int r = 0; r < 4; ++r) acc[tl][r] *= al[(4 * g + r) * 16 + tl];
             if constexpr (RPE) {
-                const float* rvb = a.Rv + (size_t)b * T * T * C + f0;
+                const float* rvb = a.Rv + (size_t)rb * T * T * C + f0;
 #pragma unroll 1
                 for (int k4 = 0; k4 < 4; ++k4) {
                     const int s = min(s0 + 4 * k4 + g, T - 1);
@@ -195,6 +196,7 @@
     const int b = blockIdx.z / NQ, t0 = 16 * (blockIdx.z - b * NQ), h = blockIdx.y, p = blockIdx.x;
     const int nq = min(16, T - t0);
     const int tid = threadIdx.x;
+    const int rb = RPE && a.item_rep ? a.item_rep[b] : b;
     const float* qb = a.qkv + ((size_t)b * T * HW + p) * C3 + h * F;
     const size_t fr = (size_t)HW * C3;
     auto ld4 = [](const float* x) { return *reinterpret_cast<const f32x4*>(x); };
@@ -203,8 +205,8 @@
         const int tl = pr / T, s = pr - tl * T, t = t0 + tl;
         const float* q = qb + t * fr;
         const float* k = qb + s * fr + C;
-        const float* rk = RPE ? a.Rk + (((size_t)b * T + t) * T + s) * C + h * F : nullptr;
-        const float* rq = RPE ? a.Rq + (((size_t)b * T + s) * T + t) * C + h * F : nullptr;
+        const float* rk = RPE ? a.Rk + (((size_t)rb * T + t) * T + s) * C + h * F : nullptr;
+        const float* rq = RPE ? a.Rq + (((size_t)rb * T + s) * T + t) * C + h * F : nullptr;
         float acc = 0.f;
         for (int f = 0; f < F; f += 4) {
             const f32x4 qv = ld4(q + f) * a.scale, kv = ld4(k + f);
@@ -232,7 +234,7 @@
         const int tl = item / F4, f4 = item - tl * F4, t = t0 + tl;
         const float* ar = sc + tl * TS;
         const float* vb = qb + 2 * C + 4 * f4;
-        const float* rv = RPE ? a.Rv + (((size_t)b * T + t) * T) * C + h * F + 4 * f4 : nullptr;
+        const float* rv = RPE ? a.Rv + (((size_t)rb * T + t) * T) * C + h * F + 4 * f4 : nullptr;
         f32x4 o = {0.f, 0.f, 0.f, 0.f};
         for (int s = 0; s < T; ++s) {
             f32x4 v = ld4(vb + s * fr);
diff --git a/video-diffusion_amd/csrc/backward.hip b/video-diffusion_amd/csrc/backward.hip
--- a/video-diffusion_amd/csrc/backward.hip
+++ b/video-diffusion_amd/csrc/backward.hip
@@ -620,6 +620,7 @@
     float* P = ks + T * FP;
     float* M = P + T * TS;
     const int p = blockIdx.x, b = blockIdx.y, tid = threadIdx.x;
+    const int rb = RPE && a.item_rep ? a.item_rep[b] : b;
     const size_t tok0 = (size_t)b * T * HW + p;
     for (int i = tid; i < T * TS; i += 256) M[i] = 0.f;
     for (int h = 0; h < a.heads; ++h) {
@@ -632,8 +633,8 @@
         __syncthreads();
         for (int pr = tid; pr < T * T; pr += 256) {
             const int t = pr / T, s_ = pr - t * T;
-            const float* rk = RPE ? a.Rk + (((size_t)b * T + t) * T + s_) * C + h * F : nullptr;
-            const float* rq = RPE ? a.Rq + (((size_t)b * T + s_) * T + t) * C + h * F : nullptr;
+            const float* rk = RPE ? a.Rk + (((size_t)rb * T + t) * T + s_) * C + h * F : nullptr;
+            const float* rq = RPE ? a.Rq + (((size_t)rb * T + s_) * T + t) * C + h * F : nullptr;
             float w = 0.f;
             for (int f = 0; f < F; ++f) {
                 const float k = ks[s_ * FP + f];
@@ -675,6 +676,7 @@
     float* ks = qs + QC * FP;
     float* P = ks + T * FP;
     float* M = P + QC * TS;
+    const int rb = RPE && a.item_rep ? a.item_rep[b] : b;
     const size_t tok0 = (size_t)b * T * HW + p;
     for (int i = tid; i < QC * TS; i += 256) M[i] = 0.f;
     for (int h = 0; h < a.heads; ++h) {
@@ -688,8 +690,8 @@
         __syncthreads();
         for (int pr = tid; pr < nr * T; pr += 256) {
             const int tl = pr / T, s_ = pr - tl * T, t = r0 + tl;
-            const float* rk = RPE ? a.Rk + (((size_t)b * T + t) * T + s_) * C + h * F : nullptr;
-            const float* rq = RPE ? a.Rq + (((size_t)b * T + s_) * T + t) * C + h * F : nullptr;
+            const float* rk = RPE ? a.Rk + (((size_t)rb * T + t) * T + s_) * C + h * F : nullptr;
+            const float* rq = RPE ? a.Rq + (((size_t)rb * T + s_) * T + t) * C + h * F : nullptr;
             float w = 0.f;
             for (int f = 0; f < F; ++f) {
                 const float k = ks[s_ * FP + f];
diff --git a/video-diffusion_amd/csrc/engine.hip b/video-diffusion_amd/csrc/engine.hip
--- a/video-diffusion_amd/csrc/engine.hip
+++ b/video-diffusion_amd/csrc/engine.hip
@@ -59,6 +59,10 @@
 static const int CH_MULT_64[] = {1, 2, 3, 4};
 static const int CH_MULT_32[] = {1, 2, 2, 2};
 static bool split_math() { return math_mode() != MATH_FP32; }
+static bool rpe_dedup_default() {
+    static const bool v = [] { const char* e = getenv("VD_RPE_DEDUP"); return !(e && e[0] == '0' && !e[1]); }();
+    return v;
+}
 
 constexpr int STEM_KPAD = 64;
 
@@ -214,7 +218,9 @@
     struct RpeGroup { int C; std::vector<int> blocks; long long* d_hid = nullptr; long long* d_out = nullptr; };
     std::vector<RpeGroup> rpe_groups;
     std::vector<float*> rpe_R;
-    int rpe_all(const float* te, const int64_t* fidx, int B, int T, hipStream_t st, Arena& ar);
+    int* rpe_rep = nullptr;
+    bool rpe_dedup = rpe_dedup_default();
+    int rpe_all(const float* te, const float* t_frames, const int64_t* fidx, int B, int T, hipStream_t st, Arena& ar);
     int rpe_tables();
     void rpe_group_blocks();
     float* d_freq_time = nullptr; int n_freq_time = 0;
@@ -826,7 +832,7 @@
                 if ((rc = launch_rpe_table(W(rp[i]->table), fidx, B, T, C, cfg.rp_alpha, cfg.rp_beta, cfg.rp_gamma,
                                            Rall + i * rrows * C, st))) return rc;
         AttnTemporalArgs ta{qkv, R[0], R[1], R[2], amask, o, B, T, HW, C, cfg.num_heads,
-                            cfg.allow_interactions_between_padding, scale};
+                            cfg.allow_interactions_between_padding, scale, cfg.use_rpe_net ? rpe_rep : nullptr};
         { const double Fd = C / cfg.num_heads;
           ProfScope ps(PC_ATTN_TEMPORAL, 10.0 * B * HW * cfg.num_heads * T * T * Fd, 16.0 * tok * C + 12.0 * rrows * C, st);
           rc = launch_attn_temporal(ta, st); }
@@ -899,13 +905,19 @@
     return 0;
 }
 
-int vd_engine::rpe_all(const float* te, const int64_t* fidx, int B, int T, hipStream_t st, Arena& ar) {
+int vd_engine::rpe_all(const float* te, const float* t_frames, const int64_t* fidx, int B, int T, hipStream_t st, Arena& ar) {
     rpe_R.clear();
+    rpe_rep = nullptr;
     if (!cfg.use_rpe_net || attn.empty() || !te_total) return 0;
     rpe_group_blocks();
     const size_t rrows = (size_t)B * T * T;
     rpe_R.assign(3 * attn.size(), nullptr);
     int rc = 0;
+    int* rep = ar.get<int>(B);
+    if (!ar.dry && !tape) {
+        if ((rc = launch_rpe_item_rep(t_frames, fidx, B, T, rpe_dedup ? 0 : 1, rep, st))) return rc;
+        rpe_rep = rep;
+    }
     for (auto& g : rpe_groups) {
         const int nn = 3 * (int)g.blocks.size(), C = g.C;
         float* Rg = ar.get<float>((size_t)nn * rrows * C);
@@ -916,11 +928,12 @@
         ar.release(mk);
         if (ar.dry) continue;
         VD_REQUIRE(g.d_hid && g.d_out, "rpe_all: offset tables missing (ensure_ws builds them)");
-        if ((rc = launch_rpe_hidden_tab(te, te_total, wbuf, g.d_hid, fidx, B, T, C, Eh, nn, rrows * C, st))) return rc;
+        if ((rc = launch_rpe_hidden_tab(te, te_total, wbuf, g.d_hid, fidx, B, T, C, Eh, nn, rrows * C, st, rpe_rep))) return rc;
         IgemmArgs q = linear_args((int)rrows, C, C);
         q.src0 = Eh; q.out = Rg;
         q.wfrag = wbuf + params[attn[g.blocks[0]].rq.ow].off; q.bias = wbuf + params[attn[g.blocks[0]].rq.ob].off;
         q.zcount = nn; q.zs_a = q.zs_out = (int)(rrows * C); q.ztab = g.d_out; q.zbase = wbuf;
+        q.item_rep = rpe_rep; q.rows_per_item = T * T;
         if ((rc = igemm_p(q, st))) return rc;
     }
     return 0;
@@ -964,7 +977,8 @@
         }
     }
     rpe_R.clear();
-    if (!(pp && pp->build_only) && (rc = rpe_all(te, in.fidx, B, T, st, ar))) return rc;
+    rpe_rep = nullptr;
+    if (!(pp && pp->build_only) && (rc = rpe_all(te, tfr, in.fidx, B, T, st, ar))) return rc;
     attn_seq = 0;
     std::vector<Tens> hs;
     Tens h{x8, STEM_KPAD, S};
@@ -2093,7 +2107,7 @@
     int n_inv = 0;
     if ((use_pre || want_suf) && (rc = invariant_frames(obs, lat, N, st, &inv, &n_inv))) return rc;
     const bool pre_on = use_pre && n_inv > 0, suf_on = want_suf && n_inv > 0 && n_inv < N;
-    key.flags = (pre_on ? 1 : 0) | (suf_on ? 2 : 0);
+    key.flags = (pre_on ? 1 : 0) | (suf_on ? 2 : 0) | (e->rpe_dedup ? 4 : 0);
     const int hit = find_window_graph(e, key, inv);
     if (hit >= 0) {
         e->win_cur = hit;
@@ -2578,6 +2592,25 @@
 
 int vd_linear_stats_split(int M, int N, int HW) { return HW / gemm_split_stats_rows(M, N); }
 
+int vd_set_rpe_dedup(vd_engine* e, int on) {
+    VD_REQUIRE(e, "null engine");
+    e->rpe_dedup = on != 0;
+    return 0;
+}
+
+int vd_rpe_dedup(vd_engine* e) { return e && e->rpe_dedup ? 1 : 0; }
+
+int vd_rpe_item_rep_host(const float* t_frames, const long long* frame_indices, int B, int T, int* rep) {
+    VD_REQUIRE(t_frames && frame_indices && rep && B > 0 && T > 0, "vd_rpe_item_rep_host: shape");
+    for (int b = 0; b < B; ++b) rep[b] = rpe_item_rep(reinterpret_cast<const unsigned*>(t_frames), frame_indices, T, b);
+    return 0;
+}
+
+int vd_rpe_rows_redundant_host(const int* rep, int rows_per_item, int m0, int m1) {
+    VD_REQUIRE(rep && rows_per_item > 0 && m0 >= 0 && m1 >= m0, "vd_rpe_rows_redundant_host: rows");
+    return rpe_rows_redundant(rep, rows_per_item, m0, m1) ? 1 : 0;
+}
+
 int vd_pack_conv3_wino(const float* host_oihw, float* host_out, int O, int I) {
     VD_REQUIRE(host_oihw && host_out && O % 64 == 0 && I % 16 == 0, "O multiple of 64, I multiple of 16");
     pack_conv3_wino(host_oihw, host_out, O, I);
diff --git a/video-diffusion_amd/csrc/gemm_frag.hip b/video-diffusion_amd/csrc/gemm_frag.hip
--- a/video-diffusion_amd/csrc/gemm_frag.hip
+++ b/video-diffusion_amd/csrc/gemm_frag.hip
@@ -24,13 +24,17 @@
     const int tid = threadIdx.x, lane = tid & 63, wave = __builtin_amdgcn_readfirstlane(tid >> 6);
     const int wm = wave >> 1, wn = wave & 1;
     const int lr = lane & 31, lh = lane >> 5;
-    const int m0 = blockIdx.x * BM, n0 = blockIdx.y * BN;
+    int bxi = blockIdx.x, byi = blockIdx.y, bzi = blockIdx.z;
+    const bool rpe_map = a.zcount > 1 && a.item_rep;
+    if (rpe_map) rpe_block_order(a.item_rep, a.M / a.rows_per_item, bxi, byi, bzi);
+    const int m0 = bxi * BM, n0 = byi * BN;
+    if (rpe_map && rpe_rows_redundant(a.item_rep, a.rows_per_item, m0, min(m0 + BM, a.M) - 1)) return;
     const int lrow = tid >> 3, lq = tid & 7;
     const int nchunk = a.Cin >> 5, ncoblk = a.Cout >> 5;
     const int C1 = a.Cin - a.C0;
     GEMM_STAMP(0);
     if (a.zcount > 1) {
-        const int z = blockIdx.z;
+        const int z = bzi;
         a.src0 += (size_t)z * a.zs_a; a.out += (size_t)z * a.zs_out;
         a.wfrag = a.zbase + a.ztab[2 * z];
         a.bias = a.zbase + a.ztab[2 * z + 1];
@@ -49,7 +53,7 @@
     const auto bsrc = __builtin_amdgcn_make_buffer_rsrc(const_cast<float*>(a.wfrag), 0, a.Cin * a.Cout * 4, 0x00020000);
     unsigned bo[NI];
 #pragma unroll
-    for (int j = 0; j < NI; ++j) bo[j] = (unsigned)min((int)blockIdx.y * (BN / 32) + wn * NI + j, ncoblk - 1) * 4096u + lane * 16u;
+    for (int j = 0; j < NI; ++j) bo[j] = (unsigned)min(byi * (BN / 32) + wn * NI + j, ncoblk - 1) * 4096u + lane * 16u;
 
     f32x4 ra[AR], bfr[4][NI], afr[2][MI];
     auto a_prefetch = [&](int chunk) {
diff --git a/video-diffusion_amd/csrc/gemm_split.hip b/video-diffusion_amd/csrc/gemm_split.hip
--- a/video-diffusion_amd/csrc/gemm_split.hip
+++ b/video-diffusion_amd/csrc/gemm_split.hip
@@ -66,13 +66,17 @@
         byi = loc % gridDim.y;
         bxi = (loc / gridDim.y) * 8 + xcd;
     }
+    int bzi = blockIdx.z;
+    const bool rpe_map = a.zcount > 1 && a.item_rep;
+    if (rpe_map) rpe_block_order(a.item_rep, a.M / a.rows_per_item, bxi, byi, bzi);
     const int m0 = bxi * BM, n0 = byi * BN;
+    if (rpe_map && rpe_rows_redundant(a.item_rep, a.rows_per_item, m0, min(m0 + BM, a.M) - 1)) return;
     const int lgrp = tid >> 3, lrow = ((lgrp >> 1) & 3) + 8 * (lgrp >> 3) + 4 * (lgrp & 1), lq = tid & 7;
     const int cpt = a.Cin >> 5;
     const int nchunk = CONV ? 9 * cpt : cpt, ncoblk = a.Cout >> 5;
     const int C1 = a.Cin - a.C0;
     if (a.zcount > 1) {
-        const int z = blockIdx.z;
+        const int z = bzi;
         a.src0 += (size_t)z * a.zs_a; a.out += (size_t)z * a.zs_out;
         a.wfrag = a.zbase + a.ztab[2 * z];
         a.bias = a.zbase + a.ztab[2 * z + 1];
diff --git a/video-diffusion_amd/csrc/misc.hip b/video-diffusion_amd/csrc/misc.hip
--- a/video-diffusion_amd/csrc/misc.hip
+++ b/video-diffusion_amd/csrc/misc.hip
@@ -156,14 +156,19 @@
 
 __global__ __launch_bounds__(256) void rpe_hidden_tab_kernel(const float* __restrict__ te, int te_ld, const float* __restrict__ wbase,
                                                              const long long* __restrict__ tab, const int64_t* __restrict__ fidx, int T, int C,
-                                                             float* __restrict__ E, size_t zs_e) {
+                                                             float* __restrict__ E, size_t zs_e, const int* __restrict__ item_rep) {
     __shared__ float feat[64][3];
-    const long long* tz = tab + 3 * blockIdx.y;
+    int bxi = blockIdx.x, byi = blockIdx.y, bzi = 0;
+    if (item_rep) {
+        rpe_block_order(item_rep, gridDim.x / T, bxi, byi, bzi);
+        if (item_rep[bxi / T] != bxi / T) return;
+    }
+    const long long* tz = tab + 3 * byi;
     te += tz[0];
     const float* Wd = wbase + tz[1];
     const float* bd = wbase + tz[2];
-    E += blockIdx.y * zs_e;
-    const int bt = blockIdx.x, b = bt / T;
+    E += byi * zs_e;
+    const int bt = bxi, b = bt / T;
     for (int s0 = 0; s0 < T; s0 += 64) {
         const int ns = min(64, T - s0);
         __syncthreads();
@@ -185,8 +190,20 @@
 }
 
 int launch_rpe_hidden_tab(const float* te, int te_ld, const float* wbase, const long long* tab, const int64_t* fidx, int B, int T, int C,
-                          float* E, int nz, size_t zs_e, hipStream_t s) {
-    hipLaunchKernelGGL(rpe_hidden_tab_kernel, dim3(B * T, nz), dim3(256), 0, s, te, te_ld, wbase, tab, fidx, T, C, E, zs_e);
+                          float* E, int nz, size_t zs_e, hipStream_t s, const int* item_rep) {
+    hipLaunchKernelGGL(rpe_hidden_tab_kernel, dim3(B * T, nz), dim3(256), 0, s, te, te_ld, wbase, tab, fidx, T, C, E, zs_e, item_rep);
+    VD_HIP(hipGetLastError());
+    return 0;
+}
+
+__global__ __launch_bounds__(64) void rpe_item_rep_kernel(const float* __restrict__ t_frames, const int64_t* __restrict__ fidx, int B, int T,
+                                                          int identity, int* __restrict__ rep) {
+    for (int b = threadIdx.x; b < B; b += 64)
+        rep[b] = identity ? b : rpe_item_rep(reinterpret_cast<const unsigned*>(t_frames), reinterpret_cast<const long long*>(fidx), T, b);
+}
+
+int launch_rpe_item_rep(const float* t_frames, const int64_t* fidx, int B, int T, int identity, int* rep, hipStream_t s) {
+    hipLaunchKernelGGL(rpe_item_rep_kernel, dim3(1), dim3(64), 0, s, t_frames, fidx, B, T, identity, rep);
     VD_HIP(hipGetLastError());
     return 0;
 }
diff --git a/video-diffusion_amd/csrc/vd_common.h b/video-diffusion_amd/csrc/vd_common.h
--- a/video-diffusion_amd/csrc/vd_common.h
+++ b/video-diffusion_amd/csrc/vd_common.h
@@ -100,6 +100,7 @@
     int stats_hw;
     int zcount, zs_a, zs_out;
     const long long* ztab = nullptr; const float* zbase = nullptr;
+    const int* item_rep = nullptr; int rows_per_item = 0;
     int wsplit;
     float* ksplit_ws;
     size_t ksplit_ws_floats;
@@ -122,7 +123,33 @@
     int B, T, HW, C, heads;
     int allow_pad;
     float scale;
-};
+    const int* item_rep = nullptr;
+};
+
+__host__ __device__ inline int rpe_item_rep(const unsigned* t_frames_bits, const long long* fidx, int T, int b) {
+    for (int c = 0; c < b; ++c) {
+        bool same = true;
+        for (int t = 0; t < T && same; ++t)
+            same = t_frames_bits[c * T + t] == t_frames_bits[b * T + t] && fidx[c * T + t] == fidx[b * T + t];
+        if (same) return c;
+    }
+    return b;
+}
+__host__ __device__ inline bool rpe_rows_redundant(const int* rep, int rows_per_item, int m0, int m1) {
+    for (int b = m0 / rows_per_item; b <= m1 / rows_per_item; ++b)
+        if (rep[b] == b) return false;
+    return true;
+}
+
+__device__ inline void rpe_block_order(const int* rep, int nitem, int& bx, int& by, int& bz) {
+    bool all = true;
+    for (int b = 0; b < nitem; ++b) all = all && rep[b] == b;
+    if (all) return;
+    const unsigned lin = blockIdx.x + gridDim.x * (blockIdx.y + gridDim.y * blockIdx.z);
+    by = (int)(lin % gridDim.y);
+    bz = (int)((lin / gridDim.y) % gridDim.z);
+    bx = (int)(lin / (gridDim.y * gridDim.z));
+}
 
 enum ConvClGather {
     CG_QUAD,
@@ -295,7 +322,8 @@
 int launch_scatter_stats(const double* src, int split, int C, const int* list, int n, double* dst, hipStream_t s);
 int launch_sinus_embed(const float* t, int n, int dim, const float* freqs, float* out, hipStream_t s);
 int launch_rpe_hidden_tab(const float* te, int te_ld, const float* wbase, const long long* tab, const int64_t* fidx, int B, int T, int C,
-                          float* E, int nz, size_t zs_e, hipStream_t s);
+                          float* E, int nz, size_t zs_e, hipStream_t s, const int* item_rep = nullptr);
+int launch_rpe_item_rep(const float* t_frames, const int64_t* fidx, int B, int T, int identity, int* rep, hipStream_t s);
 int launch_rpe_table(const float* table, const int64_t* fidx, int B, int T, int C, float alpha, float beta,
                      float gamma, float* R, hipStream_t s);
 int launch_posenc_add(const float* x, const float* P, const float* femb, int nfr, int HW, int C, float* y,
```

Result: no change. 51.34 (median of 6 runs) (+0.5%).
